# nv-tlabs/LION

Measured on AMD Instinct MI355X. Metric: shapes/sec @1000-step DDIM, Bx2048pts, higher is better.
Workload: dtype f32 (operands of the 3x3x3 voxel convolutions and of the long 1x1 convolutions cut into fp16 hi/lo pairs on the 16-bi...

## Files before the change

include/lion_hip.h:

```cpp
#ifndef LION_HIP_H_
#define LION_HIP_H_

#include <stddef.h>
#include <stdint.h>

#ifdef __cplusplus
extern "C" {
#endif

typedef void *lionStream_t;

#define LION_OK 0
#define LION_EINVAL (-1)
#define LION_EUNSUPPORTED (-2)
#define LION_EWORKSPACE (-3)

int lion_abi_version(void);

size_t lion_avg_voxelize_workspace_bytes(int B, int C, int N, int r);
int lion_avg_voxelize_forward(const float *feat, const int32_t *coords, int B, int C, int N,
                              int r, float *out, int32_t *ind, int32_t *cnt, void *ws,
                              size_t ws_bytes, lionStream_t stream);

int lion_voxelize_points_forward(const float *feat, const float *coords, int B, int C, int N,
// ... 31 lines not shown
int lion_grouping_backward(const float *gy, const int32_t *idx, int B, int C, int N, int M,
                           int U, float *gx, lionStream_t stream);

int lion_furthest_point_sampling(const float *coords, int B, int N, int M, int32_t *idx,
                                 lionStream_t stream);

int lion_gather_features_forward(const float *feat, const int32_t *idx, int B, int C, int N,
                                 int M, float *out, lionStream_t stream);
int lion_gather_features_backward(const float *gy, const int32_t *idx, int B, int C, int N,
                                  int M, float *gx, lionStream_t stream);

int lion_three_nn_interpolate_forward(const float *points, const float *centers,
                                      const float *cfeat, int B, int C, int N, int M,
                                      float *out, int32_t *idx, float *wgt,
                                      lionStream_t stream);
int lion_three_nn_interpolate_cat_forward(const float *points, const float *centers, const float *cfeat, const float *temb,
                                          int ld_t, const float *skip, int B, int C1, int C2, int C3, int N, int M,
                                          float *out, int32_t *idx, float *wgt, lionStream_t stream);
int lion_three_nn_interpolate_backward(const float *gy, const int32_t *idx, const float *wgt,
                                       int B, int C, int N, int M, float *gx,
                                       lionStream_t stream);

int lion_chamfer_forward(const float *xyz1, const float *xyz2, int B, int N, int M,
                         float *dist1, float *dist2, int32_t *idx1, int32_t *idx2,
                         lionStream_t stream);
int lion_chamfer_backward(const float *xyz1, const float *xyz2, const float *gdist1,
                          const float *gdist2, const int32_t *idx1, const int32_t *idx2, int B,
                          int N, int M, float *gxyz1, float *gxyz2, lionStream_t stream);
int lion_chamfer_loss_reduce(const float *dist1, const float *dist2, int B, int N, int M, float s1,
                             float s2, float *loss, lionStream_t stream);
int lion_chamfer_loss_backward(const float *xyz1, const float *xyz2, const int32_t *idx1,
                               const int32_t *idx2, const float *gloss, int B, int N, int M, float s1,
                               float s2, float *gxyz1, float *gxyz2, lionStream_t stream);

size_t lion_emd_workspace_bytes(int B, int N, int M);
int lion_emd_approxmatch(const float *xyz1, const float *xyz2, int B, int N, int M,
                         float *match, void *ws, size_t ws_bytes, lionStream_t stream);
int lion_emd_cost(const float *xyz1, const float *xyz2, int B, int N, int M, float *cost, void *ws,
                  size_t ws_bytes, lionStream_t stream);
int lion_emd_matchcost(const float *xyz1, const float *xyz2, const float *match, int B, int N,
                       int M, float *cost, void *ws, size_t ws_bytes, lionStream_t stream);
int lion_emd_matchcost_backward(const float *grad_cost, const float *xyz1, const float *xyz2,
                                const float *match, int B, int N, int M, float *grad1,
                                float *grad2, lionStream_t stream);

int lion_ddim_update(const float *x, const float *eps, const float *z, size_t numel, float s,
                     float c, float sigma, float *out, lionStream_t stream);
int lion_ddpm_update(const float *x, const float *eps, const float *z, size_t numel,
                     int t_is_zero, float k_outer, float k_a, float k_b, float scale,
                     float temp, float *out, lionStream_t stream);
int lion_chain_begin_step(const float *table, int n_steps, int32_t *counter, float *t_out, int B, float *cur,
                          lionStream_t stream);
int lion_chain_update_noise(int mode, const float *x, const float *eps, size_t numel, const float *cur,
                            const uint32_t *seed , uint32_t stream_id, float *out,
                            float *z_out, lionStream_t stream);
int lion_chain_begin_step_temb(const float *table, int n_steps, int32_t *counter, float *t_out, int B, float *cur,
                               const float *temb_table, int temb_width, float *temb_out, lionStream_t stream);
int lion_chain_update_noise_cm(int mode, const float *x, const float *eps_cm, int B, int N, const float *cur,
                               const uint32_t *seed, uint32_t stream_id, float *out, float *z_out, lionStream_t stream);
int lion_latent_unpack(const float *x, int B, int N, int D, float *all, float *coords, float *rest, lionStream_t stream);
int lion_concat_broadcast(const float *a, const float *t, int B, int Ca, int Ct, int N, int ld_t, float *out,
                          lionStream_t stream);

size_t lion_conv3d_packed_floats(int Cout, int Cin);
int lion_conv3d_pack_weights(const float *w, int Cout, int Cin, float *wp, lionStream_t stream);
int lion_conv3d_k3_forward(const float *x, const float *wp, const float *bias, int B, int Cin,
                           int Cout, int r, float *y, lionStream_t stream);
size_t lion_conv3d_wgrad_workspace_floats(int B, int Cin, int Cout, int r);
int lion_conv3d_k3_wgrad(const float *x, const float *gy, int B, int Cin, int Cout, int r, float *gw, float *ws,
                         size_t ws_floats, lionStream_t stream);
int lion_conv3d_k3_wgrad_split(const float *x, const float *gy, int B, int Cin, int Cout, int r, float *gw, float *ws,
                               size_t ws_floats, lionStream_t stream);
size_t lion_conv3d_wgrad_sparse_workspace_floats(int B, int Cin, int Cout, int r);
int lion_conv3d_k3_wgrad_split_sparse(const float *x, const float *gy, const int32_t *cnt, int B, int Cin, int Cout, int r,
                                      float *gw, float *ws, size_t ws_floats, lionStream_t stream);

int lion_conv3d_stat_tiles(int r, int Cout, int B, int sparse);
int lion_conv3d_k3_fused_forward(const float *x, const float *wp, const float *bias, int B, int Cin,
                                 int Cout, int r, const float *pro_a, const float *pro_b, const float *pro_bias,
                                 const float *tconst, float *y, float *stats, int32_t *occ, lionStream_t stream);
size_t lion_conv3d_occupancy_ints(int r, int Cout, int B);
int lion_conv3d_const_response(const float *wsum, const float *bias2, const float *bias1, const float *pro_a,
                               const float *pro_b, int B, int Cin, int Cout, float *tconst, lionStream_t stream);
int lion_conv3d_tile_occupancy(const int32_t *cnt, int B, int r, int Cout, int32_t *occ_m1, int32_t *occ_m2,
                               lionStream_t stream);
int lion_conv3d_tile_occupancy_aware(const int32_t *cnt, int B, int r, int Cout, int32_t *occ_m1, int32_t *occ_m2,
                                     int consumer_aware, lionStream_t stream);
int lion_groupnorm_fold(const float *stats, int B, int C, int T, int G, int voxels, const float *gamma,
                        const float *beta, const float *fac, const float *gbias, int ld_fg, float eps,
                        float *A, float *Bs, float *chmean, lionStream_t stream);
size_t lion_conv3d_split_packed_halfs(int Cout, int Cin);
int lion_conv3d_split_pack_weights(const float *w, int Cout, int Cin, uint16_t *wp, lionStream_t stream);
int lion_conv3d_split_stat_tiles(int r, int Cout);
int lion_conv3d_k3_split_forward(const float *x, const uint16_t *wp, const float *bias, int B, int Cin, int Cout,
                                 int r, const float *pro_a, const float *pro_b, const float *pro_bias,
                                 const float *tconst, float *y, float *stats, int32_t *occ, lionStream_t stream);
int lion_conv3d_k3_half_forward(const float *x, const uint16_t *wp, const float *bias, int B, int Cin, int Cout,
                                int r, const float *pro_a, const float *pro_b, const float *pro_bias,
                                const float *tconst, float *y, float *stats, int32_t *occ, lionStream_t stream);
size_t lion_skinny_packed_floats(int Cout, int Cin);
int lion_skinny_pack_weights(const float *w, int Cout, int Cin, float *wp, lionStream_t stream);
int lion_skinny_splits(int Cin, int Cout);
int lion_skinny_gemm(const float *pin, int ks_in, const float *bias_in, int act_in, const float *addT,
                     const float *wp, int nb, int Cin, int Cout, float *pout, lionStream_t stream);
int lion_skinny_finish(const float *A, int ks_a, const float *bias_a, const float *Bp, int ks_b, const float *resid,
                       int nb, int C, int mode, float *y, lionStream_t stream);
int lion_skinny_gemm_se_finish(const float *pin, int ks_in, const float *bias_in, int act_in, const float *wp, int nb, int Cin,
                               int Cout, const float *A, int ks_a, const float *bias_a, const float *resid, float *y,
                               lionStream_t stream);
int lion_to_channel_major(const float *a, int lda, int Ca, float *oa, const float *b, int ldb, int Cb, float *ob, int B,
                          lionStream_t stream);
int lion_from_channel_major(const float *x, int B, int C, float *y, lionStream_t stream);
int lion_groupnorm_fold_se(const float *stats, int B, int C, int T, int G, int voxels, const float *gamma,
                           const float *beta, const float *fac, const float *gbias, int ld_fg, float eps, const float *w1,
                           const float *w2, int H, float *A, float *Bs, lionStream_t stream);
int lion_se_gate(const float *chmean, const float *w1, const float *w2, int B, int C, int H, float *A,
                 float *Bs, lionStream_t stream);
int lion_trilinear_devoxelize_affine_forward(const float *coords, const float *feat, const float *scale,
                                             const float *shift, int B, int C, int N, int r, float *out,
                                             lionStream_t stream);
size_t lion_devoxelize_plan_bytes(int B, int N, int r);
int lion_trilinear_devoxelize_plan(const float *coords, int B, int N, int r, void *plan, size_t plan_bytes,
                                   lionStream_t stream);
int lion_trilinear_devoxelize_planned_forward(const void *plan, size_t plan_bytes, const float *coords, const float *feat,
                                              const float *scale, const float *shift, int B, int C, int N, int r,
                                              float *out, lionStream_t stream);

int lion_row_stats(const float *x, int rows, int L, float *stats, lionStream_t stream);
size_t lion_pwconv_packed_floats(int Cout, int Cin);
int lion_pwconv_pack_weights(const float *w, int Cout, int Cin, float *wp, lionStream_t stream);
int lion_pwconv_stat_tiles(int Cout, int Cin, int L);
int lion_pwconv_forward(const float *x, const float *wp, const float *bias, int B, int Cin, int Cout, int L,
                        const float *pro_a, const float *pro_b, float *y, float *stats, lionStream_t stream);
int lion_pwconv_forward_max(const float *x, const float *wp, const float *bias, int B, int Cin, int Cout, int L,
                            const float *pro_a, const float *pro_b, const float *out_a, const float *out_b,
                            float *stats, float *ymax, lionStream_t stream);
size_t lion_pwconv_split_packed_halfs(int Cout, int Cin);
int lion_pwconv_split_pack_weights(const float *w, int Cout, int Cin, uint16_t *wp, lionStream_t stream);
int lion_pwconv_split_pack_weights_t(const float *w, int Cout, int Cin, const uint16_t *wp, uint16_t *wpt, lionStream_t stream);
int lion_pwconv_split_stat_tiles(int Cout, int Cin, int L);
int lion_pwconv_split_forward(const float *x, const uint16_t *wp, const float *bias, int B, int Cin, int Cout, int L,
                              const float *pro_a, const float *pro_b, float *y, float *stats, lionStream_t stream);
int lion_linear_attention_core(const float *qkv, int B, int H, int D, int N, float *out, lionStream_t stream);
int lion_linear_attention_core_backward(const float *qkv, const float *gout, int B, int H, int D, int N, float *gqkv,
                                        lionStream_t stream);
int lion_linear_forward(const float *x, const float *wp, const float *bias, int B, int K, int O, int act, float slope,
                        float *y, lionStream_t stream);
int lion_affine_swish(const float *x, const float *A, const float *Bs, int rows, int L, float *y,
                      lionStream_t stream);
int lion_affine_swish_max(const float *x, const float *A, const float *Bs, int rows, int M, int U,
                          float *y, lionStream_t stream);
int lion_timestep_embedding(const float *t, const float *row, float scale, int B, int half, int D, float *emb,
                            lionStream_t stream);
int lion_affine_swish_add(const float *x, const float *A, const float *Bs, const float *addend, int rows, int L, float *y,
                          lionStream_t stream);

size_t lion_scatter_csr_workspace_bytes(int B, int E, int bins);
int lion_scatter_csr(const float *gy, const int32_t *idx, const float *w, int B, int C, int S, int E, int bins, void *ws,
                     size_t ws_bytes, float *gx, lionStream_t stream);

size_t lion_pwconv_wgrad_workspace_bytes(int B, int Cin, int Cout, int L);
int lion_pwconv_wgrad(const float *x, const float *gy, int B, int Cin, int Cout, int L, void *ws, size_t ws_bytes,
                      float *gw, float *gb, lionStream_t stream);

int lion_gn_train_fold(const float *stats, const float *gw, const float *gb, const float *fac, int fac_stride,
                       const float *bias, int bias_stride, int B, int C, int G, int L, float eps, float *A, float *Bs,
                       float *mean, float *rstd, lionStream_t stream);
int lion_row_stats64(const float *x, int rows, int L, double *stats, lionStream_t stream);
int lion_gn_train_fold64(const double *stats, const float *gw, const float *gb, const float *fac, int fac_stride,
                         const float *bias, int bias_stride, int B, int C, int G, int L, float eps, float *A,
                         float *Bs, float *mean, float *rstd, lionStream_t stream);
int lion_gn_train_bwd_fold(const float *S, const float *mean, const float *rstd, const float *gw, const float *gb,
                           const float *fac, int fac_stride, int B, int C, int G, int L, float *Q, float *R, float *dfac,
                           float *dbias, int d_stride, float *pw, const float *A, const double *xstats, const float *gate,
                           const float *qse, float *Aout, lionStream_t stream);
int lion_gn_train_param_grads(const float *pw, int B, int C, float *dgw, float *dgb, float *dxs, lionStream_t stream);
int lion_se_gate_fwd(const float *stats, const float *w1, const float *w2, int B, int C, int Cr, int L, float *mean, float *h,
                     float *g, float *zero, lionStream_t stream);
int lion_se_gate_bwd(const float *S, const float *g, const float *h, const float *mean, const float *w1, const float *w2, int B,
                     int C, int Cr, int L, float *dpre2, float *dpre1, float *Q, float *dw1, float *dw2, lionStream_t stream);
int lion_rows_dot2(const float *g, const float *v, const float *ws, int B, int C, int N, float *S, lionStream_t stream);
int lion_trilinear_devoxelize_backward_affine(const float *gy, const int32_t *inds, const float *wgts, const float *x,
                                              const float *Ap, const float *Q, const float *R, int B, int C, int N, int r3,
                                              float *dx, lionStream_t stream);
int lion_gn_se_gate_fwd(const double *xstats, const float *A, const float *Bs, const float *w1, const float *w2, int B, int C, int Cr,
                        int L, float *mean, float *h, float *g, float *A2, float *B2, lionStream_t stream);
int lion_gn_se_gate_bwd(const float *S, const double *xstats, const float *A, const float *Bs, const float *g, const float *h,
                        const float *mean, const float *w1, const float *w2, int B, int C, int Cr, int L, float *Sp, float *dpre2,
                        float *dpre1, float *Qse, float *dw1, float *dw2, lionStream_t stream);
int lion_affine_act(const float *x, const float *A, const float *Bs, int rows, int L, int act, float *y,
                    lionStream_t stream);
int lion_affine_act_bwd_stats(const float *x, const float *gy, const float *A, const float *Bs, int rows, int L, int act,
                              float *S, lionStream_t stream);
int lion_affine_act_bwd_apply(const float *x, const float *gy, const float *A, const float *Bs, const float *Q,
                              const float *R, int rows, int L, int act, float *dx, lionStream_t stream);
int lion_affine_act_dropout(const float *x, const float *A, const float *Bs, int rows, int L, int act, const uint64_t *seed,
                            float keep, float *y, lionStream_t stream);
int lion_affine_act_dropout_bwd_stats(const float *x, const float *gy, const float *A, const float *Bs, int rows, int L, int act,
                                      const uint64_t *seed, float keep, float *S, lionStream_t stream);
int lion_affine_act_dropout_bwd_apply(const float *x, const float *gy, const float *A, const float *Bs, const float *Q,
                                      const float *R, int rows, int L, int act, const uint64_t *seed, float keep, float *dx,
                                      lionStream_t stream);
int lion_affine_act_max(const float *x, const float *A, const float *Bs, int rows, int M, int U, int act, float *y,
                        lionStream_t stream);
int lion_affine_act_max_bwd_stats(const float *x, const float *gy, const float *A, const float *Bs, int rows, int M, int U,
                                  int act, float *S, lionStream_t stream);
int lion_affine_act_max_bwd_apply(const float *x, const float *gy, const float *A, const float *Bs, const float *Q,
                                  const float *R, int rows, int M, int U, int act, float *dx, lionStream_t stream);

int lion_adam_chunk(void);
int lion_adam_row(void);
int lion_adam_step(const uint64_t *table, const int32_t *numel, const int32_t *blockmap, int blocks, int tensors, const float *lr,
                   float beta1, float beta2, float eps, float weight_decay, float ema_decay, lionStream_t stream);

int lion_grad_sqnorm_partials(const uint64_t *table, const int32_t *numel, const int32_t *blockmap, int blocks, float *partials,
                              lionStream_t stream);
int lion_grad_clip_coef(const float *partials, int n, float max_norm, float *out2, lionStream_t stream);
int lion_adam_step_scaled(const uint64_t *table, const int32_t *numel, const int32_t *blockmap, int blocks, int tensors,
                          const float *lr, float beta1, float beta2, float eps, float weight_decay, float ema_decay,
                          const float *grad_scale, lionStream_t stream);

#define LION_ODE_RUNNING 0
#define LION_ODE_FINISHED 1
#define LION_ODE_TOO_SMALL_STEP (-1)
typedef struct lion_ode_ctrl {
  double t, h_abs, t_bound, direction, rtol, atol;
  double h, t_new, err_norm, h0, d1, sign;
  int32_t stage, cur, status, step_rejected;
  int32_t yslot, fslot, nfe, n_accepted;
  int32_t n_rejected, accepted, pad0, pad1;
} lion_ode_ctrl;
size_t lion_ode_partials_bytes(size_t n);
int lion_ode_stage(double *Y, const double *K, size_t n, lion_ode_ctrl *ctrl, float *x32, float *t_model, int B,
                   lionStream_t stream);
int lion_ode_drift(const float *eps, int cm_points, const float *x32, size_t n, const float *t_model, float beta_start,
                   float beta_delta, float neg_beta_start, float half_beta_delta, float one_minus_sigma2_0,
                   const float *mix_a, const float *mix_b, int mix_len, double *K, lion_ode_ctrl *ctrl,
                   lionStream_t stream);
// ... 9 lines not shown
```

lion_amd/_lib.py:

```python
from __future__ import annotations

import ctypes as C
import os

_HERE = os.path.dirname(os.path.abspath(__file__))
SO_PATH = os.environ.get("LION_HIP_SO") or os.path.join(_HERE, "csrc", "liblion_hip.so")

_vp, _i, _f, _sz = C.c_void_p, C.c_int, C.c_float, C.c_size_t

SIGNATURES = {
    "lion_abi_version": (_i, []),
    "lion_avg_voxelize_workspace_bytes": (_sz, [_i, _i, _i, _i]),
    "lion_avg_voxelize_forward": (_i, [_vp, _vp, _i, _i, _i, _i, _vp, _vp, _vp, _vp, _sz, _vp]),
    "lion_voxelize_points_forward": (_i, [_vp, _vp, _i, _i, _i, _i, _i, _f, _vp, _vp, _vp, _vp,
                                          _vp, _sz, _vp]),
    "lion_voxel_plan_bytes": (_sz, [_i, _i, _i]),
    "lion_voxel_index": (_i, [_vp, _i, _i, _i, _i, _f, _vp, _vp, _vp, _vp, _sz, _vp]),
    "lion_voxel_scatter": (_i, [_vp, _vp, _sz, _i, _i, _i, _i, _vp, _vp]),
    "lion_voxel_scatter_read": (_i, [_vp, _vp, _sz, _i, _i, _i, _i, _vp, _vp, _vp]),
    "lion_avg_voxelize_backward": (_i, [_vp, _vp, _vp, _i, _i, _i, _i, _vp, _vp]),
    "lion_trilinear_devoxelize_forward": (_i, [_vp, _vp, _i, _i, _i, _i, _i, _vp, _vp, _vp, _vp]),
    "lion_trilinear_devoxelize_backward": (_i, [_vp, _vp, _vp, _i, _i, _i, _i, _vp, _vp]),
    "lion_ball_query": (_i, [_vp, _vp, _i, _i, _i, _f, _i, _vp, _vp]),
    "lion_grouping_forward": (_i, [_vp, _vp, _i, _i, _i, _i, _i, _vp, _vp]),
    "lion_group_points_forward": (_i, [_vp, _vp, _vp, _vp, _i, _i, _i, _i, _i, _vp, _vp]),
    "lion_grouping_backward": (_i, [_vp, _vp, _i, _i, _i, _i, _i, _vp, _vp]),
    "lion_furthest_point_sampling": (_i, [_vp, _i, _i, _i, _vp, _vp]),
    "lion_gather_features_forward": (_i, [_vp, _vp, _i, _i, _i, _i, _vp, _vp]),
    "lion_gather_features_backward": (_i, [_vp, _vp, _i, _i, _i, _i, _vp, _vp]),
    "lion_three_nn_interpolate_forward": (_i, [_vp, _vp, _vp, _i, _i, _i, _i, _vp, _vp, _vp, _vp]),
    "lion_three_nn_interpolate_backward": (_i, [_vp, _vp, _vp, _i, _i, _i, _i, _vp, _vp]),
    "lion_chamfer_forward": (_i, [_vp, _vp, _i, _i, _i, _vp, _vp, _vp, _vp, _vp]),
    "lion_chamfer_backward": (_i, [_vp, _vp, _vp, _vp, _vp, _vp, _i, _i, _i, _vp, _vp, _vp]),
    "lion_chamfer_loss_reduce": (_i, [_vp, _vp, _i, _i, _i, _f, _f, _vp, _vp]),
    "lion_chamfer_loss_backward": (_i, [_vp, _vp, _vp, _vp, _vp, _i, _i, _i, _f, _f, _vp, _vp, _vp]),
    "lion_emd_workspace_bytes": (_sz, [_i, _i, _i]),
    "lion_emd_approxmatch": (_i, [_vp, _vp, _i, _i, _i, _vp, _vp, _sz, _vp]),
    "lion_emd_cost": (_i, [_vp, _vp, _i, _i, _i, _vp, _vp, _sz, _vp]),
    "lion_emd_matchcost": (_i, [_vp, _vp, _vp, _i, _i, _i, _vp, _vp, _sz, _vp]),
    "lion_emd_matchcost_backward": (_i, [_vp, _vp, _vp, _vp, _i, _i, _i, _vp, _vp, _vp]),
    "lion_conv3d_packed_floats": (_sz, [_i, _i]),
    "lion_conv3d_pack_weights": (_i, [_vp, _i, _i, _vp, _vp]),
    "lion_conv3d_k3_forward": (_i, [_vp, _vp, _vp, _i, _i, _i, _i, _vp, _vp]),
    "lion_conv3d_wgrad_workspace_floats": (_sz, [_i, _i, _i, _i]),
    "lion_conv3d_k3_wgrad": (_i, [_vp, _vp, _i, _i, _i, _i, _vp, _vp, _sz, _vp]),
    "lion_conv3d_k3_wgrad_split": (_i, [_vp, _vp, _i, _i, _i, _i, _vp, _vp, _sz, _vp]),
    "lion_conv3d_wgrad_sparse_workspace_floats": (_sz, [_i, _i, _i, _i]),
    "lion_conv3d_k3_wgrad_split_sparse": (_i, [_vp, _vp, _vp, _i, _i, _i, _i, _vp, _vp, _sz, _vp]),
    "lion_conv3d_stat_tiles": (_i, [_i, _i, _i, _i]),
    "lion_conv3d_k3_fused_forward": (_i, [_vp, _vp, _vp, _i, _i, _i, _i, _vp, _vp, _vp, _vp, _vp, _vp, _vp, _vp]),
    "lion_conv3d_const_response": (_i, [_vp, _vp, _vp, _vp, _vp, _i, _i, _i, _vp, _vp]),
    "lion_conv3d_occupancy_ints": (_sz, [_i, _i, _i]),
    "lion_conv3d_tile_occupancy": (_i, [_vp, _i, _i, _i, _vp, _vp, _vp]),
    "lion_conv3d_tile_occupancy_aware": (_i, [_vp, _i, _i, _i, _vp, _vp, _i, _vp]),
    "lion_conv3d_split_packed_halfs": (_sz, [_i, _i]),
    "lion_conv3d_split_pack_weights": (_i, [_vp, _i, _i, _vp, _vp]),
    "lion_conv3d_split_stat_tiles": (_i, [_i, _i]),
    "lion_conv3d_k3_split_forward": (_i, [_vp, _vp, _vp, _i, _i, _i, _i, _vp, _vp, _vp, _vp, _vp, _vp, _vp, _vp]),
    "lion_conv3d_k3_half_forward": (_i, [_vp, _vp, _vp, _i, _i, _i, _i, _vp, _vp, _vp, _vp, _vp, _vp, _vp, _vp]),
    "lion_groupnorm_fold": (_i, [_vp, _i, _i, _i, _i, _i, _vp, _vp, _vp, _vp, _i, _f, _vp, _vp, _vp, _vp]),
    "lion_groupnorm_fold_se": (_i, [_vp, _i, _i, _i, _i, _i, _vp, _vp, _vp, _vp, _i, _f, _vp, _vp, _i, _vp, _vp, _vp]),
    "lion_skinny_packed_floats": (_sz, [_i, _i]),
    "lion_skinny_pack_weights": (_i, [_vp, _i, _i, _vp, _vp]),
    "lion_skinny_splits": (_i, [_i, _i]),
    "lion_skinny_gemm": (_i, [_vp, _i, _vp, _i, _vp, _vp, _i, _i, _i, _vp, _vp]),
    "lion_skinny_gemm_se_finish": (_i, [_vp, _i, _vp, _i, _vp, _i, _i, _i, _vp, _i, _vp, _vp, _vp, _vp]),
    "lion_skinny_finish": (_i, [_vp, _i, _vp, _vp, _i, _vp, _i, _i, _i, _vp, _vp]),
    "lion_to_channel_major": (_i, [_vp, _i, _i, _vp, _vp, _i, _i, _vp, _i, _vp]),
    "lion_from_channel_major": (_i, [_vp, _i, _i, _vp, _vp]),
    "lion_se_gate": (_i, [_vp, _vp, _vp, _i, _i, _i, _vp, _vp, _vp]),
    "lion_trilinear_devoxelize_affine_forward": (_i, [_vp, _vp, _vp, _vp, _i, _i, _i, _i, _vp, _vp]),
    "lion_devoxelize_plan_bytes": (_sz, [_i, _i, _i]),
    "lion_trilinear_devoxelize_plan": (_i, [_vp, _i, _i, _i, _vp, _sz, _vp]),
    "lion_trilinear_devoxelize_planned_forward": (_i, [_vp, _sz, _vp, _vp, _vp, _vp, _i, _i, _i, _i, _vp, _vp]),
    "lion_row_stats": (_i, [_vp, _i, _i, _vp, _vp]),
    "lion_pwconv_packed_floats": (_sz, [_i, _i]),
    "lion_pwconv_pack_weights": (_i, [_vp, _i, _i, _vp, _vp]),
    "lion_pwconv_stat_tiles": (_i, [_i, _i, _i]),
    "lion_pwconv_forward": (_i, [_vp, _vp, _vp, _i, _i, _i, _i, _vp, _vp, _vp, _vp, _vp]),
    "lion_pwconv_forward_max": (_i, [_vp, _vp, _vp, _i, _i, _i, _i, _vp, _vp, _vp, _vp, _vp, _vp, _vp]),
    "lion_pwconv_split_packed_halfs": (_sz, [_i, _i]),
    "lion_pwconv_split_pack_weights": (_i, [_vp, _i, _i, _vp, _vp]),
    "lion_pwconv_split_pack_weights_t": (_i, [_vp, _i, _i, _vp, _vp, _vp]),
    "lion_pwconv_split_stat_tiles": (_i, [_i, _i, _i]),
    "lion_pwconv_split_forward": (_i, [_vp, _vp, _vp, _i, _i, _i, _i, _vp, _vp, _vp, _vp, _vp]),
    "lion_linear_attention_core": (_i, [_vp, _i, _i, _i, _i, _vp, _vp]),
    "lion_linear_attention_core_backward": (_i, [_vp, _vp, _i, _i, _i, _i, _vp, _vp]),
    "lion_linear_forward": (_i, [_vp, _vp, _vp, _i, _i, _i, _i, _f, _vp, _vp]),
    "lion_affine_swish": (_i, [_vp, _vp, _vp, _i, _i, _vp, _vp]),
    "lion_affine_swish_max": (_i, [_vp, _vp, _vp, _i, _i, _i, _vp, _vp]),
    "lion_timestep_embedding": (_i, [_vp, _vp, _f, _i, _i, _i, _vp, _vp]),
    "lion_affine_swish_add": (_i, [_vp, _vp, _vp, _vp, _i, _i, _vp, _vp]),
    "lion_scatter_csr_workspace_bytes": (_sz, [_i, _i, _i]),
    "lion_scatter_csr": (_i, [_vp, _vp, _vp, _i, _i, _i, _i, _i, _vp, _sz, _vp, _vp]),
    "lion_pwconv_wgrad_workspace_bytes": (_sz, [_i, _i, _i, _i]),
    "lion_pwconv_wgrad": (_i, [_vp, _vp, _i, _i, _i, _i, _vp, _sz, _vp, _vp, _vp]),
    "lion_gn_train_fold": (_i, [_vp, _vp, _vp, _vp, _i, _vp, _i, _i, _i, _i, _i, _f, _vp, _vp, _vp, _vp, _vp]),
    "lion_row_stats64": (_i, [_vp, _i, _i, _vp, _vp]),
    "lion_gn_train_fold64": (_i, [_vp, _vp, _vp, _vp, _i, _vp, _i, _i, _i, _i, _i, _f, _vp, _vp, _vp, _vp, _vp]),
    "lion_gn_train_bwd_fold": (_i, [_vp, _vp, _vp, _vp, _vp, _vp, _i, _i, _i, _i, _i, _vp, _vp, _vp, _vp, _i, _vp, _vp, _vp, _vp, _vp,
                                    _vp, _vp]),
    "lion_gn_train_param_grads": (_i, [_vp, _i, _i, _vp, _vp, _vp, _vp]),
    "lion_adam_chunk": (_i, []),
    "lion_adam_row": (_i, []),
    "lion_adam_step": (_i, [_vp, _vp, _vp, _i, _i, _vp, _f, _f, _f, _f, _f, _vp]),
    "lion_grad_sqnorm_partials": (_i, [_vp, _vp, _vp, _i, _vp, _vp]),
    "lion_grad_clip_coef": (_i, [_vp, _i, _f, _vp, _vp]),
    "lion_adam_step_scaled": (_i, [_vp, _vp, _vp, _i, _i, _vp, _f, _f, _f, _f, _f, _vp, _vp]),
    "lion_se_gate_fwd": (_i, [_vp, _vp, _vp, _i, _i, _i, _i, _vp, _vp, _vp, _vp, _vp]),
    "lion_se_gate_bwd": (_i, [_vp, _vp, _vp, _vp, _vp, _vp, _i, _i, _i, _i, _vp, _vp, _vp, _vp, _vp, _vp]),
    "lion_rows_dot2": (_i, [_vp, _vp, _vp, _i, _i, _i, _vp, _vp]),
    "lion_trilinear_devoxelize_backward_affine": (_i, [_vp, _vp, _vp, _vp, _vp, _vp, _vp, _i, _i, _i, _i, _vp, _vp]),
    "lion_gn_se_gate_fwd": (_i, [_vp, _vp, _vp, _vp, _vp, _i, _i, _i, _i, _vp, _vp, _vp, _vp, _vp, _vp]),
    "lion_gn_se_gate_bwd": (_i, [_vp, _vp, _vp, _vp, _vp, _vp, _vp, _vp, _vp, _i, _i, _i, _i, _vp, _vp, _vp, _vp, _vp, _vp, _vp]),
    "lion_affine_act": (_i, [_vp, _vp, _vp, _i, _i, _i, _vp, _vp]),
    "lion_affine_act_bwd_stats": (_i, [_vp, _vp, _vp, _vp, _i, _i, _i, _vp, _vp]),
    "lion_affine_act_bwd_apply": (_i, [_vp, _vp, _vp, _vp, _vp, _vp, _i, _i, _i, _vp, _vp]),
    "lion_affine_act_dropout": (_i, [_vp, _vp, _vp, _i, _i, _i, _vp, _f, _vp, _vp]),
    "lion_affine_act_dropout_bwd_stats": (_i, [_vp, _vp, _vp, _vp, _i, _i, _i, _vp, _f, _vp, _vp]),
    "lion_affine_act_dropout_bwd_apply": (_i, [_vp, _vp, _vp, _vp, _vp, _vp, _i, _i, _i, _vp, _f, _vp, _vp]),
    "lion_affine_act_max": (_i, [_vp, _vp, _vp, _i, _i, _i, _i, _vp, _vp]),
    "lion_affine_act_max_bwd_stats": (_i, [_vp, _vp, _vp, _vp, _i, _i, _i, _i, _vp, _vp]),
    "lion_affine_act_max_bwd_apply": (_i, [_vp, _vp, _vp, _vp, _vp, _vp, _i, _i, _i, _i, _vp, _vp]),
    "lion_ddim_update": (_i, [_vp, _vp, _vp, _sz, _f, _f, _f, _vp, _vp]),
    "lion_ddpm_update": (_i, [_vp, _vp, _vp, _sz, _i, _f, _f, _f, _f, _f, _vp, _vp]),
    "lion_chain_begin_step": (_i, [_vp, _i, _vp, _vp, _i, _vp, _vp]),
    "lion_chain_update_noise": (_i, [_i, _vp, _vp, _sz, _vp, _vp, C.c_uint32, _vp, _vp, _vp]),
    "lion_chain_begin_step_temb": (_i, [_vp, _i, _vp, _vp, _i, _vp, _vp, _i, _vp, _vp]),
    "lion_chain_update_noise_cm": (_i, [_i, _vp, _vp, _i, _i, _vp, _vp, C.c_uint32, _vp, _vp, _vp]),
    "lion_latent_unpack": (_i, [_vp, _i, _i, _i, _vp, _vp, _vp, _vp]),
    "lion_concat_broadcast": (_i, [_vp, _vp, _i, _i, _i, _i, _i, _vp, _vp]),
    "lion_three_nn_interpolate_cat_forward": (_i, [_vp, _vp, _vp, _vp, _i, _vp, _i, _i, _i, _i, _i, _i, _vp, _vp, _vp, _vp]),
    "lion_ode_partials_bytes": (_sz, [_sz]),
    "lion_ode_stage": (_i, [_vp, _vp, _sz, _vp, _vp, _vp, _i, _vp]),
    "lion_ode_drift": (_i, [_vp, _i, _vp, _sz, _vp, _f, _f, _f, _f, _f, _vp, _vp, _i, _vp, _vp, _vp]),
    "lion_ode_error_partials": (_i, [_vp, _vp, _sz, _vp, _vp, _vp]),
    "lion_ode_control": (_i, [_vp, _sz, _vp, _vp]),
}



_ERR = {-1: "LION_EINVAL (bad shape / null pointer)",
        -2: "LION_EUNSUPPORTED (shape outside what the kernels implement)",
        -3: "LION_EWORKSPACE (workspace too small)"}

_lib = None


def load() -> C.CDLL:
    global _lib
    if _lib is not None:
        return _lib
    if not os.path.exists(SO_PATH):
        raise RuntimeError(
            f"lion_amd: HIP extension not built: {SO_PATH} is missing. Run "
            f"`python -c 'import __graft_entry__ as g; g.build()'` or lion_amd/csrc/build.sh. "
            f"There is no CPU fallback.")
    lib = C.CDLL(SO_PATH)
    for name, (res, args) in SIGNATURES.items():
        try:
            fn = getattr(lib, name)
        except AttributeError as e:
            raise RuntimeError(f"lion_amd: {SO_PATH} does not export {name}") from e
        fn.restype = res
        fn.argtypes = args
    _lib = lib
    return lib


def check(code: int, what: str) -> None:
    if code != 0:
        msg = _ERR.get(code, f"hipError {code}" if code > 0 else f"error {code}")
        raise RuntimeError(f"lion_amd: {what} failed: {msg}")


# ... 40 lines not shown
```

lion_amd/chain.py:

```python
from __future__ import annotations

from collections import OrderedDict

import numpy as np
import torch

from . import _lib, _wcache

DDIM, DDPM = 0, 1
RECORD = None
TEMB_TABLE = __import__("os").environ.get("LION_TEMB_TABLE", "1") != "0"
CHANNEL_MAJOR_EPS = __import__("os").environ.get("LION_CHAIN_CM_EPS", "1") != "0"

def policy_key() -> tuple:
    from . import conv_ops, fused_ops, geometry
    from .models import pvcnn2_ada
    return (pvcnn2_ada.SPARSE_CONV1, pvcnn2_ada.FUSE_INFERENCE, pvcnn2_ada.OVERLAP_POINT_BRANCH, geometry.ENABLED,
            geometry.SPLIT_GRAPH, conv_ops.SPLIT, fused_ops.PW_SPLIT, pvcnn2_ada.VOX_PLAN, TEMB_TABLE, fused_ops.MAX_RECOMPUTE,
            pvcnn2_ada.SKIP_UNREAD, pvcnn2_ada.SKIP_UNREAD_LEVEL2, CHANNEL_MAJOR_EPS, conv_ops.PRECISION)


def channel_major(model, shape) -> bool:
    n_pts, n_cls = getattr(model, "num_points", 0), getattr(model, "num_classes", 0)
    return CHANNEL_MAJOR_EPS and hasattr(model, "geometry_source") and n_cls == 4 and int(np.prod(shape)) == n_pts * n_cls


def same_conditioning(owner, condition_input, clip_feat) -> bool:
    same = lambda buf, new: (buf is None) == (new is None) and (buf is None or buf.shape == new.shape)
    return same(owner.cond, condition_input) and same(owner.clip, clip_feat)


class LRU:

    def __init__(self, capacity=4):
        self._entries, self._capacity = OrderedDict(), capacity

    def lookup(self, key, usable, build):
        hit = self._entries.get(key)
        if hit is not None and usable(hit):
            self._entries.move_to_end(key)
            return hit
        self._entries.pop(key, None)
        hit = self._entries[key] = build()
        while len(self._entries) > self._capacity:
            self._entries.popitem(last=False)
        return hit

    def clear(self):
        self._entries.clear()


class CapturedStep:

    def __init__(self, model, step, x, *, warmup=2, split=None):
        self.model, self.x = model, x
        self.fingerprint, self.policy = _wcache.fingerprint(model), policy_key()
        self.pinned = []
        dev = x.device
        from . import geometry
        src = getattr(model, "geometry_source", None)
        self.geo_graphs = self.graph_b = self.graphs = self.waits = self.geo_plan = None
        if split is None:
            split = geometry.SPLIT_GRAPH and src is not None and not geometry.ENABLED
        main = torch.cuda.current_stream(dev)
        side = torch.cuda.Stream(device=dev)
        side.wait_stream(main)
        with _wcache.pinning(self.pinned):
            with torch.no_grad(), torch.cuda.stream(side):
                for _ in range(warmup):
                    step()
            main.wait_stream(side)
            if split:
                self.geo_stream = torch.cuda.Stream(device=dev)
                self.ev_step = torch.cuda.Event()

                def geo(boundary=None):
                    mods, coords = src(x)
                    return geometry.compute_chain(mods, coords, boundary=boundary)
                self.geo_stream.wait_stream(main)
                with torch.no_grad(), torch.cuda.stream(self.geo_stream):
                    geo()
                main.wait_stream(self.geo_stream)
                torch.cuda.synchronize(dev)
                self.geo_graphs = [torch.cuda.CUDAGraph()]
                gs = torch.cuda.Stream(device=dev)
                gs.wait_stream(main)

                def geo_cut(i):
                    if i == 1:
                        self.geo_graphs[-1].capture_end()
                        self.geo_graphs.append(torch.cuda.CUDAGraph())
                        self.geo_graphs[-1].capture_begin(pool=self.geo_graphs[0].pool())
                with torch.no_grad(), torch.cuda.stream(gs):
                    self.geo_graphs[0].capture_begin()
                    try:
                        self.geo_plan = geo(geo_cut)
                    finally:
                        self.geo_graphs[-1].capture_end()
                main.wait_stream(gs)
                torch.cuda.synchronize(dev)
                self.geo_stage_of_graph = [0, self.geo_plan["stages"] - 1][:len(self.geo_graphs)]
                self.ev_geo = [torch.cuda.Event() for _ in self.geo_graphs]
# ... 166 lines not shown
```

lion_amd/csrc/conv3d.hip:

```cpp
#include "common.h"

namespace {

typedef float f32x16 __attribute__((ext_vector_type(16)));
#ifndef LION_CONV_KC
#define LION_CONV_KC 4
#endif
#ifndef LION_CONV_WAVES
#define LION_CONV_WAVES 2
#endif
constexpr int KC = LION_CONV_KC;

__device__ __forceinline__ float pro_act(float v, float pa, float pb) {
  const float t = v * pa + pb;
  return swish_fast(t);
}

template <int TD, int TH, int TW, int COT, int VB, bool PRO, bool STATS>
__global__ __launch_bounds__(256, LION_CONV_WAVES) void conv3d_k3_kernel(const float *__restrict__ x,
                                                                const float *__restrict__ wp,
                                                                const float *__restrict__ bias,
                                                                float *__restrict__ y, int Cin,
                                                                int Cout, int r,
                                                                const float *__restrict__ pro_a,
                                                                const float *__restrict__ pro_b,
                                                                const float *__restrict__ pro_bias,
                                                                const float *__restrict__ tconst,
                                                                float *__restrict__ stats,
                                                                int32_t *__restrict__ occ, int B,
                                                                int ntiles) {
  constexpr int TM = 256;
  static_assert(TD * TH * TW == 4 * VB * 32, "tile voxels = 4 waves x VB column blocks x 32");
  constexpr int HD = TD + 2, HH = TH + 2, HW = TW + 2, HALO = HD * HH * HW;
  constexpr int NJ = (HALO + TM - 1) / TM;
  constexpr int WV4 = KC * 27 * COT / 4;
  constexpr int NWV = (WV4 + TM - 1) / TM;
  constexpr int CB = COT / 32;
  constexpr int SWS = ((KC * 27 * COT + 255) / 256) * 256 + 256;
  extern __shared__ __attribute__((aligned(16))) float smem[];
  float *sx = smem;
  float *sw = sx + ((KC * HALO + 3) & ~3);
  float *sbias = sw + 2 * SWS;
  const int npro = PRO ? ((Cin + 63) & ~63) : 0;
  float *spa = sbias + COT, *spb = spa + npro;
  float *spc = spb + npro;
  float *sred = spc + npro;
  float *sT = sx;
  const int tid = threadIdx.x, lane = tid & 63, wave = __builtin_amdgcn_readfirstlane(tid >> 6);
  __shared__ int s_work;
  const bool queued = occ != nullptr;
  const int ncz = Cout / COT;
  for (int iter = 0;; ++iter) {
  int b, tile, co0;
  if (queued) {
    __syncthreads();
    if (tid == 0) s_work = atomicAdd(occ + 2 * B * ntiles, 1);
    __syncthreads();
    const int work = s_work;
    if (work >= B * ntiles * ncz) break;
    const int item = work / ncz;
    b = item % B;
    tile = occ[B * ntiles + b * ntiles + item / B];
    co0 = (work % ncz) * COT;
  } else {
    if (iter) break;
    b = blockIdx.x;
    tile = blockIdx.y;
    co0 = blockIdx.z * COT;
  }
  const int ntw = r / TW, nth = r / TH;
  const int tw_i = tile % ntw, th_i = (tile / ntw) % nth, td_i = tile / (ntw * nth);
  const int d0 = td_i * TD, h0 = th_i * TH, w0 = tw_i * TW;
  const int r2 = r * r, r3 = r2 * r;

  const bool delta = PRO && tconst != nullptr;
  if (PRO) {
    for (int c = tid; c < Cin; c += TM) {
      const float pa = pro_a[(size_t)b * Cin + c], pb = pro_b[(size_t)b * Cin + c];
      spa[c] = pa;
      spb[c] = pb;
      spc[c] = delta ? pro_act(pro_bias ? pro_bias[c] : 0.f, pa, pb) : 0.f;
    }
  }
// ... 87 lines not shown
      for (int cb = 0; cb < CB; ++cb) av[buf][cb] = ap[cb * 32];
    };
    if (wave_on) {
    lds_step(0, 0);
#pragma unroll
    for (int st = 0; st < NS; ++st) {
      if (st + 1 < NS) lds_step(st + 1, (st + 1) & 1);
      __builtin_amdgcn_sched_barrier(0);
#pragma unroll
      for (int cb = 0; cb < CB; ++cb)
#pragma unroll
        for (int vb = 0; vb < VB; ++vb)
          acc[cb][vb] = __builtin_amdgcn_mfma_f32_32x32x2f32(av[st & 1][cb], bv[st & 1][vb], acc[cb][vb], 0, 0, 0);
      __builtin_amdgcn_sched_barrier(0);
    }
    }
  }

  if (delta) {
    __syncthreads();
    for (int e = tid; e < 27 * COT; e += TM) sT[e] = tconst[((size_t)b * 27 + e / COT) * Cout + co0 + e % COT];
    __syncthreads();
  } else if (empty) {
    __syncthreads();
  }
  float *yb = y + ((size_t)b * Cout + co0) * r3;
#pragma unroll
  for (int vb = 0; vb < VB; ++vb) {
    const int v = (wave * VB + vb) * 32 + (lane & 31);
    const int d = v / (TH * TW), h = (v / TW) % TH, w = v % TW;
    const int gv = ((d0 + d) * r + (h0 + h)) * r + (w0 + w);
    const int gd = d0 + d, gh = h0 + h, gw = w0 + w;
    const int cfg = (((gd == 0 ? 0 : gd == r - 1 ? 2 : 1) * 3 + (gh == 0 ? 0 : gh == r - 1 ? 2 : 1)) * 3 +
                     (gw == 0 ? 0 : gw == r - 1 ? 2 : 1));
    const float *addv = delta ? sT + cfg * COT : sbias;
#pragma unroll
    for (int cb = 0; cb < CB; ++cb)
#pragma unroll
      for (int i = 0; i < 16; ++i) {
        const int co = cb * 32 + (i & 3) + 8 * (i >> 2) + 4 * (lane >> 5);
        const float o = acc[cb][vb][i] + addv[co];
        acc[cb][vb][i] = o;
        yb[(size_t)co * r3 + gv] = o;
      }
  }
  if (STATS) {
    constexpr int NWAVE = 4;
#pragma unroll
    for (int cb = 0; cb < CB; ++cb)
#pragma unroll
      for (int i = 0; i < 16; ++i) {
        float s1 = acc[cb][0][i], s2 = acc[cb][0][i] * acc[cb][0][i];
#pragma unroll
        for (int vb = 1; vb < VB; ++vb) { s1 += acc[cb][vb][i]; s2 += acc[cb][vb][i] * acc[cb][vb][i]; }
        s1 = row16_sum_rn(s1); s2 = row16_sum_rn(s2);
        s1 = row_pair_sum_odd_rows(s1); s2 = row_pair_sum_odd_rows(s2);
        if ((lane & 31) == 16) {
          const int co = cb * 32 + (i & 3) + 8 * (i >> 2) + 4 * (lane >> 5);
          sred[(wave * COT + co) * 2] = s1;
          sred[(wave * COT + co) * 2 + 1] = s2;
        }
      }
    __syncthreads();
    if (tid < COT) {
      float s1 = 0.f, s2 = 0.f;
#pragma unroll
      for (int w = 0; w < NWAVE; ++w) { s1 += sred[(w * COT + tid) * 2]; s2 += sred[(w * COT + tid) * 2 + 1]; }
      float *o = stats + (((size_t)b * Cout + co0 + tid) * ntiles + tile) * 2;
      o[0] = s1;
      o[1] = s2;
    }
  }
  }
  if (queued && tid == 0) {
    int32_t *q = occ + 2 * B * ntiles;
    if (atomicAdd(q + 1, 1) == (int)gridDim.x - 1) { q[0] = 0; q[1] = 0; }
  }
}

__global__ void gn_fold_kernel(const float *__restrict__ stats, int C, int T, int G, float count,
                               const float *__restrict__ gamma, const float *__restrict__ beta,
                               const float *__restrict__ fac, const float *__restrict__ gbias, int ld_fg, float eps,
                               float *__restrict__ A, float *__restrict__ Bs, float *__restrict__ chmean) {
  __shared__ double cs[64][2];
  __shared__ double gs[2];
  const int b = blockIdx.y, g = blockIdx.x, cpg = C / G, tid = threadIdx.x;
  int cp2 = 1;
  while (cp2 < cpg) cp2 <<= 1;
  const int LPC = 256 / cp2, ch = tid / LPC, sub = tid % LPC;
  double s1 = 0.0, s2 = 0.0;
  if (ch < cpg) {
    const float2 *p = reinterpret_cast<const float2 *>(stats + (((size_t)b * C + g * cpg + ch) * T) * 2);
    for (int t = sub; t < T; t += LPC) { const float2 v = p[t]; s1 += (double)v.x; s2 += (double)v.y; }
  }
  for (int m = 1; m < LPC && m < 64; m <<= 1) { s1 += __shfl_xor(s1, m, 64); s2 += __shfl_xor(s2, m, 64); }
  if (LPC > 64) {
    __shared__ double ws[4][2];
    if ((tid & 63) == 0) { ws[tid >> 6][0] = s1; ws[tid >> 6][1] = s2; }
    __syncthreads();
    if (sub == 0) {
      s1 = 0.0; s2 = 0.0;
      for (int w = 0; w < LPC / 64; ++w) { s1 += ws[(tid >> 6) + w][0]; s2 += ws[(tid >> 6) + w][1]; }
    }
  }
  if (ch < cpg && sub == 0) {
    cs[ch][0] = s1;
    cs[ch][1] = s2;
    chmean[(size_t)b * C + g * cpg + ch] = (float)(s1 / count);
  }
  __syncthreads();
  if (tid == 0) {
    double g1 = 0.0, g2 = 0.0;
    for (int c = 0; c < cpg; ++c) { g1 += cs[c][0]; g2 += cs[c][1]; }
    gs[0] = g1;
    gs[1] = g2;
  }
  __syncthreads();
  if (tid < cpg) {
    const double n = (double)count * cpg;
    const double mean = gs[0] / n;
    double var = gs[1] / n - mean * mean;
    var = var > 0.0 ? var : 0.0;
    const float rstd = (float)(1.0 / sqrt(var + (double)eps));
    const int c = g * cpg + tid;
    const float f = fac[(size_t)b * ld_fg + c], gb = gbias[(size_t)b * ld_fg + c];
    const float a0 = rstd * gamma[c];
    A[(size_t)b * C + c] = a0 * f;
    Bs[(size_t)b * C + c] = (beta[c] - (float)mean * a0) * f + gb;
  }
}

__global__ __launch_bounds__(256) void gn_fold_se_kernel(const float *__restrict__ stats, int C, int T, int G, float count,
                                                         const float *__restrict__ gamma, const float *__restrict__ beta,
                                                         const float *__restrict__ fac, const float *__restrict__ gbias,
                                                         int ld_fg, float eps, const float *__restrict__ w1,
                                                         const float *__restrict__ w2, int H, float *__restrict__ A,
                                                         float *__restrict__ Bs) {
  __shared__ double cs[256][2];
  __shared__ float sA[256], sB[256], sm[256], sh[128];
  const int b = blockIdx.x, tid = threadIdx.x, lane = tid & 63, wave = tid >> 6, cpg = C / G;
  int cp2 = 1;
  while (cp2 < C) cp2 <<= 1;
  const int LPC = 256 / cp2, ch = tid / LPC, sub = tid % LPC;
  double s1 = 0.0, s2 = 0.0;
  if (ch < C) {
    const float2 *p = reinterpret_cast<const float2 *>(stats + (((size_t)b * C + ch) * T) * 2);
    for (int t = sub; t < T; t += LPC) { const float2 v = p[t]; s1 += (double)v.x; s2 += (double)v.y; }
  }
  for (int m = 1; m < LPC; m <<= 1) { s1 += __shfl_xor(s1, m, 64); s2 += __shfl_xor(s2, m, 64); }
  if (ch < C && sub == 0) { cs[ch][0] = s1; cs[ch][1] = s2; }
  __syncthreads();
  if (tid < C) {
    const int g0 = (tid / cpg) * cpg;
    double g1 = 0.0, g2 = 0.0;
    for (int k = 0; k < cpg; ++k) { g1 += cs[g0 + k][0]; g2 += cs[g0 + k][1]; }
    const double n = (double)count * cpg, mean = g1 / n;
    double var = g2 / n - mean * mean;
    var = var > 0.0 ? var : 0.0;
    const float rstd = (float)(1.0 / sqrt(var + (double)eps));
    const float f = fac[(size_t)b * ld_fg + tid], gb = gbias[(size_t)b * ld_fg + tid];
    const float a0 = rstd * gamma[tid];
    const float a = a0 * f, bb = (beta[tid] - (float)mean * a0) * f + gb;
    sA[tid] = a;
    sB[tid] = bb;
    sm[tid] = a * (float)(cs[tid][0] / count) + bb;
  }
  __syncthreads();
  for (int j = wave; j < H; j += 4) {
    float acc = 0.f;
    for (int c = lane; c < C; c += 64) acc += w1[(size_t)j * C + c] * sm[c];
#pragma unroll
    for (int m = 32; m >= 1; m >>= 1) acc += __shfl_xor(acc, m, 64);
    if (lane == 0) sh[j] = acc > 0.f ? acc : 0.f;
  }
  __syncthreads();
  if (tid < C) {
    float acc = 0.f;
    for (int j = 0; j < H; ++j) acc += w2[(size_t)tid * H + j] * sh[j];
    const float g = 1.0f / (1.0f + expf(-acc));
    A[(size_t)b * C + tid] = sA[tid] * g;
    Bs[(size_t)b * C + tid] = sB[tid] * g;
  }
}

__global__ __launch_bounds__(1024) void conv_tile_occ_kernel(const int32_t *__restrict__ cnt, int r, int TD, int TH,
                                                             int32_t *__restrict__ occ1, int32_t *__restrict__ occ2,
                                                             int aware) {
  __shared__ unsigned col[32 * 32];
  __shared__ int flag[2][256];
  const int b = blockIdx.x, B = gridDim.x, tid = threadIdx.x;
  const int nth = r / TH, ntiles = (r / TD) * nth, total = B * ntiles;
  for (int i = tid; i < r * r; i += 1024) col[i] = 0u;
  __syncthreads();
  const int4 *c4 = reinterpret_cast<const int4 *>(cnt + (size_t)b * r * r * r);
  for (int i = tid; i < (r * r * r) >> 2; i += 1024) {
    const int4 v = c4[i];
    if (v.x | v.y | v.z | v.w) {
      const unsigned m4 = (v.x ? 1u : 0u) | (v.y ? 2u : 0u) | (v.z ? 4u : 0u) | (v.w ? 8u : 0u);
      atomicOr(&col[(i << 2) / r], m4 << ((i << 2) % r));
    }
  }
  __syncthreads();
  const int RW = 64 / r;
  for (int e = tid; e < 2 * ntiles; e += 1024) {
    const int t = e % ntiles, margin = 1 + e / ntiles;
    const int dt = (t / nth) * TD, ht = (t % nth) * TH;
    int mask = 0;
    for (int w = 0; w < 4; ++w) {
      const int dl = dt + (w * RW) / TH, hl = ht + (w * RW) % TH;
      unsigned any = 0u;
      for (int d = max(dl - margin, 0); d <= min(dl + margin, r - 1); ++d)
        for (int h = max(hl - margin, 0); h <= min(hl + RW - 1 + margin, r - 1); ++h) any |= col[d * r + h];
      mask |= (any ? 1 : 0) << w;
    }
    flag[margin - 1][t] = mask;
  }
  __syncthreads();
  __shared__ unsigned long long bal[2][4];
  const int m = tid >> 8, t = tid & 255, lane = tid & 63, w = (tid >> 6) & 3;
  const bool live = tid < 512 && t < ntiles;
  const int f = live ? flag[m][t] : 0;
  const unsigned long long bl = __ballot(f != 0);
  if (tid < 512 && lane == 0) bal[m][w] = bl;
  __syncthreads();
  if (live) {
    int32_t *occ = m == 0 ? occ1 : occ2;
    if (occ) {
      int before = __popcll(bal[m][w] & ((1ull << lane) - 1ull)), occupied = 0;
      for (int ww = 0; ww < 4; ++ww) {
        const int c = __popcll(bal[m][ww]);
        if (ww < w) before += c;
        occupied += c;
      }
      int32_t *fl = occ + (size_t)b * ntiles, *list = occ + total + (size_t)b * ntiles;
      int need = flag[1][t] != 0;
      if (m == 0) {
        if (aware == 2) {
          need = 0;
        } else {
          const int td = t / nth, th = t % nth;
          for (int dd = max(td - 1, 0); dd <= min(td + 1, r / TD - 1); ++dd)
            for (int hh = max(th - 1, 0); hh <= min(th + 1, nth - 1); ++hh) need |= flag[1][dd * nth + hh] != 0;
        }
      }
      fl[t] = f | (need << 8) | ((m == 1 && flag[0][t] != 0) ? (1 << 9) : 0);
      list[f ? before : occupied + (t - before)] = t;
      if (b == 0 && t == 0) { occ[2 * total] = 0; occ[2 * total + 1] = 0; occ[2 * total + 2] = aware; }
    }
  }
}

__global__ __launch_bounds__(256) void conv_tconst_kernel(const float *__restrict__ wsum, const float *__restrict__ bias2,
                                                          const float *__restrict__ bias1, const float *__restrict__ pro_a,
                                                          const float *__restrict__ pro_b, int Cin, int Cout,
                                                          float *__restrict__ tconst) {
  __shared__ float sc[256];
  const int cfg = blockIdx.x, b = blockIdx.y, tid = threadIdx.x;
  for (int c = tid; c < Cin; c += 256)
    sc[c] = pro_act(bias1 ? bias1[c] : 0.f, pro_a[(size_t)b * Cin + c], pro_b[(size_t)b * Cin + c]);
  __syncthreads();
  for (int co = tid; co < Cout; co += 256) {
    double acc = bias2 ? (double)bias2[co] : 0.0;
    const float *w = wsum + (size_t)cfg * Cin * Cout + co;
    for (int c = 0; c < Cin; ++c) acc += (double)w[(size_t)c * Cout] * (double)sc[c];
    tconst[((size_t)b * 27 + cfg) * Cout + co] = (float)acc;
  }
}

__global__ void conv3d_pack_kernel(const float *__restrict__ w, int Cout, int Cin, int Cin_pad,
                                   float *__restrict__ wp) {
  const int i = blockIdx.x * blockDim.x + threadIdx.x;
  const int total = Cin_pad * 27 * Cout;
  if (i >= total) return;
  const int co = i % Cout, t = (i / Cout) % 27, ci = i / (Cout * 27);
  wp[i] = ci < Cin ? w[((size_t)co * Cin + ci) * 27 + t] : 0.f;
}

template <int TD, int TH, int TW, int COT, int VB>
static int launch_conv_t(const float *x, const float *wp, const float *bias, float *y, int B, int Cin,
                         int Cout, int r, const float *pa, const float *pb, const float *pbias, const float *tconst,
                         float *stats, int32_t *occ, hipStream_t st) {
  const int tiles = (r / TD) * (r / TH) * (r / TW);
  int n_cu = 0;
  if (int e = lion_cu_count(&n_cu)) return e;
  const long items = (long)B * tiles * (Cout / COT);
  const dim3 grid = occ ? dim3((unsigned)(items < 2L * n_cu ? items : 2L * n_cu)) : dim3(B, tiles, Cout / COT);
  constexpr int NT = 256;
  constexpr int HALO = (TD + 2) * (TH + 2) * (TW + 2);
  constexpr int SWS = ((KC * 27 * COT + 255) / 256) * 256 + 256;
  static_assert(KC * HALO >= 27 * COT, "the response table must fit the input tile buffer");
  const size_t LDS = (size_t)(((KC * HALO + 3) & ~3) + 2 * SWS + COT + (pa ? 3 * ((Cin + 63) & ~63) : 0) +
                              (NT / 64) * COT * 2) * 4;
#define LION_CONV_GO(PRO_, ST_)                                                                           \
  {                                                                                                       \
    static LionLdsLimit cfg = {};                                                                         \
    if (int e = lion_dynamic_lds(&conv3d_k3_kernel<TD, TH, TW, COT, VB, PRO_, ST_>, LDS, cfg)) return e;  \
    conv3d_k3_kernel<TD, TH, TW, COT, VB, PRO_, ST_><<<grid, NT, LDS, st>>>(x, wp, bias, y, Cin, Cout, r, \
                                                                            pa, pb, pbias, tconst, stats, occ, B, \
                                                                            tiles);                      \
  }
  if (pa && stats) LION_CONV_GO(true, true)
  else if (pa) LION_CONV_GO(true, false)
  else if (stats) LION_CONV_GO(false, true)
  else LION_CONV_GO(false, false)
#undef LION_CONV_GO
  LION_LAUNCH_CHECK();
  return 0;
}

struct ConvPlan { int vb, cot, tiles; };
static ConvPlan conv_plan(int r, int Cout, int B, bool sparse) {
  const int r3 = r * r * r;
  if (!sparse && Cout % 64 == 0 && r >= 16 && (long)(r3 / 512) * (Cout / 64) * B >= 512) return {4, 64, r3 / 512};
  if (Cout % 64 == 0 && (long)(r3 / 256) * (Cout / 64) * B >= 512) return {2, 64, r3 / 256};
  if (Cout % 32 == 0 && r >= 16 && !sparse) return {4, 32, r3 / 512};
  if (Cout % 32 == 0 && r >= 16) return {2, 32, r3 / 256};
  if (Cout % 32 == 0) return {1, 32, r3 / 128};
  return {0, 0, 0};
}

static void conv_tile_dims(int r, int vb, int *td, int *th, int *tw) {
  *tw = r;
  if (r == 32) { *td = vb == 2 ? 2 : 4; *th = 4; }
  else if (r == 16) { *td = vb == 2 ? 4 : 8; *th = 4; }
  else { *td = vb == 2 ? 4 : 2; *th = 8; }
}

static int launch_conv(const float *x, const float *wp, const float *bias, float *y, int B, int Cin, int Cout,
                       int r, const float *pa, const float *pb, const float *pbias, const float *tconst, float *stats,
                       int32_t *occ, hipStream_t st) {
  const ConvPlan p = conv_plan(r, Cout, B, occ != nullptr);
#define LION_CONV_TILE(R_, VB_, COT_, TD_, TH_, TW_)                                                       \
  if (r == R_ && p.vb == VB_ && p.cot == COT_)                                                             \
    return launch_conv_t<TD_, TH_, TW_, COT_, VB_>(x, wp, bias, y, B, Cin, Cout, r, pa, pb, pbias, tconst, stats, occ, st);
  LION_CONV_TILE(32, 2, 64, 2, 4, 32)
  LION_CONV_TILE(32, 4, 64, 4, 4, 32)
  LION_CONV_TILE(16, 4, 64, 8, 4, 16)
  LION_CONV_TILE(32, 4, 32, 4, 4, 32)
  LION_CONV_TILE(32, 2, 32, 2, 4, 32)
  LION_CONV_TILE(16, 2, 32, 4, 4, 16)
  LION_CONV_TILE(16, 2, 64, 4, 4, 16)
  LION_CONV_TILE(16, 4, 32, 8, 4, 16)
  LION_CONV_TILE(8, 2, 64, 4, 8, 8)
  LION_CONV_TILE(8, 1, 32, 2, 8, 8)
#undef LION_CONV_TILE
  return LION_EUNSUPPORTED;
}

}

int lion_internal_sparse_tile_dims(int r, int *td, int *th) {
  if (r != 16 && r != 32) return LION_EUNSUPPORTED;
  const ConvPlan a = conv_plan(r, 64, 32, true), b = conv_plan(r, 32, 32, true), c = conv_plan(r, 64, 1, true);
  if (!a.vb || a.vb != b.vb || a.vb != c.vb) return LION_EUNSUPPORTED;
  int tw;
  conv_tile_dims(r, a.vb, td, th, &tw);
  return 0;
}

extern "C" {

size_t lion_conv3d_packed_floats(int Cout, int Cin) {
  return (size_t)((Cin + KC - 1) / KC * KC) * 27 * Cout;
}

int lion_conv3d_pack_weights(const float *w, int Cout, int Cin, float *wp, lionStream_t stream) {
  if (!w || !wp || Cout <= 0 || Cin <= 0) return LION_EINVAL;
  const int Cin_pad = (Cin + KC - 1) / KC * KC;
  const int total = Cin_pad * 27 * Cout;
  conv3d_pack_kernel<<<lion_cdiv(total, 256), 256, 0, static_cast<hipStream_t>(stream)>>>(w, Cout, Cin, Cin_pad, wp);
  LION_LAUNCH_CHECK();
  return 0;
}

int lion_conv3d_k3_fused_forward(const float *x, const float *wp, const float *bias, int B, int Cin,
                                 int Cout, int r, const float *pro_a, const float *pro_b, const float *pro_bias,
                                 const float *tconst, float *y, float *stats, int32_t *occ, lionStream_t stream) {
  if (!x || !wp || !y || B <= 0 || Cin <= 0 || Cout <= 0) return LION_EINVAL;
  if ((pro_a == nullptr) != (pro_b == nullptr)) return LION_EINVAL;
  if (tconst && !pro_a) return LION_EINVAL;
  if (occ && pro_a && !tconst) return LION_EINVAL;
  if (Cin % KC != 0 || (pro_a && Cin > 256)) return LION_EUNSUPPORTED;
  hipStream_t st = static_cast<hipStream_t>(stream);
  if (r != 8 && r != 16 && r != 32) return LION_EUNSUPPORTED;
  return launch_conv(x, wp, bias, y, B, Cin, Cout, r, pro_a, pro_b, pro_bias, tconst, stats, occ, st);
}

int lion_conv3d_k3_forward(const float *x, const float *wp, const float *bias, int B, int Cin,
                           int Cout, int r, float *y, lionStream_t stream) {
  return lion_conv3d_k3_fused_forward(x, wp, bias, B, Cin, Cout, r, nullptr, nullptr, nullptr, nullptr, y, nullptr,
                                      nullptr, stream);
}

int lion_conv3d_const_response(const float *wsum, const float *bias2, const float *bias1, const float *pro_a,
                               const float *pro_b, int B, int Cin, int Cout, float *tconst, lionStream_t stream) {
  if (!wsum || !pro_a || !pro_b || !tconst || B <= 0 || Cin <= 0 || Cout <= 0) return LION_EINVAL;
  if (Cin > 256) return LION_EUNSUPPORTED;
  conv_tconst_kernel<<<dim3(27, B), 256, 0, static_cast<hipStream_t>(stream)>>>(wsum, bias2, bias1, pro_a, pro_b, Cin,
                                                                                 Cout, tconst);
  LION_LAUNCH_CHECK();
  return 0;
}

size_t lion_conv3d_occupancy_ints(int r, int Cout, int B) {
  if (r != 16 && r != 32) return 0;
  return (size_t)2 * B * conv_plan(r, Cout, B, true).tiles + 4;
}

int lion_conv3d_tile_occupancy(const int32_t *cnt, int B, int r, int Cout, int32_t *occ_m1, int32_t *occ_m2,
                               lionStream_t stream) {
  return lion_conv3d_tile_occupancy_aware(cnt, B, r, Cout, occ_m1, occ_m2, 0, stream);
}

int lion_conv3d_tile_occupancy_aware(const int32_t *cnt, int B, int r, int Cout, int32_t *occ_m1, int32_t *occ_m2,
                                     int consumer_aware, lionStream_t stream) {
  if (!cnt || (!occ_m1 && !occ_m2) || B <= 0 || Cout <= 0) return LION_EINVAL;
  if (r != 16 && r != 32) return LION_EUNSUPPORTED;
  const ConvPlan p = conv_plan(r, Cout, B, true);
  if (!p.vb || p.tiles > 256 || (((uintptr_t)cnt) & 15) != 0) return LION_EUNSUPPORTED;
  int td, th, tw;
  conv_tile_dims(r, p.vb, &td, &th, &tw);
  conv_tile_occ_kernel<<<B, 1024, 0, static_cast<hipStream_t>(stream)>>>(cnt, r, td, th, occ_m1, occ_m2,
                                                                         consumer_aware == 2 ? 2 : consumer_aware ? 1 : 0);
  LION_LAUNCH_CHECK();
  return 0;
}

int lion_conv3d_stat_tiles(int r, int Cout, int B, int sparse) {
  if (r != 8 && r != 16 && r != 32) return 0;
  return conv_plan(r, Cout, B, sparse != 0).tiles;
}

int lion_groupnorm_fold_se(const float *stats, int B, int C, int T, int G, int voxels, const float *gamma,
                           const float *beta, const float *fac, const float *gbias, int ld_fg, float eps, const float *w1,
                           const float *w2, int H, float *A, float *Bs, lionStream_t stream) {
  if (!stats || !gamma || !beta || !fac || !gbias || !w1 || !w2 || !A || !Bs) return LION_EINVAL;
  if (B <= 0 || C <= 0 || T <= 0 || G <= 0 || C % G != 0 || ld_fg < C || H <= 0) return LION_EINVAL;
  if (C > 256 || C < 4 || H > 128) return LION_EUNSUPPORTED;
  gn_fold_se_kernel<<<B, 256, 0, static_cast<hipStream_t>(stream)>>>(stats, C, T, G, (float)voxels, gamma, beta, fac, gbias,
                                                                     ld_fg, eps, w1, w2, H, A, Bs);
  LION_LAUNCH_CHECK();
  return 0;
}

int lion_groupnorm_fold(const float *stats, int B, int C, int T, int G, int voxels, const float *gamma,
                        const float *beta, const float *fac, const float *gbias, int ld_fg, float eps,
                        float *A, float *Bs, float *chmean, lionStream_t stream) {
  if (!stats || !gamma || !beta || !fac || !gbias || !A || !Bs || !chmean) return LION_EINVAL;
  if (B <= 0 || C <= 0 || T <= 0 || G <= 0 || C % G != 0 || C / G > 64 || ld_fg < C) return LION_EINVAL;
  gn_fold_kernel<<<dim3(G, B), 256, 0, static_cast<hipStream_t>(stream)>>>(stats, C, T, G, (float)voxels, gamma,
                                                                         beta, fac, gbias, ld_fg, eps, A, Bs, chmean);
  LION_LAUNCH_CHECK();
  return 0;
}

}
```

lion_amd/csrc/devoxelize.hip:

```cpp
#include "common.h"

namespace {

template <bool V> struct BoolT { static constexpr bool value = V; };

struct Corners {
  int ix[8];
  float w[8];
};

__device__ __forceinline__ Corners corners_of(float x, float y, float z, int r, int r2) {
  Corners k;
  const float xl = floorf(x), yl = floorf(y), zl = floorf(z);
  const float xd1 = sub_rn(x, xl), yd1 = sub_rn(y, yl), zd1 = sub_rn(z, zl);
  const float xd0 = sub_rn(1.0f, xd1), yd0 = sub_rn(1.0f, yd1), zd0 = sub_rn(1.0f, zd1);
  k.w[0] = mul_rn(mul_rn(xd0, yd0), zd0);
  k.w[1] = mul_rn(mul_rn(xd0, yd0), zd1);
  k.w[2] = mul_rn(mul_rn(xd0, yd1), zd0);
  k.w[3] = mul_rn(mul_rn(xd0, yd1), zd1);
  k.w[4] = mul_rn(mul_rn(xd1, yd0), zd0);
  k.w[5] = mul_rn(mul_rn(xd1, yd0), zd1);
  k.w[6] = mul_rn(mul_rn(xd1, yd1), zd0);
  k.w[7] = mul_rn(mul_rn(xd1, yd1), zd1);
  const int xlo = (int)xl, ylo = (int)yl, zlo = (int)zl;
  const int xs = (xd1 > 0.0f) ? r2 : 0;
  const int ys = (yd1 > 0.0f) ? r : 0;
  const int zs = (zd1 > 0.0f) ? 1 : 0;
  k.ix[0] = xlo * r2 + ylo * r + zlo;
  k.ix[1] = k.ix[0] + zs;
  k.ix[2] = k.ix[0] + ys;
  k.ix[3] = k.ix[2] + zs;
  k.ix[4] = k.ix[0] + xs;
  k.ix[5] = k.ix[4] + zs;
  k.ix[6] = k.ix[4] + ys;
  k.ix[7] = k.ix[6] + zs;
  return k;
}

template <int CT, bool AFF>
__global__ __launch_bounds__(256) void devox_fwd_kernel(const float *__restrict__ coords,
                                                        const float *__restrict__ feat, int C,
                                                        int N, int r, int training,
                                                        float *__restrict__ out,
                                                        int32_t *__restrict__ inds,
                                                        float *__restrict__ wgts,
                                                        const float *__restrict__ scale,
                                                        const float *__restrict__ shift) {
  const int b = blockIdx.z, i = blockIdx.x * blockDim.x + threadIdx.x;
  if (i >= N) return;
  const int r2 = r * r, r3 = r2 * r;
  const float *co = coords + (size_t)b * 3 * N;
  Corners k = corners_of(co[i], co[i + N], co[i + 2 * N], r, r2);
  if (training && blockIdx.y == 0) {
#pragma unroll
    for (int q = 0; q < 8; ++q) {
      wgts[((size_t)b * 8 + q) * N + i] = k.w[q];
      inds[((size_t)b * 8 + q) * N + i] = k.ix[q];
    }
  }
#pragma unroll
  for (int q = 0; q < 8; ++q) k.ix[q] = min(max(k.ix[q], 0), r3 - 1);
  const int c0 = blockIdx.y * CT, c1 = min(C, c0 + CT);
  const float *f = feat + ((size_t)b * C + c0) * r3;
  float *o = out + ((size_t)b * C + c0) * N + i;
  float wsum = 0.f;
  if (AFF) {
    wsum = k.w[0];
#pragma unroll
    for (int q = 1; q < 8; ++q) wsum += k.w[q];
  }
#pragma unroll 4
  for (int c = c0; c < c1; ++c, f += r3, o += N) {
    float v[8];
#pragma unroll
    for (int q = 0; q < 8; ++q) v[q] = f[k.ix[q]];
    float acc = mul_rn(k.w[0], v[0]);
#pragma unroll
    for (int q = 1; q < 8; ++q) acc = add_rn(acc, mul_rn(k.w[q], v[q]));
    if (AFF) acc = acc * scale[(size_t)b * C + c] + shift[(size_t)b * C + c] * wsum;
    *o = acc;
  }
}


template <int LD, bool AFF>
__global__ __launch_bounds__(256) void devox_slab_kernel(
    const float *__restrict__ coords, const float *__restrict__ feat, int C, int N, int r, int PX,
    int XS, int CT, int CI, int slab_floats, int training, float *__restrict__ out,
    int32_t *__restrict__ inds, float *__restrict__ wgts, const float *__restrict__ scale,
    const float *__restrict__ shift) {
  extern __shared__ __attribute__((aligned(16))) unsigned char smem[];
  float *lds = reinterpret_cast<float *>(smem);
  constexpr int PP = 8;
  const int tid = threadIdx.x, b = blockIdx.y, c0 = blockIdx.x * CT;
  const int nch = min(CT, C - c0);
  const int r2 = r * r, r3 = r2 * r;
  const float *co = coords + (size_t)b * 3 * N;
  uint16_t *sorted = reinterpret_cast<uint16_t *>(lds + 2 * slab_floats);
  int *scnt = reinterpret_cast<int *>(sorted + ((N + 1) & ~1));
  unsigned *need = reinterpret_cast<unsigned *>(scnt + XS);

  const int ngrp = (nch + CI - 1) / CI;
  const int nit = ngrp * XS;
  auto slab_count4 = [&](int g, int xs) {
    return XS == 1 ? (min(CI, nch - g * CI) * r3) >> 2 : ((min(r, xs * PX + PX + 1) - xs * PX) * r2) >> 2;
  };
  typedef __attribute__((address_space(3))) float lds_float;
  const uint32_t lds_base = (uint32_t)(uintptr_t)(lds_float *)lds;
  const int wave = __builtin_amdgcn_readfirstlane(tid >> 6);
  auto issue = [&](int it) {
    const int g = it / XS, xs = it - g * XS;
    const float4 *src = reinterpret_cast<const float4 *>(feat + ((size_t)b * C + c0 + g * CI) * r3 + (size_t)xs * PX * r2);
    const int n4 = slab_count4(g, xs);
    const uint32_t dst0 = lds_base + (uint32_t)((it & 1) * slab_floats * 4 + wave * 1024);
    const int row0 = XS == 1 ? 0 : xs * PX * r;
#pragma unroll
    for (int j = 0; j < LD; ++j) {
      const int f = tid + j * 256;
      const float4 *gp = src + f;
      const uint32_t dst = __builtin_amdgcn_readfirstlane(dst0 + j * 4096);
      int row = (4 * f) / r;
      if (XS == 1) row %= r2;
      else row += row0;
      const bool want = f < n4 && ((need[row >> 5] >> (row & 31)) & 1u);
      if (want) {
        unsigned keep;
        asm volatile("s_mov_b32 %0, m0\n\ts_mov_b32 m0, %2\n\ts_nop 0\n\tglobal_load_lds_dwordx4 %1, off\n\ts_mov_b32 m0, %0"
                     : "=&s"(keep) : "v"(gp), "s"(dst) : "memory");
      }
    }
  };
  const int nwords = (r2 + 31) >> 5;
  for (int w = tid; w < nwords; w += 256) need[w] = 0u;
  __syncthreads();
  for (int i = tid; i < N; i += 256) {
    const float x = co[i], y = co[i + N];
    const float xl = floorf(x), yl = floorf(y);
    if (xl >= 0.f && yl >= 0.f && xl < (float)r && yl < (float)r) {
      const int x0 = (int)xl, y0 = (int)yl;
      const int x1 = min(x0 + (sub_rn(x, xl) > 0.0f ? 1 : 0), r - 1), y1 = min(y0 + (sub_rn(y, yl) > 0.0f ? 1 : 0), r - 1);
      const int ra = x0 * r + y0, rb = x0 * r + y1, rc = x1 * r + y0, rd = x1 * r + y1;
      atomicOr(&need[ra >> 5], 1u << (ra & 31));
      atomicOr(&need[rb >> 5], 1u << (rb & 31));
      atomicOr(&need[rc >> 5], 1u << (rc & 31));
      atomicOr(&need[rd >> 5], 1u << (rd & 31));
    }
  }
  __syncthreads();
  issue(0);

  for (int s2 = tid; s2 < XS; s2 += 256) scnt[s2] = 0;
  __syncthreads();
  int sl0[PP];
#pragma unroll
  for (int p = 0; p < PP; ++p) {
    const int i = tid + p * 256;
    sl0[p] = -1;
    if (i < N) {
      sl0[p] = min(max((int)floorf(co[i]) / PX, 0), XS - 1);
      if (XS > 1) atomicAdd(&scnt[sl0[p]], 1);
    }
  }
  __syncthreads();
  if (tid == 0) {
    int run = 0;
    for (int s2 = 0; s2 < XS; ++s2) { const int c = scnt[s2]; scnt[s2] = run; run += c; }
  }
  __syncthreads();
#pragma unroll
  for (int p = 0; p < PP; ++p) {
    const int i = tid + p * 256;
    if (i < N) sorted[XS > 1 ? atomicAdd(&scnt[sl0[p]], 1) : i] = (uint16_t)i;
  }
  __syncthreads();

  int ix0[PP], xsl[PP], pid[PP];
  float xd1[PP], yd1[PP], zd1[PP];
#pragma unroll
  for (int p = 0; p < PP; ++p) {
    const int k = tid + p * 256;
    xsl[p] = -1;
    ix0[p] = 0;
    pid[p] = 0;
    xd1[p] = yd1[p] = zd1[p] = 0.f;
    if (k < N) {
      const int i = sorted[k];
      pid[p] = i;
      const float x = co[i], y = co[i + N], z = co[i + 2 * N];
      const Corners kk = corners_of(x, y, z, r, r2);
      if (training && blockIdx.x == 0) {
#pragma unroll
        for (int q = 0; q < 8; ++q) {
          wgts[((size_t)b * 8 + q) * N + i] = kk.w[q];
          inds[((size_t)b * 8 + q) * N + i] = kk.ix[q];
        }
      }
      const float xl = floorf(x), yl = floorf(y), zl = floorf(z);
      xd1[p] = sub_rn(x, xl);
      yd1[p] = sub_rn(y, yl);
      zd1[p] = sub_rn(z, zl);
      ix0[p] = kk.ix[0];
      xsl[p] = min(max((int)xl / PX, 0), XS - 1);
      const int xin = (int)xl - xsl[p] * PX;
      const bool ok = xl >= 0.f && yl >= 0.f && zl >= 0.f && xl < (float)r && yl < (float)r && zl < (float)r &&
                      kk.ix[7] < r3 && xin >= 0 && xin < PX;
      if (!ok) xsl[p] = -2;
    }
  }

  for (int it = 0; it < nit; ++it) {
    const int g = it / XS, xs = it - g * XS;
    const int cg = c0 + g * CI, cin = min(CI, nch - g * CI);
    float *buf = lds + (it & 1) * slab_floats;
    asm volatile("s_waitcnt vmcnt(0)" ::: "memory");
    __syncthreads();
    if (it + 1 < nit) issue(it + 1);
    const int base = xs * PX * r2;
    float *o = out + ((size_t)b * C + cg) * N;
#pragma unroll
    for (int p = 0; p < PP; ++p) {
      if (xsl[p] == xs) {
        const float xd0 = sub_rn(1.0f, xd1[p]), yd0 = sub_rn(1.0f, yd1[p]), zd0 = sub_rn(1.0f, zd1[p]);
        const int xo = (xd1[p] > 0.0f) ? r2 : 0, yo = (yd1[p] > 0.0f) ? r : 0, zo = (zd1[p] > 0.0f) ? 1 : 0;
        const float w0 = mul_rn(mul_rn(xd0, yd0), zd0), w1 = mul_rn(mul_rn(xd0, yd0), zd1[p]);
        const float w2 = mul_rn(mul_rn(xd0, yd1[p]), zd0), w3 = mul_rn(mul_rn(xd0, yd1[p]), zd1[p]);
        const float w4 = mul_rn(mul_rn(xd1[p], yd0), zd0), w5 = mul_rn(mul_rn(xd1[p], yd0), zd1[p]);
        const float w6 = mul_rn(mul_rn(xd1[p], yd1[p]), zd0), w7 = mul_rn(mul_rn(xd1[p], yd1[p]), zd1[p]);
        float wsum = w0;
        if (AFF) { wsum += w1; wsum += w2; wsum += w3; wsum += w4; wsum += w5; wsum += w6; wsum += w7; }
        const float *f0 = buf + (ix0[p] - base);
        for (int ci = 0; ci < cin; ++ci, f0 += r3) {
          const float *f1 = f0 + xo;
          const float v0 = f0[0], v1 = f0[zo], v2 = f0[yo], v3 = f0[yo + zo];
          const float v4 = f1[0], v5 = f1[zo], v6 = f1[yo], v7 = f1[yo + zo];
          float a = mul_rn(w0, v0);
          a = add_rn(a, mul_rn(w1, v1));
          a = add_rn(a, mul_rn(w2, v2));
          a = add_rn(a, mul_rn(w3, v3));
          a = add_rn(a, mul_rn(w4, v4));
          a = add_rn(a, mul_rn(w5, v5));
          a = add_rn(a, mul_rn(w6, v6));
          a = add_rn(a, mul_rn(w7, v7));
          if (AFF) a = a * scale[(size_t)b * C + cg + ci] + shift[(size_t)b * C + cg + ci] * wsum;
          o[(size_t)ci * N + pid[p]] = a;
        }
      } else if (xsl[p] == -2 && xs == 0) {
        for (int ci = 0; ci < cin; ++ci) o[(size_t)ci * N + pid[p]] = 0.f;
      }
    }
  }
}

constexpr int DVR_R = 32, DVR_NT = 512, DVR_PP = 2048 / DVR_NT;
constexpr int DVR_RING_BYTES = 144 * 1024;
constexpr int DVR_NJ = 9;

__device__ __forceinline__ void wait_vm_uniform(int n) {
  n = __builtin_amdgcn_readfirstlane(n);
#define LION_WVM(k) case k: asm volatile("s_waitcnt vmcnt(" #k ")" ::: "memory"); break;
  switch (n < 0 ? 0 : n) {
    LION_WVM(0) LION_WVM(1) LION_WVM(2) LION_WVM(3) LION_WVM(4) LION_WVM(5) LION_WVM(6) LION_WVM(7) LION_WVM(8) LION_WVM(9)
    LION_WVM(10) LION_WVM(11) LION_WVM(12) LION_WVM(13) LION_WVM(14) LION_WVM(15) LION_WVM(16) LION_WVM(17) LION_WVM(18)
    LION_WVM(19) LION_WVM(20) LION_WVM(21) LION_WVM(22) LION_WVM(23) LION_WVM(24) LION_WVM(25) LION_WVM(26) LION_WVM(27)
    LION_WVM(28) LION_WVM(29) LION_WVM(30) LION_WVM(31) LION_WVM(32) LION_WVM(33) LION_WVM(34) LION_WVM(35) LION_WVM(36)
    LION_WVM(37) LION_WVM(38) LION_WVM(39)
  default: asm volatile("s_waitcnt vmcnt(40)" ::: "memory"); break;
  }
#undef LION_WVM
}

template <int G> constexpr int devox_plan_stride() { return 16 + (DVR_NJ * DVR_NT / (G / 4)) * 2 + 2048 * 16 + 2048; }

template <bool AFF, int G, int MODE>
__global__ __launch_bounds__(DVR_NT) void devox_ring_kernel(const float *__restrict__ coords,
                                                            const float *__restrict__ feat, int C, int N, int CT,
                                                            int training, float *__restrict__ out,
                                                            int32_t *__restrict__ inds, float *__restrict__ wgts,
                                                            const float *__restrict__ scale,
                                                            const float *__restrict__ shift, int dmax,
                                                            unsigned char *__restrict__ plan) {
  extern __shared__ __attribute__((aligned(16))) unsigned char smem[];
  constexpr int PP = DVR_PP, r = DVR_R, r2 = r * r, r3 = r2 * r, NT = DVR_NT;
  constexpr int PPR = r / G, NP = r2 * PPR, nwords = NP / 32, LP = G / 4;
  constexpr int NPMAX = DVR_NJ * NT / LP;
  static_assert(nwords <= 128, "two bitmap words per lane of the ranking wave");
  float *lds = reinterpret_cast<float *>(smem);
  const int tid = threadIdx.x, b = blockIdx.y, c0 = blockIdx.x * CT;
  const int nch = min(CT, C - c0);
  unsigned *need = reinterpret_cast<unsigned *>(smem + DVR_RING_BYTES);
  unsigned *base = need + nwords;
  uint16_t *plist = reinterpret_cast<uint16_t *>(base + nwords);
  float *s_sc = reinterpret_cast<float *>(plist + NPMAX);
  int *s_np = reinterpret_cast<int *>(s_sc + 32);
  const float *co = coords + (size_t)b * 3 * N;
  unsigned char *pl_b = (MODE != 0) ? plan + (size_t)b * devox_plan_stride<G>() : nullptr;
  const uint16_t *pl_list = reinterpret_cast<const uint16_t *>(pl_b + 16);
  uint16_t *pl_off = reinterpret_cast<uint16_t *>(pl_b + 16 + NPMAX * 2);
  signed char *pl_st = reinterpret_cast<signed char *>(pl_b + 16 + NPMAX * 2 + 2048 * 16);

  if (tid < nwords) need[tid] = 0u;
  if (AFF && tid < 2 * 16) {
    const int ci = tid & 15;
    s_sc[tid] = ci < nch ? (tid < 16 ? scale : shift)[(size_t)b * C + c0 + ci] : 0.f;
  }
  __syncthreads();
  int np = 0, nj = 0, buf_bytes = 0, D = 2;
  bool fits = false;
  int goff[DVR_NJ];
  typedef __attribute__((address_space(3))) float lds_float;
  const uint32_t lds_base = (uint32_t)(uintptr_t)(lds_float *)lds;
  const int wave = __builtin_amdgcn_readfirstlane(tid >> 6);
  int ops = 0;
  int mark[4] = {0, 0, 0, 0};
  auto ring_shape = [&]() {
    nj = (np * LP + NT - 1) / NT;
    buf_bytes = nj * NT * 16;
    D = nj == 0 ? 2 : min(min(dmax, 4), DVR_RING_BYTES / (nj ? buf_bytes : 1));
    fits = nj <= DVR_NJ && D >= 2;
  };
  auto issue = [&](int ci) {
    const float *src = feat + ((size_t)b * C + c0 + ci) * r3;
    const uint32_t dst0 = lds_base + (uint32_t)((ci % D) * buf_bytes + wave * 1024);
#pragma unroll
    for (int j = 0; j < DVR_NJ; ++j) {
      if (j < nj) {
        const uint32_t dst = __builtin_amdgcn_readfirstlane(dst0 + j * (NT * 16));
// ... 212 lines not shown
  const float *wg = wgts + (size_t)b * 8 * N;
  for (int i = tid; i < N; i += nt) {
    const float gv = g[i];
#pragma unroll
    for (int q = 0; q < 8; ++q) {
      const int ix = min(max(id[(size_t)q * N + i], 0), r3 - 1) - lo;
      if (ix >= 0 && ix < part) atomicAdd(slab + ix, mul_rn(wg[(size_t)q * N + i], gv));
    }
  }
  __syncthreads();
  float *o = gx + ((size_t)b * C + c) * r3 + lo;
  for (int v = tid * 4; v < part; v += nt * 4)
    *reinterpret_cast<float4 *>(o + v) = *reinterpret_cast<const float4 *>(slab + v);
}

__global__ __launch_bounds__(1024) void devox_bwd_affine_kernel(const float *__restrict__ gy, const int32_t *__restrict__ inds,
                                                                const float *__restrict__ wgts, const float *__restrict__ x,
                                                                const float *__restrict__ Ap, const float *__restrict__ Q,
                                                                const float *__restrict__ R, int C, int N, int r3,
                                                                float *__restrict__ dx) {
  extern __shared__ __attribute__((aligned(16))) unsigned char smem[];
  float *slab = reinterpret_cast<float *>(smem);
  const int tid = threadIdx.x, nt = blockDim.x;
  const int c = blockIdx.x, b = blockIdx.y;
  const int part = r3 / gridDim.z, lo = blockIdx.z * part;
  const size_t row = (size_t)b * C + c;
  const float a = Ap[row], q = Q[row], rr = R[row];
  const float *xr = x + row * r3 + lo;
  for (int v = tid * 4; v < part; v += nt * 4) {
    const float4 t = *reinterpret_cast<const float4 *>(xr + v);
    *reinterpret_cast<float4 *>(slab + v) = make_float4(q + rr * t.x, q + rr * t.y, q + rr * t.z, q + rr * t.w);
  }
  __syncthreads();
  const float *g = gy + row * N;
  const int32_t *id = inds + (size_t)b * 8 * N;
  const float *wg = wgts + (size_t)b * 8 * N;
  for (int i = tid; i < N; i += nt) {
    const float gv = a * g[i];
#pragma unroll
    for (int k = 0; k < 8; ++k) {
      const int ix = min(max(id[(size_t)k * N + i], 0), r3 - 1) - lo;
      if (ix >= 0 && ix < part) atomicAdd(slab + ix, mul_rn(wg[(size_t)k * N + i], gv));
    }
  }
  __syncthreads();
  float *o = dx + row * r3 + lo;
  for (int v = tid * 4; v < part; v += nt * 4)
    *reinterpret_cast<float4 *>(o + v) = *reinterpret_cast<const float4 *>(slab + v);
}

__global__ void devox_bwd_atomic_kernel(const float *__restrict__ gy,
                                        const int32_t *__restrict__ inds,
                                        const float *__restrict__ wgts, int C, int N, int r3,
                                        int CT, float *__restrict__ gx) {
  const int b = blockIdx.z, i = blockIdx.x * blockDim.x + threadIdx.x;
  if (i >= N) return;
  int ix[8];
  float w[8];
  for (int q = 0; q < 8; ++q) {
    ix[q] = min(max(inds[((size_t)b * 8 + q) * N + i], 0), r3 - 1);
    w[q] = wgts[((size_t)b * 8 + q) * N + i];
  }
  const int c0 = blockIdx.y * CT, c1 = min(C, c0 + CT);
  for (int c = c0; c < c1; ++c) {
    const float gv = gy[((size_t)b * C + c) * N + i];
    for (int q = 0; q < 8; ++q) atomicAdd(gx + ((size_t)b * C + c) * r3 + ix[q], mul_rn(w[q], gv));
  }
}

}

constexpr int DVR_G = 8;
constexpr size_t DVR_LDS = (size_t)DVR_RING_BYTES + (size_t)2 * (DVR_R * DVR_R * (DVR_R / DVR_G) / 32) * 4 +
                           (size_t)(DVR_NJ * DVR_NT / (DVR_G / 4)) * 2 + 32 * 4 + 16;
static int devox_ring_depth() {
  static const int d = getenv("LION_DEVOX_RING") ? atoi(getenv("LION_DEVOX_RING")) : 4;
  return d < 2 ? 2 : d;
}

extern "C" {

static int devox_launch(const float *coords, const float *feat, int B, int C, int N, int r,
                        int training, float *out, int32_t *inds, float *wgts, const float *scale,
                        const float *shift, hipStream_t st) {
  const int r2 = r * r;
  if (r == DVR_R && N <= 2048 && (((uintptr_t)feat) & 15) == 0) {
    int CT = 8;
    while (CT > 1 && (long)B * lion_cdiv(C, CT) < 256) CT >>= 1;
    dim3 grid(lion_cdiv(C, CT), B);
    static LionLdsLimit cfgr0 = {}, cfgr1 = {};
    if (scale) {
      if (int e = lion_dynamic_lds(&devox_ring_kernel<true, DVR_G, 0>, DVR_LDS, cfgr1)) return e;
      devox_ring_kernel<true, DVR_G, 0><<<grid, DVR_NT, DVR_LDS, st>>>(coords, feat, C, N, CT, training, out, inds, wgts, scale, shift, devox_ring_depth(), nullptr);
    } else {
      if (int e = lion_dynamic_lds(&devox_ring_kernel<false, DVR_G, 0>, DVR_LDS, cfgr0)) return e;
      devox_ring_kernel<false, DVR_G, 0><<<grid, DVR_NT, DVR_LDS, st>>>(coords, feat, C, N, CT, training, out, inds, wgts, scale, shift, devox_ring_depth(), nullptr);
    }
    LION_LAUNCH_CHECK();
    return 0;
  }
  if ((r2 % 4) == 0 && N <= 2048 && r2 <= 4608 && (((uintptr_t)feat) & 15) == 0) {
    const int planes_max = 9216 / r2;
    const int PX = planes_max >= r ? r : planes_max - 1;
    const int XS = lion_cdiv(r, PX);
    const int CI = XS == 1 ? (9216 / (r2 * r) < 16 ? 9216 / (r2 * r) : 16) : 1;
    const int ld0 = lion_cdiv((XS == 1 ? CI * r2 * r : (PX + 1) * r2) / 4, 256);
    const int ld = ld0 <= 1 ? 1 : ld0 <= 2 ? 2 : ld0 <= 4 ? 4 : 9;
    const int slab_floats = ld * 1024;
    const size_t lds = (size_t)2 * slab_floats * 4 + (size_t)((N + 1) & ~1) * 2 + (size_t)XS * 4 +
                       (size_t)((r2 + 31) / 32) * 4;
    int CT = 4 * CI;
    while (CT > CI && (long)B * lion_cdiv(C, CT) < 512) CT >>= 1;
    dim3 grid(lion_cdiv(C, CT), B);
#define DEVOX_SLAB(LD_)                                                                                    \
  {                                                                                                        \
    static LionLdsLimit cfg0 = {}, cfg1 = {};                                                              \
    if (scale) {                                                                                           \
      if (int e = lion_dynamic_lds(&devox_slab_kernel<LD_, true>, lds, cfg1)) return e;                    \
      devox_slab_kernel<LD_, true><<<grid, 256, lds, st>>>(coords, feat, C, N, r, PX, XS, CT, CI, slab_floats, \
                                                           training, out, inds, wgts, scale, shift);       \
    } else {                                                                                               \
      if (int e = lion_dynamic_lds(&devox_slab_kernel<LD_, false>, lds, cfg0)) return e;                   \
      devox_slab_kernel<LD_, false><<<grid, 256, lds, st>>>(coords, feat, C, N, r, PX, XS, CT, CI, slab_floats, \
                                                            training, out, inds, wgts, scale, shift);      \
    }                                                                                                      \
  }
    if (ld <= 1) DEVOX_SLAB(1)
    else if (ld <= 2) DEVOX_SLAB(2)
    else if (ld <= 4) DEVOX_SLAB(4)
    else DEVOX_SLAB(9)
#undef DEVOX_SLAB
    LION_LAUNCH_CHECK();
    return 0;
  }
  const int pt = lion_cdiv(N, 256);
  int ct = 16;
  while (ct > 2 && (long)B * pt * lion_cdiv(C, ct) < 2048) ct >>= 1;
  dim3 grid(pt, lion_cdiv(C, ct), B);
#define DEVOX_CASE(CT_)                                                                                   \
  if (scale) devox_fwd_kernel<CT_, true><<<grid, 256, 0, st>>>(coords, feat, C, N, r, training, out, inds, wgts, scale, shift); \
  else devox_fwd_kernel<CT_, false><<<grid, 256, 0, st>>>(coords, feat, C, N, r, training, out, inds, wgts, scale, shift)
  switch (ct) {
  case 16: DEVOX_CASE(16); break;
  case 8:  DEVOX_CASE(8); break;
  case 4:  DEVOX_CASE(4); break;
  default: DEVOX_CASE(2); break;
  }
#undef DEVOX_CASE
  LION_LAUNCH_CHECK();
  return 0;
}

int lion_trilinear_devoxelize_forward(const float *coords, const float *feat, int B, int C, int N,
                                      int r, int training, float *out, int32_t *inds, float *wgts,
                                      lionStream_t stream) {
  if (!coords || !feat || !out || B <= 0 || C <= 0 || N <= 0 || r <= 0) return LION_EINVAL;
  if (training && (!inds || !wgts)) return LION_EINVAL;
  return devox_launch(coords, feat, B, C, N, r, training, out, inds, wgts, nullptr, nullptr,
                      static_cast<hipStream_t>(stream));
}

int lion_trilinear_devoxelize_affine_forward(const float *coords, const float *feat, const float *scale,
                                             const float *shift, int B, int C, int N, int r, float *out,
                                             lionStream_t stream) {
  if (!coords || !feat || !out || !scale || !shift || B <= 0 || C <= 0 || N <= 0 || r <= 0) return LION_EINVAL;
  return devox_launch(coords, feat, B, C, N, r, 0, out, nullptr, nullptr, scale, shift,
                      static_cast<hipStream_t>(stream));
}

size_t lion_devoxelize_plan_bytes(int B, int N, int r) {
  if (B <= 0 || N <= 0 || N > 2048 || r != DVR_R) return 0;
  return (size_t)B * devox_plan_stride<DVR_G>();
}

int lion_trilinear_devoxelize_plan(const float *coords, int B, int N, int r, void *plan, size_t plan_bytes,
                                   lionStream_t stream) {
  if (!coords || !plan || B <= 0 || N <= 0) return LION_EINVAL;
  const size_t need = lion_devoxelize_plan_bytes(B, N, r);
  if (!need || (((uintptr_t)plan) & 15) != 0) return LION_EUNSUPPORTED;
  if (plan_bytes < need) return LION_EWORKSPACE;
  static LionLdsLimit cfg = {};
  if (int e = lion_dynamic_lds(&devox_ring_kernel<false, DVR_G, 2>, DVR_LDS, cfg)) return e;
  devox_ring_kernel<false, DVR_G, 2><<<dim3(1, B), DVR_NT, DVR_LDS, static_cast<hipStream_t>(stream)>>>(
      coords, nullptr, 1, N, 1, 0, nullptr, nullptr, nullptr, nullptr, nullptr, devox_ring_depth(),
      static_cast<unsigned char *>(plan));
  LION_LAUNCH_CHECK();
  return 0;
}

int lion_trilinear_devoxelize_planned_forward(const void *plan, size_t plan_bytes, const float *coords, const float *feat,
                                              const float *scale, const float *shift, int B, int C, int N, int r,
                                              float *out, lionStream_t stream) {
  if (!plan || !coords || !feat || !out || B <= 0 || C <= 0 || N <= 0) return LION_EINVAL;
  if ((scale == nullptr) != (shift == nullptr)) return LION_EINVAL;
  const size_t need = lion_devoxelize_plan_bytes(B, N, r);
  if (!need || (((uintptr_t)plan) & 15) != 0 || (((uintptr_t)feat) & 15) != 0) return LION_EUNSUPPORTED;
  if (plan_bytes < need) return LION_EWORKSPACE;
  hipStream_t st = static_cast<hipStream_t>(stream);
  int CT = 8;
  while (CT > 1 && (long)B * lion_cdiv(C, CT) < 256) CT >>= 1;
  dim3 grid(lion_cdiv(C, CT), B);
  unsigned char *pl = const_cast<unsigned char *>(static_cast<const unsigned char *>(plan));
  static LionLdsLimit cfg0 = {}, cfg1 = {};
  if (scale) {
    if (int e = lion_dynamic_lds(&devox_ring_kernel<true, DVR_G, 1>, DVR_LDS, cfg1)) return e;
    devox_ring_kernel<true, DVR_G, 1><<<grid, DVR_NT, DVR_LDS, st>>>(coords, feat, C, N, CT, 0, out, nullptr, nullptr, scale, shift, devox_ring_depth(), pl);
  } else {
    if (int e = lion_dynamic_lds(&devox_ring_kernel<false, DVR_G, 1>, DVR_LDS, cfg0)) return e;
    devox_ring_kernel<false, DVR_G, 1><<<grid, DVR_NT, DVR_LDS, st>>>(coords, feat, C, N, CT, 0, out, nullptr, nullptr, nullptr, nullptr, devox_ring_depth(), pl);
  }
  LION_LAUNCH_CHECK();
  return 0;
}

int lion_trilinear_devoxelize_backward(const float *gy, const int32_t *inds, const float *wgts,
                                       int B, int C, int N, int r3, float *gx,
                                       lionStream_t stream) {
  if (!gy || !inds || !wgts || !gx || B <= 0 || C <= 0 || N <= 0 || r3 <= 0) return LION_EINVAL;
  hipStream_t st = static_cast<hipStream_t>(stream);
  if ((size_t)r3 * 4 <= 128 * 1024 && (r3 % 4) == 0) {
    int parts = (size_t)r3 * 4 > 64 * 1024 ? 2 : 1;
    if (r3 % (4 * parts) != 0) parts = 1;
    const size_t lds = (size_t)(r3 / parts) * 4;
    static LionLdsLimit configured = {};
    if (int e = lion_dynamic_lds(&devox_bwd_lds_kernel, lds, configured)) return e;
    const int nt = r3 >= 16384 ? 1024 : 256;
    devox_bwd_lds_kernel<<<dim3(C, B, parts), nt, lds, st>>>(gy, inds, wgts, C, N, r3, gx);
    LION_LAUNCH_CHECK();
    return 0;
  }
  hipError_t e = hipMemsetAsync(gx, 0, (size_t)B * C * r3 * 4, st);
  if (e != hipSuccess) return (int)e;
  const int CT = 8;
  devox_bwd_atomic_kernel<<<dim3(lion_cdiv(N, 256), lion_cdiv(C, CT), B), 256, 0, st>>>(
      gy, inds, wgts, C, N, r3, CT, gx);
  LION_LAUNCH_CHECK();
  return 0;
}

int lion_trilinear_devoxelize_backward_affine(const float *gy, const int32_t *inds, const float *wgts, const float *x,
                                              const float *Ap, const float *Q, const float *R, int B, int C, int N, int r3,
                                              float *dx, lionStream_t stream) {
  if (!gy || !inds || !wgts || !x || !Ap || !Q || !R || !dx || B <= 0 || C <= 0 || N <= 0 || r3 <= 0) return LION_EINVAL;
  if ((size_t)r3 * 4 > 128 * 1024 || (r3 % 8) != 0 || (((uintptr_t)x | (uintptr_t)dx) & 15) != 0) return LION_EUNSUPPORTED;
  hipStream_t st = static_cast<hipStream_t>(stream);
  const int parts = (size_t)r3 * 4 > 64 * 1024 ? 2 : 1;
  const size_t lds = (size_t)(r3 / parts) * 4;
  static LionLdsLimit configured = {};
  if (int e = lion_dynamic_lds(&devox_bwd_affine_kernel, lds, configured)) return e;
  const int nt = r3 >= 16384 ? 1024 : 256;
// ... 7 lines not shown
```

lion_amd/csrc/pointwise.hip:

```cpp
#include "common.h"

namespace {

__device__ __forceinline__ float swishf(float t) { return swish_fast(t); }

__global__ __launch_bounds__(256) void row_stats_kernel(const float *__restrict__ x, int L,
                                                        float *__restrict__ stats) {
  __shared__ float r1[4], r2[4];
  const int row = blockIdx.x, tid = threadIdx.x, lane = tid & 63, wave = tid >> 6;
  const float *p = x + (size_t)row * L;
  float s1 = 0.f, s2 = 0.f;
  if ((L & 3) == 0) {
    for (int i = tid * 4; i < L; i += 1024) {
      const float4 v = *reinterpret_cast<const float4 *>(p + i);
      s1 += (v.x + v.y) + (v.z + v.w);
      s2 += (v.x * v.x + v.y * v.y) + (v.z * v.z + v.w * v.w);
    }
  } else {
    for (int i = tid; i < L; i += 256) { const float v = p[i]; s1 += v; s2 += v * v; }
  }
  s1 = row16_sum_rn(s1); s2 = row16_sum_rn(s2);
#pragma unroll
  for (int m = 16; m < 64; m <<= 1) { s1 += __shfl_xor(s1, m, 64); s2 += __shfl_xor(s2, m, 64); }
  if (lane == 0) { r1[wave] = s1; r2[wave] = s2; }
  __syncthreads();
  if (tid == 0) {
    stats[(size_t)row * 2] = (r1[0] + r1[1]) + (r1[2] + r1[3]);
    stats[(size_t)row * 2 + 1] = (r2[0] + r2[1]) + (r2[2] + r2[3]);
  }
}

__global__ __launch_bounds__(256) void affine_swish_kernel(const float *__restrict__ x,
                                                           const float *__restrict__ A,
                                                           const float *__restrict__ Bs, int L,
                                                           float *__restrict__ y) {
  const int row = blockIdx.y;
  const float a = A[row], b = Bs[row];
  const float *p = x + (size_t)row * L;
  float *q = y + (size_t)row * L;
  const int i = (blockIdx.x * 256 + threadIdx.x) * 4;
  if (i + 3 < L && (L & 3) == 0) {
    const float4 v = *reinterpret_cast<const float4 *>(p + i);
    *reinterpret_cast<float4 *>(q + i) =
        make_float4(swishf(v.x * a + b), swishf(v.y * a + b), swishf(v.z * a + b), swishf(v.w * a + b));
  } else {
    for (int j = i; j < L && j < i + 4; ++j) q[j] = swishf(p[j] * a + b);
  }
}

__global__ __launch_bounds__(256) void affine_swish_add_kernel(const float *__restrict__ x, const float *__restrict__ A,
                                                               const float *__restrict__ Bs,
                                                               const float *__restrict__ addend, int L,
                                                               float *__restrict__ y) {
  const int row = blockIdx.y;
  const float a = A[row], b = Bs[row];
  const float *p = x + (size_t)row * L, *ad = addend + (size_t)row * L;
  float *q = y + (size_t)row * L;
  const int i = (blockIdx.x * 256 + threadIdx.x) * 4;
  if (i + 3 < L && (L & 3) == 0) {
    const float4 v = *reinterpret_cast<const float4 *>(p + i), w = *reinterpret_cast<const float4 *>(ad + i);
    *reinterpret_cast<float4 *>(q + i) = make_float4(swishf(v.x * a + b) + w.x, swishf(v.y * a + b) + w.y,
                                                     swishf(v.z * a + b) + w.z, swishf(v.w * a + b) + w.w);
  } else {
    for (int j = i; j < L && j < i + 4; ++j) q[j] = swishf(p[j] * a + b) + ad[j];
  }
}

__global__ void timestep_embedding_kernel(const float *__restrict__ t, const float *__restrict__ row, float scale, int B,
                                          int half, int D, float *__restrict__ emb) {
  const int e = blockIdx.x * blockDim.x + threadIdx.x;
  if (e >= B * D) return;
  const int b = e / D, i = e - b * D;
  float v = 0.f;
  if (i < 2 * half) {
    const float ang = mul_rn(mul_rn(t[b], scale), row[i < half ? i : i - half]);
    v = i < half ? sinf(ang) : cosf(ang);
  }
  emb[e] = v;
}

__global__ __launch_bounds__(256) void affine_swish_max_kernel(const float *__restrict__ x,
                                                               const float *__restrict__ A,
                                                               const float *__restrict__ Bs, int M,
                                                               int U, float *__restrict__ y) {
  const int row = blockIdx.y, m = blockIdx.x * 256 + threadIdx.x;
  if (m >= M) return;
  const float a = A[row], b = Bs[row];
  const float *p = x + ((size_t)row * M + m) * U;
  float best = -INFINITY;
  if ((U & 3) == 0) {
    for (int u = 0; u < U; u += 4) {
      const float4 v = *reinterpret_cast<const float4 *>(p + u);
      best = fmaxf(best, fmaxf(fmaxf(swishf(v.x * a + b), swishf(v.y * a + b)),
                               fmaxf(swishf(v.z * a + b), swishf(v.w * a + b))));
    }
  } else {
    for (int u = 0; u < U; ++u) best = fmaxf(best, swishf(p[u] * a + b));
  }
  y[(size_t)row * M + m] = best;
}

template <int LPM>
__global__ __launch_bounds__(256) void affine_swish_max_coop_kernel(const float *__restrict__ x,
                                                                    const float *__restrict__ A,
                                                                    const float *__restrict__ Bs, int M,
                                                                    float *__restrict__ y) {
  constexpr int MPW = 64 / LPM;
  constexpr int IT = 8;
  const int row = blockIdx.y, lane = threadIdx.x & 63, wave = threadIdx.x >> 6;
  const float a = A[row], b = Bs[row];
  const int m0 = (blockIdx.x * 4 + wave) * MPW * IT;
  const float4 *p = reinterpret_cast<const float4 *>(x + (size_t)row * M * (LPM * 4));
  float4 v[IT];
#pragma unroll
  for (int i = 0; i < IT; ++i) {
    const int m = min(m0 + i * MPW + lane / LPM, M - 1);
    v[i] = p[(size_t)m * LPM + (lane % LPM)];
  }
#pragma unroll
  for (int i = 0; i < IT; ++i) {
    float best = fmaxf(fmaxf(swishf(v[i].x * a + b), swishf(v[i].y * a + b)),
                       fmaxf(swishf(v[i].z * a + b), swishf(v[i].w * a + b)));
    if (LPM >= 2) best = fmaxf(best, LION_DPP_F32(best, 0xB1));
    if (LPM >= 4) best = fmaxf(best, LION_DPP_F32(best, 0x4E));
    if (LPM >= 8) best = fmaxf(best, LION_DPP_F32(best, 0x141));
    if (LPM >= 16) best = fmaxf(best, LION_DPP_F32(best, 0x140));
    const int m = m0 + i * MPW + lane / LPM;
    if ((lane % LPM) == 0 && m < M) y[(size_t)row * M + m] = best;
  }
}

__global__ __launch_bounds__(256) void se_gate_kernel(const float *__restrict__ chmean,
                                                      const float *__restrict__ w1,
                                                      const float *__restrict__ w2, int C, int H,
                                                      float *__restrict__ A, float *__restrict__ Bs) {
  __shared__ float sm[1024], sh[128];
  const int b = blockIdx.x, tid = threadIdx.x, lane = tid & 63, wave = tid >> 6;
  for (int c = tid; c < C; c += 256) sm[c] = A[(size_t)b * C + c] * chmean[(size_t)b * C + c] + Bs[(size_t)b * C + c];
  __syncthreads();
  for (int j = wave; j < H; j += 4) {
    float acc = 0.f;
    for (int c = lane; c < C; c += 64) acc += w1[(size_t)j * C + c] * sm[c];
#pragma unroll
    for (int m = 32; m >= 1; m >>= 1) acc += __shfl_xor(acc, m, 64);
    if (lane == 0) sh[j] = acc > 0.f ? acc : 0.f;
  }
  __syncthreads();
  for (int c = tid; c < C; c += 256) {
    float acc = 0.f;
    for (int j = 0; j < H; ++j) acc += w2[(size_t)c * H + j] * sh[j];
    const float g = 1.0f / (1.0f + expf(-acc));
    A[(size_t)b * C + c] *= g;
    Bs[(size_t)b * C + c] *= g;
  }
}


__global__ __launch_bounds__(256) void latent_unpack_kernel(const float *__restrict__ x, int N, int D,
                                                            float *__restrict__ all, float *__restrict__ coords,
                                                            float *__restrict__ rest) {
  __shared__ float tile[256 * 9];
  const int b = blockIdx.y, n0 = blockIdx.x * 256, tid = threadIdx.x;
  const int np = min(256, N - n0);
  const float *src = x + ((size_t)b * N + n0) * D;
  for (int i = tid; i < np * D; i += 256) tile[(i / D) * (D + 1) + i % D] = src[i];
  __syncthreads();
  if (tid >= np) return;
  for (int d = 0; d < D; ++d) {
    const float v = tile[tid * (D + 1) + d];
    if (all) all[((size_t)b * D + d) * N + n0 + tid] = v;
    if (coords && d < 3) coords[((size_t)b * 3 + d) * N + n0 + tid] = v;
    if (rest && d >= 3) rest[((size_t)b * (D - 3) + d - 3) * N + n0 + tid] = v;
  }
}

__global__ __launch_bounds__(256) void concat_broadcast_kernel(const float *__restrict__ a, const float *__restrict__ t,
                                                               int Ca, int Ct, int N4, int ld_t, float4 *__restrict__ out) {
  const int row = blockIdx.y, C = Ca + Ct, b = row / C, c = row % C;
  float4 *o = out + (size_t)row * N4;
  if (c < Ca) {
    const float4 *s = reinterpret_cast<const float4 *>(a) + ((size_t)b * Ca + c) * N4;
    for (int i = blockIdx.x * 256 + threadIdx.x; i < N4; i += gridDim.x * 256) o[i] = s[i];
  } else {
    const float v = t[(size_t)b * ld_t + c - Ca];
    for (int i = blockIdx.x * 256 + threadIdx.x; i < N4; i += gridDim.x * 256) o[i] = make_float4(v, v, v, v);
  }
}

}

extern "C" {

int lion_row_stats(const float *x, int rows, int L, float *stats, lionStream_t stream) {
  if (!x || !stats || rows <= 0 || L <= 0) return LION_EINVAL;
  row_stats_kernel<<<rows, 256, 0, static_cast<hipStream_t>(stream)>>>(x, L, stats);
  LION_LAUNCH_CHECK();
  return 0;
}

int lion_affine_swish(const float *x, const float *A, const float *Bs, int rows, int L, float *y,
                      lionStream_t stream) {
  if (!x || !A || !Bs || !y || rows <= 0 || L <= 0) return LION_EINVAL;
  affine_swish_kernel<<<dim3(lion_cdiv(lion_cdiv(L, 4), 256), rows), 256, 0, static_cast<hipStream_t>(stream)>>>(
      x, A, Bs, L, y);
  LION_LAUNCH_CHECK();
  return 0;
}

int lion_timestep_embedding(const float *t, const float *row, float scale, int B, int half, int D, float *emb,
                            lionStream_t stream) {
  if (!t || !row || !emb || B <= 0 || half <= 0 || D < 2 * half) return LION_EINVAL;
  timestep_embedding_kernel<<<lion_cdiv(B * D, 256), 256, 0, static_cast<hipStream_t>(stream)>>>(t, row, scale, B, half, D, emb);
  LION_LAUNCH_CHECK();
  return 0;
}

int lion_affine_swish_add(const float *x, const float *A, const float *Bs, const float *addend, int rows, int L, float *y,
                          lionStream_t stream) {
  if (!x || !A || !Bs || !addend || !y || rows <= 0 || L <= 0) return LION_EINVAL;
  affine_swish_add_kernel<<<dim3(lion_cdiv(lion_cdiv(L, 4), 256), rows), 256, 0, static_cast<hipStream_t>(stream)>>>(
      x, A, Bs, addend, L, y);
  LION_LAUNCH_CHECK();
  return 0;
}

int lion_affine_swish_max(const float *x, const float *A, const float *Bs, int rows, int M, int U,
                          float *y, lionStream_t stream) {
  if (!x || !A || !Bs || !y || rows <= 0 || M <= 0 || U <= 0) return LION_EINVAL;
  hipStream_t st = static_cast<hipStream_t>(stream);
  const bool al = (((uintptr_t)x) & 15) == 0;
#define LION_ASM_COOP(LPM_)                                                                                  \
  affine_swish_max_coop_kernel<LPM_><<<dim3(lion_cdiv(M, 4 * (64 / LPM_) * 8), rows), 256, 0, st>>>(x, A, Bs, M, y)
  if (al && U == 32) LION_ASM_COOP(8);
  else if (al && U == 16) LION_ASM_COOP(4);
  else if (al && U == 64) LION_ASM_COOP(16);
  else affine_swish_max_kernel<<<dim3(lion_cdiv(M, 256), rows), 256, 0, st>>>(x, A, Bs, M, U, y);
#undef LION_ASM_COOP
  LION_LAUNCH_CHECK();
  return 0;
}

int lion_se_gate(const float *chmean, const float *w1, const float *w2, int B, int C, int H, float *A,
                 float *Bs, lionStream_t stream) {
  if (!chmean || !w1 || !w2 || !A || !Bs || B <= 0 || C <= 0 || H <= 0) return LION_EINVAL;
  if (C > 1024 || H > 128) return LION_EUNSUPPORTED;
  se_gate_kernel<<<B, 256, 0, static_cast<hipStream_t>(stream)>>>(chmean, w1, w2, C, H, A, Bs);
  LION_LAUNCH_CHECK();
  return 0;
}

int lion_latent_unpack(const float *x, int B, int N, int D, float *all, float *coords, float *rest, lionStream_t stream) {
  if (!x || B <= 0 || N <= 0 || D < 3 || D > 8 || (!all && !coords && !rest)) return LION_EINVAL;
  if (rest && D == 3) return LION_EINVAL;
  latent_unpack_kernel<<<dim3(lion_cdiv(N, 256), B), 256, 0, static_cast<hipStream_t>(stream)>>>(x, N, D, all, coords, rest);
  LION_LAUNCH_CHECK();
  return 0;
}

int lion_concat_broadcast(const float *a, const float *t, int B, int Ca, int Ct, int N, int ld_t, float *out,
                          lionStream_t stream) {
  if (!a || !t || !out || B <= 0 || Ca <= 0 || Ct <= 0 || N <= 0 || ld_t < 0) return LION_EINVAL;
  if (N % 4 != 0 || ((((uintptr_t)a) | ((uintptr_t)out)) & 15) != 0) return LION_EUNSUPPORTED;
  if ((long)B * (Ca + Ct) > 65535) return LION_EUNSUPPORTED;
  const int N4 = N / 4;
  concat_broadcast_kernel<<<dim3(lion_cdiv(N4, 256) > 4 ? 4 : lion_cdiv(N4, 256), B * (Ca + Ct)), 256, 0,
                            static_cast<hipStream_t>(stream)>>>(a, t, Ca, Ct, N4, ld_t, reinterpret_cast<float4 *>(out));
  LION_LAUNCH_CHECK();
  return 0;
}

}
```

lion_amd/fused_ops.py:

```python
import os

import torch

from . import _lib
from ._wcache import WeightCache
from . import conv_ops
from .conv_ops import packed_weight, supported


def _border_sums(weight):
    m = torch.tensor([[0., 1., 1.], [1., 1., 1.], [1., 1., 0.]], dtype=torch.float64, device=weight.device)
    ws = torch.einsum("oidhw,ad,bh,cw->abcio", weight.detach().double(), m, m, m)
    return ws.reshape(27, weight.shape[1], weight.shape[0]).float().contiguous()


_WSUM_CACHE = WeightCache(_border_sums)


def border_weight_sums(weight):
    return _WSUM_CACHE.get(weight)


def conv3d_occupancy(counts, r, cout, b, consumer_aware=False):
    lib = _lib.load()
    n = lib.lion_conv3d_occupancy_ints(r, cout, b)
    buf = torch.empty((2, n), device=counts.device, dtype=torch.int32)
    _lib.call("lion_conv3d_tile_occupancy_aware", counts.contiguous(), b, r, cout, buf[0], buf[1], int(consumer_aware))
    return buf[0], buf[1]


class FoldSpec:

    def __init__(self, gn: torch.nn.GroupNorm, fac, gbias, count, se=None):
        self.gn, self.fac, self.gbias, self.count, self.se = gn, fac, gbias, int(count), se

    def apply(self, stats):
        if self.se is not None:
            merged = groupnorm_fold_se(stats, self.gn, self.fac, self.gbias, self.count, self.se)
            if merged is not None:
                return merged
            a, b_, m = groupnorm_fold(stats, self.gn, self.fac, self.gbias, self.count)
            return se_gate_(a, b_, m, self.se)
        a, b_, _ = groupnorm_fold(stats, self.gn, self.fac, self.gbias, self.count)
        return a, b_


def conv3d_fused(x, conv, pro=None, want_stats=True, occ=None, prev_conv=None, split=None, fold=None):
    lib = _lib.load()
    b, cin, r = x.shape[0], x.shape[1], x.shape[2]
    cout = conv.out_channels
    use_split = conv_ops.use_split(split, cin, cout, r)
    if cin % 4:
        assert pro is None
        x = torch.cat([x, x.new_zeros(b, 4 - cin % 4, r, r, r)], dim=1)
        cin = x.shape[1]
    x = x.contiguous()
    wp = conv_ops.split_packed_weight(conv.weight) if use_split else packed_weight(conv.weight)
    y = torch.empty((b, cout, r, r, r), device=x.device, dtype=torch.float32)
    pa = pb = pbias = tconst = None
    if pro is not None:
        pa, pb = pro[0].contiguous(), pro[1].contiguous()
    bias = conv.bias.detach().contiguous() if conv.bias is not None else None
    sparse = occ is not None and r >= 16
    if sparse and pro is not None:
        if prev_conv is None or cin > 256:
            sparse = False
        else:
            ws = border_weight_sums(conv.weight)
            pbias = prev_conv.bias.detach().contiguous() if prev_conv.bias is not None else None
            tconst = torch.empty((b, 27, cout), device=x.device, dtype=torch.float32)
            _lib.call("lion_conv3d_const_response", ws, bias, pbias, pa, pb, b, cin, cout, tconst)
    stats = None
    if want_stats:
        tiles = lib.lion_conv3d_split_stat_tiles(r, cout) if use_split else lib.lion_conv3d_stat_tiles(r, cout, b, int(sparse))
        stats = torch.empty((b, cout, tiles, 2), device=x.device, dtype=torch.float32)
    if not sparse:
        occ = None
    entry = "lion_conv3d_k3_fused_forward"
    if use_split:
        entry = "lion_conv3d_k3_half_forward" if conv_ops.use_half(cin, cout, r, x) else "lion_conv3d_k3_split_forward"
    _lib.call(entry, x, wp, bias, b, cin, cout, r, pa, pb, pbias, tconst, y, stats, occ)
    if fold is not None:
        return y, fold.apply(stats)
    return y, stats


def groupnorm_fold(stats, gn: torch.nn.GroupNorm, fac, gbias, voxels):
    b, c, t, _ = stats.shape
    A = torch.empty((b, c), device=stats.device, dtype=torch.float32)
    Bs = torch.empty_like(A)
    cm = torch.empty_like(A)
    if not (fac.stride(1) == 1 and gbias.stride(1) == 1 and fac.stride(0) == gbias.stride(0) and fac.stride(0) >= c):
        fac, gbias = fac.contiguous(), gbias.contiguous()
    _lib.call("lion_groupnorm_fold", stats, b, c, t, gn.num_groups, int(voxels), gn.weight, gn.bias, fac, gbias,
              int(fac.stride(0)), float(gn.eps), A, Bs, cm)
    return A, Bs, cm


def groupnorm_fold_se(stats, gn: torch.nn.GroupNorm, fac, gbias, voxels, se):
    b, c, t, _ = stats.shape
    w1, w2 = se.fc[0].weight.detach(), se.fc[2].weight.detach()
    h = w1.shape[0]
    if c > 256 or c < 4 or h > 128 or not (w1.is_contiguous() and w2.is_contiguous()):
        return None
    A = torch.empty((b, c), device=stats.device, dtype=torch.float32)
    Bs = torch.empty_like(A)
    if not (fac.stride(1) == 1 and gbias.stride(1) == 1 and fac.stride(0) == gbias.stride(0) and fac.stride(0) >= c):
        fac, gbias = fac.contiguous(), gbias.contiguous()
    _lib.call("lion_groupnorm_fold_se", stats, b, c, t, gn.num_groups, int(voxels), gn.weight, gn.bias, fac, gbias,
              int(fac.stride(0)), float(gn.eps), w1, w2, h, A, Bs)
    return A, Bs


def se_gate_(A, Bs, chmean, se):
    w1, w2 = se.fc[0].weight.detach(), se.fc[2].weight.detach()
    h, c = w1.shape
    if c > 1024 or h > 128 or not (w1.is_contiguous() and w2.is_contiguous()):
        gate = se.fc(A * chmean + Bs)
        return A * gate, Bs * gate
    _lib.call("lion_se_gate", chmean, w1, w2, A.shape[0], c, h, A, Bs)
    return A, Bs


def devoxelize_plan(coords, r):
    lib = _lib.load()
    b, _, n = coords.shape
    nbytes = lib.lion_devoxelize_plan_bytes(b, n, int(r))
    if nbytes == 0 or not coords.is_contiguous() or coords.dtype != torch.float32:
        return None
    buf = torch.empty((nbytes,), device=coords.device, dtype=torch.uint8)
    _lib.call("lion_trilinear_devoxelize_plan", coords, b, n, int(r), buf, nbytes)
    return {"buf": buf, "coords": coords, "shape": (b, n, int(r))}


def devoxelize_affine(grid, coords, r, scale, shift, plan=None):
    b, c = grid.shape[:2]
    n = coords.shape[2]
    out = torch.empty((b, c, n), device=grid.device, dtype=torch.float32)
    co_c, gr_c, sc_c, sh_c = coords.contiguous(), grid.contiguous(), scale.contiguous(), shift.contiguous()
    if plan is not None and plan["shape"] == (b, n, int(r)) and plan["coords"].data_ptr() == co_c.data_ptr():
        buf = plan["buf"]
        _lib.call("lion_trilinear_devoxelize_planned_forward", buf, buf.numel(), co_c, gr_c, sc_c, sh_c, b, c, n, int(r), out)
        return out
    _lib.call("lion_trilinear_devoxelize_affine_forward", co_c, gr_c, sc_c, sh_c, b, c, n, int(r), out)
    return out


def fusable(conv1, conv2, r, x):
    return (x.is_cuda and x.dtype == torch.float32 and not torch.is_autocast_enabled()
            and supported(conv1.in_channels, conv1.out_channels, r)
            and supported(conv2.in_channels, conv2.out_channels, r)
            and conv2.in_channels % 4 == 0 and conv2.in_channels <= 256)


def _pw_pack(weight):
    return conv_ops.pack_with(weight, "lion_pwconv_packed_floats", "lion_pwconv_pack_weights", torch.float32, as_matrix=True)


_PW_CACHE = WeightCache(_pw_pack)
PW_ALL = os.environ.get("LION_PW_ALL", "1") != "0"


def pw_packed_weight(weight):
    return _PW_CACHE.get(weight)


def _pw_split_pack(weight):
    return conv_ops.pack_with(weight, "lion_pwconv_split_packed_halfs", "lion_pwconv_split_pack_weights", torch.int16,
                              as_matrix=True)


_PW_SPLIT_CACHE = WeightCache(_pw_split_pack)
PW_SPLIT = os.environ.get("LION_PW_SPLIT", "1") != "0"


def pw_use_split(split, b, cin, cout, L):
    can = cin * L < (1 << 29) and cin <= 4096
    if split is None:
        return PW_SPLIT and can and b * L >= 8192 and (L <= 4096 or cin * cout >= 8192)
    return bool(split) and can


def pw_supported(conv, x):
    if not PW_ALL:
        L = x[0, 0].numel()
        if not (conv.out_channels in (32, 64, 128, 256) and L >= 1024 and x.shape[0] * L * conv.out_channels >= (1 << 22)):
            return False
    return (conv.groups == 1 and all(k == 1 for k in conv.kernel_size) and all(s == 1 for s in conv.stride)
            and all(p == 0 for p in conv.padding) and x.is_cuda and x.dtype == torch.float32 and x[0, 0].numel() > 0
            and _lib.load().lion_pwconv_stat_tiles(conv.out_channels, conv.in_channels, x[0, 0].numel()) > 0)


def pwconv_fused(x, conv, pro=None, want_stats=True, split=None):
    lib = _lib.load()
    x = x.contiguous()
    b, cin = x.shape[:2]
    L = x[0, 0].numel()
    cout = conv.out_channels
    use_split = pw_use_split(split, b, cin, cout, L)
    wp = _PW_SPLIT_CACHE.get(conv.weight) if use_split else pw_packed_weight(conv.weight)
    y = torch.empty((b, cout) + tuple(x.shape[2:]), device=x.device, dtype=torch.float32)
    tiles = (lib.lion_pwconv_split_stat_tiles if use_split else lib.lion_pwconv_stat_tiles)(cout, cin, L)
    stats = torch.empty((b, cout, tiles, 2), device=x.device, dtype=torch.float32) if want_stats else None
    pa = pb = None
    if pro is not None:
        pa, pb = pro[0].contiguous(), pro[1].contiguous()
    bias = conv.bias.detach().contiguous() if conv.bias is not None else None
    _lib.call("lion_pwconv_split_forward" if use_split else "lion_pwconv_forward",
              x, wp, bias, b, cin, cout, L, pa, pb, y, stats)
    return y, stats


MAX_RECOMPUTE = os.environ.get("LION_PW_MAX_RECOMPUTE", "0") != "0"


def pwconv_max_recompute(x, conv, gn, style, pro):
    lib = _lib.load()
    x = x.contiguous()
    b, cin, m, u = x.shape
    L = m * u
    cout = conv.out_channels
# ... 31 lines not shown
        _lib.call("lion_pwconv_split_pack_weights_t", w2d.detach().contiguous(), cin, cout, wf, wp)
    elif transposed:
        wp = (_pw_split_pack if use_split else _pw_pack)(w2d.detach().t().contiguous())
    elif cached_param is not None:
        wp = _PW_SPLIT_CACHE.get(cached_param) if use_split else _PW_CACHE.get(cached_param)
    else:
        wp = (_pw_split_pack if use_split else _pw_pack)(w2d)
    y = torch.empty((b, cout) + tuple(x.shape[2:]), device=x.device, dtype=torch.float32)
    bias_c = bias.detach().contiguous() if bias is not None else None
    _lib.call("lion_pwconv_split_forward" if use_split else "lion_pwconv_forward",
              x, wp, bias_c, b, cin, cout, L, None, None, y, None)
    return y


def pwconv_wgrad(x, gy, want_bias=False):
    lib = _lib.load()
    x, gy = x.contiguous(), gy.contiguous()
    b, cin = x.shape[:2]
    cout = gy.shape[1]
    L = x[0, 0].numel()
    wsb = lib.lion_pwconv_wgrad_workspace_bytes(b, cin, cout, L)
    ws = torch.empty((wsb,), device=x.device, dtype=torch.uint8)
    gw = torch.empty((cout, cin), device=x.device, dtype=torch.float32)
    gb = torch.empty((cout,), device=x.device, dtype=torch.float32) if want_bias else None
    _lib.call("lion_pwconv_wgrad", x, gy, b, cin, cout, L, ws, wsb, gw, gb)
    return (gw, gb) if want_bias else gw


def group_points(coords, centers, feat, idx):
    b, _, n = coords.shape
    m, u = idx.shape[1], idx.shape[2]
    c = 0 if feat is None else feat.shape[1]
    out = torch.empty((b, 3 + c, m, u), device=coords.device, dtype=torch.float32)
    _lib.call("lion_group_points_forward", coords.contiguous(), centers.contiguous(), None if feat is None else feat.contiguous(),
              idx.contiguous(), b, c, n, m, u, out)
    return out


def linear_rows(x, weight, bias=None, act=0, slope=0.0):
    x = x.contiguous()
    b, k = x.shape
    o = weight.shape[0]
    wp = pw_packed_weight(weight)
    y = torch.empty((b, o), device=x.device, dtype=torch.float32)
    bias_c = bias.detach().contiguous() if bias is not None else None
    _lib.call("lion_linear_forward", x, wp, bias_c, b, k, o, int(act), float(slope), y)
    return y


def linear_attention_core(qkv, heads, dim_head):
    qkv = qkv.contiguous()
    b, n = qkv.shape[0], qkv[0, 0].numel()
    out = torch.empty((b, heads * dim_head) + tuple(qkv.shape[2:]), device=qkv.device, dtype=torch.float32)
    _lib.call("lion_linear_attention_core", qkv, b, heads, dim_head, n, out)
    return out


def row_stats(x):
    x = x.contiguous()
    rows = x.shape[0] * x.shape[1]
    stats = torch.empty((rows, 2), device=x.device, dtype=torch.float32)
    _lib.call("lion_row_stats", x, rows, x[0, 0].numel(), stats)
    return stats


def affine_swish(x, A, Bs, reduce_max=False, add=None):
    b, c = x.shape[:2]
    if add is not None and not reduce_max:
        add = add.contiguous()
        assert add.shape == x.shape and add.dtype == torch.float32
        y = torch.empty_like(x)
        _lib.call("lion_affine_swish_add", x, A, Bs, add, b * c, x[0, 0].numel(), y)
        return y
    if reduce_max:
        m, u = x.shape[2], x.shape[3]
        y = torch.empty((b, c, m), device=x.device, dtype=torch.float32)
        _lib.call("lion_affine_swish_max", x, A, Bs, b * c, m, u, y)
        return y
    y = torch.empty_like(x)
    _lib.call("lion_affine_swish", x, A, Bs, b * c, x[0, 0].numel(), y)
    return y


def shared_mlp(x, convs, adagns, style, reduce_max=False, add=None):
    pro = None
    for li, (conv, gn) in enumerate(zip(convs, adagns)):
        if (MAX_RECOMPUTE and reduce_max and add is None and li == len(convs) - 1 and x.dim() == 4 and x.shape[3] == 32
                and pw_supported(conv, x)
                and not pw_use_split(None, x.shape[0], x.shape[1], conv.out_channels, x[0, 0].numel())):
            out = pwconv_max_recompute(x, conv, gn, style, pro)
            if out is not None:
                return out
        if pw_supported(conv, x):
            x, st = pwconv_fused(x, conv, pro)
        else:
            if pro is not None:
                x = affine_swish(x, pro[0], pro[1])
            x = conv(x).contiguous()
            st = row_stats(x).view(x.shape[0], x.shape[1], 1, 2)
        f, g = gn.affine(style)
        A, Bs, _ = groupnorm_fold(st, gn.norm, f, g, x[0, 0].numel())
        pro = (A, Bs)
    out = affine_swish(x, pro[0], pro[1], reduce_max, add=None if reduce_max else add)
    return out + add if (add is not None and reduce_max) else out


def adagn_swish(x, adagn, style, reduce_max=False):
    x = x.contiguous()
    stats = row_stats(x).view(x.shape[0], x.shape[1], 1, 2)
    f, g = adagn.affine(style)
    A, Bs, _ = groupnorm_fold(stats, adagn.norm, f, g, x[0, 0].numel())
    return affine_swish(x, A, Bs, reduce_max)



def broadcast_rows(temb):
    if temb is None or temb.dim() != 3 or temb.stride(2) != 0 or temb.stride(1) != 1 or temb.dtype != torch.float32:
        return None
    rows = temb[:, :, 0]
    return rows, int(rows.stride(0))


def latent_unpack(x, n_points, d, want_all=True, want_coords=True, want_rest=True):
    b = x.shape[0]
    mk = lambda c, want: torch.empty((b, c, n_points), device=x.device, dtype=torch.float32) if want and c > 0 else None
    al, co, re = mk(d, want_all), mk(3, want_coords), mk(d - 3, want_rest)
    _lib.call("lion_latent_unpack", x.contiguous(), b, n_points, d, al, co, re)
    return al, co, re


def concat_broadcast(a, temb):
    br = broadcast_rows(temb)
    if br is None or a.dim() != 3 or a.dtype != torch.float32 or a.shape[2] % 4 or not a.is_contiguous() \
            or temb.shape[0] != a.shape[0] or temb.shape[2] != a.shape[2]:
        return None
    rows, ld = br
    b, ca, n = a.shape
    ct = rows.shape[1]
    out = torch.empty((b, ca + ct, n), device=a.device, dtype=torch.float32)
    return out if _lib.call("lion_concat_broadcast", a, rows, b, ca, ct, n, ld, out, unsupported_ok=True) else None


def three_nn_interpolate_cat(points, centers, cfeat, temb, skip):
    rows, ld, c2 = None, 0, 0
    if temb is not None:
        br = broadcast_rows(temb)
        if br is None or temb.shape[0] != cfeat.shape[0]:
            return None
        rows, ld = br
        c2 = rows.shape[1]
    if cfeat.dtype != torch.float32 or (skip is not None and skip.dtype != torch.float32):
        return None
    from .functional import backend as _bk
    fn = getattr(_bk._backend, "three_nearest_neighbors_interpolate_cat_forward", None)
    if fn is None:
        return None
    points, centers, cfeat = points[:, :3].contiguous(), centers[:, :3].contiguous(), cfeat.contiguous()
    skip = None if skip is None else skip.contiguous()
    return fn(points, centers, cfeat, rows, ld, skip)[0]



def _rows2d(x):
    b, c = x.shape[0], x.shape[1]
    v = x.reshape(b, c) if x.dim() != 2 else x
    if not (v.is_cuda and v.dtype == torch.float32 and (c == 1 or v.stride(1) == 1)):
        return None
    return v, (0 if b == 1 else int(v.stride(0)))


def to_channel_major_pair(x, t):
    rx, rt = _rows2d(x), _rows2d(t)
    if rx is None or rt is None or torch.is_grad_enabled():
        if t.shape[0] == 1 and x.shape[0] > 1:
            t = t.expand(x.shape[0], *t.shape[1:])
        return to_channel_major(x), to_channel_major(t)
    (vx, ldx), (vt, ldt) = rx, rt
    b = x.shape[0]
    nb = (b + 31) // 32
    ox = torch.empty((nb, vx.shape[1], 32), device=x.device, dtype=torch.float32)
    ot = torch.empty((nb, vt.shape[1], 32), device=x.device, dtype=torch.float32)
    _lib.call("lion_to_channel_major", vx, ldx, vx.shape[1], ox, vt, ldt, vt.shape[1], ot, b)
    return ox, ot
# ... 63 lines not shown
```

lion_amd/models/pvcnn2_ada.py:

```python
import contextlib
import functools
import os

import torch
import torch.nn as nn
from einops import rearrange

from .. import functional as F
from ..conv_ops import conv3d_module
from .. import fused_ops

FUSE_INFERENCE = True
SPARSE_CONV1 = True
OVERLAP_POINT_BRANCH = os.environ.get("LION_OVERLAP_POINT_BRANCH", "0") != "0"
_POINT_STREAMS = {}


_VOX_PLANS = None
VOX_PLAN = os.environ.get("LION_VOX_PLAN", "1") != "0"
OCC_PLAN = os.environ.get("LION_OCC_PLAN", "1") != "0"
SKIP_UNREAD = os.environ.get("LION_CONV_SKIP_UNREAD", "1") != "0"
SKIP_UNREAD_LEVEL2 = os.environ.get("LION_CONV_SKIP_UNREAD_LEVEL2", "1") != "0"
OCC_CLONE = os.environ.get("LION_OCC_CLONE", "0") != "0"
DEVOX_PLAN = os.environ.get("LION_DEVOX_PLAN", "1") != "0"


@contextlib.contextmanager
def voxel_plans():
    global _VOX_PLANS
    prev, _VOX_PLANS = _VOX_PLANS, ({} if VOX_PLAN else None)
    try:
        yield
    finally:
        _VOX_PLANS = prev


def _occupancy(counts, r, cout, b, level=None):
    if level is None:
        level = 1 if SKIP_UNREAD else 0
    if _VOX_PLANS is None or not OCC_PLAN:
        return fused_ops.conv3d_occupancy(counts, r, cout, b, consumer_aware=level)
    key = ("occ", counts.data_ptr(), tuple(counts.shape), int(r), int(b), int(level))
    hit = _VOX_PLANS.get(key)
    if hit is None:
        o1, o2 = fused_ops.conv3d_occupancy(counts, r, cout, b, consumer_aware=level)
        hit = (counts, (o1, o2))
        _VOX_PLANS[key] = hit
    if OCC_CLONE:
        return hit[1][0].clone(), hit[1][1].clone()
    return hit[1]


def _devox_plan(voxel_coords, r):
    if _VOX_PLANS is None or not DEVOX_PLAN or r != 32 or voxel_coords.shape[2] > 2048 or not voxel_coords.is_contiguous():
        return None
    key = ("devox", voxel_coords.data_ptr(), tuple(voxel_coords.shape), int(r))
    hit = _VOX_PLANS.get(key)
    if hit is None:
        plan = fused_ops.devoxelize_plan(voxel_coords, r)
        hit = (voxel_coords, plan)
        _VOX_PLANS[key] = hit
    return hit[1]


def _point_stream(device):
    key = (device.type, device.index)
    if key not in _POINT_STREAMS:
        _POINT_STREAMS[key] = torch.cuda.Stream(device=device)
    return _POINT_STREAMS[key]
from .adagn import AdaGN


class SE3d(nn.Module):

    def __init__(self, channel, reduction=8):
        super().__init__()
        self.fc = nn.Sequential(
            nn.Linear(channel, channel // reduction, bias=False),
            nn.ReLU(inplace=True),
            nn.Linear(channel // reduction, channel, bias=False),
            nn.Sigmoid())
        self.channel = channel

    def __repr__(self):
        return f"SE({self.channel}, {self.channel})"

    def gate(self, inputs):
        return self.fc(inputs.mean(-1).mean(-1).mean(-1))

    def forward(self, inputs):
        return inputs * self.gate(inputs).view(inputs.shape[0], inputs.shape[1], 1, 1, 1)


class LinearAttention(nn.Module):

    def __init__(self, dim, heads=4, dim_head=32, verbose=True):
        super().__init__()
        self.heads = heads
        hidden_dim = dim_head * heads
        self.to_qkv = nn.Conv2d(dim, hidden_dim * 3, 1, bias=False)
        self.to_out = nn.Conv2d(hidden_dim, dim, 1)

    def forward(self, x):
        if own_kernels(x) and self.to_qkv.out_channels == 3 * self.heads * 32 and fused_ops.pw_supported(self.to_qkv, x):
            qkv = fused_ops.pwconv_fused(x, self.to_qkv, None, want_stats=False)[0]
            core = fused_ops.linear_attention_core(qkv, self.heads, 32)
            return fused_ops.pwconv_fused(core, self.to_out, None, want_stats=False)[0]
# ... 68 lines not shown
    if own_kernels(x) and fused_ops.pw_supported(conv, x):
        if x[0, 0].numel() == 1:
            y = fused_ops.linear_rows(x.reshape(x.shape[0], x.shape[1]), conv.weight.flatten(1), conv.bias)
            return y.reshape(x.shape[0], conv.out_channels, *x.shape[2:])
        return fused_ops.pwconv_fused(x, conv, None, want_stats=False)[0]
    from .. import train_ops
    if train_ops.pwconv_trainable(conv, x):
        return train_ops.pwconv(conv, x)
    from .. import _fallback
    if (x.is_cuda and torch.is_grad_enabled() and all(k == 1 for k in conv.kernel_size) and all(s == 1 for s in conv.stride)
            and all(p == 0 for p in conv.padding) and conv.groups == 1):
        _fallback.note("pvcnn2_ada.conv1x1 (training matmul)", f"{tuple(conv.weight.shape)} on {tuple(x.shape)}")
        y = torch.matmul(conv.weight.flatten(1), x.flatten(2))
        if conv.bias is not None:
            y = y + conv.bias[:, None]
        return y.reshape(x.shape[0], conv.out_channels, *x.shape[2:])
    _fallback.note("pvcnn2_ada.conv1x1 (library conv)", f"{tuple(conv.weight.shape)} on {tuple(x.shape)} {x.dtype} {x.device.type}")
    return type(conv).forward(conv, x)


def route_1x1_convs(module):
    for m in module.modules():
        if (isinstance(m, (nn.Conv1d, nn.Conv2d)) and all(k == 1 for k in m.kernel_size) and m.groups == 1
                and all(s == 1 for s in m.stride) and all(p == 0 for p in m.padding)
                and "forward" not in m.__dict__):
            m.forward = functools.partial(conv1x1, m)
    return module


def run_layers(layers, x, style, conv, reduce_max=False):
    from .. import train_ops
    i, n = 0, len(layers)
    while i < n:
        layer = layers[i]
        if isinstance(layer, AdaGN):
            if train_ops.usable(x) and layer.n_channel <= 1024:
                fused_act = i + 1 < n and isinstance(layers[i + 1], Swish)
                factor, bias = layer.affine(style)
                if (not fused_act and i + 1 < n and isinstance(layers[i + 1], SE3d) and x.dim() == 5
                        and train_ops.se3d_trainable(layers[i + 1], x)):
                    x = train_ops.adagn_se(x, layer.norm, factor, bias, layers[i + 1])
                    i += 2
                    continue
                if reduce_max and i + (2 if fused_act else 1) == n and train_ops.adagn_act_max_usable(x):
                    return train_ops.adagn_act_max(x, layer.norm, factor, bias, act=fused_act)
                i += 2 if fused_act else 1
                drop_p, used = train_ops.fusable_dropout(layers, i) if fused_act else (0.0, 0)
                x = train_ops.adagn_act(x, layer.norm, factor, bias, act=fused_act, dropout_p=drop_p)
                i += used
                continue
            x = layer(x, style)
        elif isinstance(layer, (nn.Conv1d, nn.Conv2d, nn.Conv3d)):
            x = conv(layer, x)
        elif isinstance(layer, SE3d) and train_ops.se3d_trainable(layer, x):
            x = train_ops.se3d(layer, x)
        else:
            x = layer(x)
        i += 1
    return x.max(dim=-1).values if reduce_max else x


class SharedMLP(nn.Module):

    def __init__(self, in_channels, out_channels, dim=1, cfg={}):
        assert len(cfg) > 0, cfg
        super().__init__()
        conv = nn.Conv1d if dim == 1 else nn.Conv2d
        if not isinstance(out_channels, (list, tuple)):
            out_channels = [out_channels]
        layers = []
        for oc in out_channels:
            layers += [conv(in_channels, oc, 1), AdaGN(dim, cfg, oc), Swish()]
            in_channels = oc
        self.layers = nn.ModuleList(layers)

    def _fusable(self, x):
        return (FUSE_INFERENCE and not self.training and not torch.is_grad_enabled() and x.is_cuda
                and x.dtype == torch.float32 and not torch.is_autocast_enabled())

    def _run(self, x, style, reduce_max=False, add=None):
        if self._fusable(x):
            n = len(self.layers) // 3
            convs, gns = [self.layers[3 * i] for i in range(n)], [self.layers[3 * i + 1] for i in range(n)]
            return fused_ops.shared_mlp(x, convs, gns, style, reduce_max, add=add)
        x = run_layers(list(self.layers), x, style, conv1x1, reduce_max=reduce_max)
        return x if add is None else x + add

    def forward_max(self, x, style):
        return self._run(x, style, reduce_max=True)

    def forward(self, *inputs):
        if len(inputs) == 1 and len(inputs[0]) == 4:
            inputs = inputs[0]
        if len(inputs) == 4:
            x, _, _, style = inputs
            return (self._run(x, style), *inputs[1:])
        if len(inputs) == 2:
            return self._run(*inputs)
        raise NotImplementedError


class Voxelization(nn.Module):

    def __init__(self, resolution, normalize=True, eps=0):
        super().__init__()
        self.r = int(resolution)
        self.normalize = normalize
        self.eps = eps

    def forward(self, features, coords, return_counts=False, sparse_reader=False):
        coords = coords.detach()
        if return_counts:
            from ..functional.backend import _backend
            b, c = features.shape[:2]
            co = coords[:, :3].float().contiguous()
            plan = None
            if _VOX_PLANS is not None and hasattr(_backend, "voxel_index"):
                key = (co.data_ptr(), tuple(co.shape), self.r, bool(self.normalize), float(self.eps))
                hit = _VOX_PLANS.get(key)
                if hit is None:
                    plan = _backend.voxel_index(co, self.r, self.normalize, self.eps)
                    if plan is not None:
                        _VOX_PLANS[key] = (co, plan)
                else:
                    plan = hit[1]
            if plan is not None:
                occ_m1 = None
                if sparse_reader and SKIP_UNREAD and SPARSE_CONV1 and self.r in (16, 32) and hasattr(_backend, "voxel_scatter"):
                    occ_m1 = _occupancy(plan["cnt"], self.r, 64, b, int(sparse_reader))[0]
                out = _backend.voxel_scatter(features.float().contiguous(), plan, occ_m1)
                return out.view(b, c, self.r, self.r, self.r), plan["norm"], plan["cnt"]
            out, norm_coords, _, counts = _backend.voxelize_points_forward(
                features.float().contiguous(), co, self.r, self.normalize, self.eps)
            return out.view(b, c, self.r, self.r, self.r), norm_coords, counts
        if features is None:
            from ..functional.backend import _backend
            _, norm_coords, _, _ = _backend.voxelize_points_forward(
                None, coords[:, :3].float().contiguous(), self.r, self.normalize, self.eps)
            return features, norm_coords
        return F.voxelize_points(features, coords, self.r, self.normalize, self.eps)

    def extra_repr(self):
        return 'resolution={}{}'.format(
            self.r, ', normalized eps = {}'.format(self.eps) if self.normalize else '')


class PVConv(nn.Module):

    def __init__(self, in_channels, out_channels, kernel_size, resolution, normalize=1, eps=0,
                 with_se=False, add_point_feat=True, attention=False, dropout=0.1, verbose=True,
                 cfg={}):
        super().__init__()
        assert len(cfg) > 0, cfg
        self.resolution = resolution
        self.voxelization = Voxelization(resolution, normalize=normalize, eps=eps)
        norm = functools.partial(AdaGN, 3, cfg)
        voxel_layers = [
            nn.Conv3d(in_channels, out_channels, kernel_size, stride=1, padding=kernel_size // 2),
            norm(out_channels),
            Swish(),
            nn.Dropout(dropout),
            nn.Conv3d(out_channels, out_channels, kernel_size, stride=1, padding=kernel_size // 2),
            norm(out_channels),
        ]
        if with_se:
            voxel_layers.append(SE3d(out_channels))
        self.voxel_layers = nn.ModuleList(voxel_layers)
        self.attn = LinearAttention(out_channels, verbose=verbose) if attention else None
        if add_point_feat:
            self.point_features = SharedMLP(in_channels, out_channels, cfg=cfg)
        self.add_point_feat = add_point_feat

    def _aware_level(self):
        if not SKIP_UNREAD:
            return 0
        from .. import conv_ops
        conv2 = self.voxel_layers[4]
        return 2 if (SKIP_UNREAD_LEVEL2 and conv_ops.use_split(None, conv2.in_channels, conv2.out_channels, self.resolution)) else 1

    def _fused_voxel_branch(self, grid, voxel_coords, style, counts=None):
        conv1, gn1, conv2, gn2 = self.voxel_layers[0], self.voxel_layers[1], self.voxel_layers[4], self.voxel_layers[5]
        se = self.voxel_layers[6] if len(self.voxel_layers) > 6 else None
        r = self.resolution
        occ1 = occ2 = None
        if SPARSE_CONV1 and counts is not None and r >= 16:
            occ1, occ2 = _occupancy(counts, r, conv1.out_channels, grid.shape[0], self._aware_level())
        f1, g1 = gn1.affine(style)
        y1, (a1, b1) = fused_ops.conv3d_fused(grid, conv1, None, True, occ1,
                                              fold=fused_ops.FoldSpec(gn1.norm, f1, g1, r ** 3))
        f2, g2 = gn2.affine(style)
        y2, (a2, b2) = fused_ops.conv3d_fused(y1, conv2, (a1, b1), True, occ2, prev_conv=conv1,
                                              fold=fused_ops.FoldSpec(gn2.norm, f2, g2, r ** 3, se))
        return fused_ops.devoxelize_affine(y2, voxel_coords, r, a2, b2, plan=_devox_plan(voxel_coords, r))

    def forward(self, inputs):
        features, coords_input, time_emb, style = inputs
        coords = coords_input[:, :3] if coords_input.shape[1] > 3 else coords_input
        assert features.shape[0] == coords.shape[0] and features.shape[2] == coords.shape[2], \
            f'get feat: {features.shape} and {coords.shape}'
        assert coords.shape[1] == 3, f'expect coords: B,3,Npoint, get: {coords.shape}'
        counts = None
        if (FUSE_INFERENCE and not self.training and not torch.is_grad_enabled() and features.is_cuda
                and not torch.is_autocast_enabled()):
            will_fuse = fused_ops.fusable(self.voxel_layers[0], self.voxel_layers[4], self.resolution, features.float())
            grid, voxel_coords, counts = self.voxelization(features, coords, return_counts=True,
                                                           sparse_reader=self._aware_level() if will_fuse else 0)
        else:
            grid, voxel_coords = self.voxelization(features, coords)
        if (FUSE_INFERENCE and not self.training and not torch.is_grad_enabled()
                and fused_ops.fusable(self.voxel_layers[0], self.voxel_layers[4], self.resolution, grid)):
            pf = None
            if self.add_point_feat and OVERLAP_POINT_BRANCH:
                main, side = torch.cuda.current_stream(features.device), _point_stream(features.device)
                side.wait_stream(main)
                with torch.cuda.stream(side):
                    pf = self.point_features(features, style)
            fused = self._fused_voxel_branch(grid, voxel_coords, style, counts)
            if pf is not None:
                main.wait_stream(side)
                pf.record_stream(main)
                fused = fused + pf
            elif self.add_point_feat:
                fused = self.point_features._run(features, style, add=fused)
            if self.attn is not None:
                fused = self.attn(fused)
            return fused, coords_input, time_emb, style
        layers = list(self.voxel_layers)
        from .. import train_ops
        if (self.training and len(layers) >= 2 and isinstance(layers[-1], SE3d) and isinstance(layers[-2], AdaGN)
                and train_ops.usable(grid) and layers[-2].n_channel <= 1024 and train_ops.adagn_se_devox_usable(grid, layers[-1])):
            grid = run_layers(layers[:-2], grid, style, conv3d_module)
            factor, bias = layers[-2].affine(style)
            fused = train_ops.adagn_se_devox(grid, layers[-2].norm, factor, bias, layers[-1], voxel_coords, self.resolution)
        else:
            grid = run_layers(layers, grid, style, conv3d_module)
            fused = F.trilinear_devoxelize(grid, voxel_coords, self.resolution, self.training)
        if self.add_point_feat:
            fused = fused + self.point_features(features, style)
        if self.attn is not None:
            fused = self.attn(fused)
        return fused, coords_input, time_emb, style


class PointNetAModule(nn.Module):

    def __init__(self, in_channels, out_channels, include_coordinates=True, cfg={}):
        super().__init__()
        if not isinstance(out_channels, (list, tuple)):
            out_channels = [[out_channels]]
        elif not isinstance(out_channels[0], (list, tuple)):
            out_channels = [out_channels]
        mlps, total = [], 0
        for oc in out_channels:
            mlps.append(SharedMLP(in_channels + (3 if include_coordinates else 0), oc, dim=1, cfg=cfg))
            total += oc[-1]
        self.include_coordinates = include_coordinates
        self.out_channels = total
        self.mlps = nn.ModuleList(mlps)

    def forward(self, inputs):
        features, coords, time_emb, style = inputs
        if self.include_coordinates:
            features = torch.cat([features, coords], dim=1)
        coords = torch.zeros((coords.size(0), 3, 1), device=coords.device)
        pooled = [mlp(features, style).max(dim=-1, keepdim=True).values for mlp in self.mlps]
        return (torch.cat(pooled, dim=1) if len(pooled) > 1 else pooled[0]), coords, time_emb

    def extra_repr(self):
        return f'out_channels={self.out_channels}, include_coordinates={self.include_coordinates}'


class PointNetSAModule(nn.Module):

    def __init__(self, num_centers, radius, num_neighbors, in_channels, out_channels,
                 include_coordinates=True, cfg={}):
        super().__init__()
# ... 173 lines not shown
```

Before: 5.390.

## Defer GroupNorm fold into consumer kernels to cut small launches

GroupNorm statistics are no longer reduced to per-channel scale/shift in a standalone kernel. The reduction now runs inside whichever kernel consumes it: the const-response kernel for the next conv3d, the devoxelize slab kernel (with the SE gate) and the final affine-swish-add of the shared MLP. The fold code moves into a shared header so all consumers use the same logic. This removes several tiny kernel launches per block in each diffusion step, at the cost of repeating the fold work per consumer block and adding fallback paths for unsupported shapes.

```diff
diff --git a/include/lion_hip.h b/include/lion_hip.h
--- a/include/lion_hip.h
+++ b/include/lion_hip.h
@@ -137,6 +137,10 @@
 size_t lion_conv3d_occupancy_ints(int r, int Cout, int B);
 int lion_conv3d_const_response(const float *wsum, const float *bias2, const float *bias1, const float *pro_a,
                                const float *pro_b, int B, int Cin, int Cout, float *tconst, lionStream_t stream);
+int lion_conv3d_fold_const_response(const float *stats, int B, int Cin, int T, int G, int voxels, const float *gamma,
+                                    const float *beta, const float *fac, const float *gbias, int ld_fg, float eps,
+                                    const float *wsum, const float *bias2, const float *bias1, int Cout, float *A1,
+                                    float *Bs1, float *tconst, lionStream_t stream);
 int lion_conv3d_tile_occupancy(const int32_t *cnt, int B, int r, int Cout, int32_t *occ_m1, int32_t *occ_m2,
                                lionStream_t stream);
 int lion_conv3d_tile_occupancy_aware(const int32_t *cnt, int B, int r, int Cout, int32_t *occ_m1, int32_t *occ_m2,
@@ -209,6 +213,14 @@
                             lionStream_t stream);
 int lion_affine_swish_add(const float *x, const float *A, const float *Bs, const float *addend, int rows, int L, float *y,
                           lionStream_t stream);
+
+int lion_trilinear_devoxelize_fold_se_forward(const float *coords, const float *feat, const float *stats, int T, int G,
+                                              int voxels, const float *gamma, const float *beta, const float *fac,
+                                              const float *gbias, int ld_fg, float eps, const float *w1, const float *w2,
+                                              int H, int B, int C, int N, int r, float *out, lionStream_t stream);
+int lion_fold_affine_swish_add(const float *stats, int B, int C, int T, int G, int count, const float *gamma,
+                               const float *beta, const float *fac, const float *gbias, int ld_fg, float eps,
+                               const float *x, const float *addend, int L, float *y, lionStream_t stream);
 
 size_t lion_scatter_csr_workspace_bytes(int B, int E, int bins);
 int lion_scatter_csr(const float *gy, const int32_t *idx, const float *w, int B, int C, int S, int E, int bins, void *ws,
diff --git a/lion_amd/_lib.py b/lion_amd/_lib.py
--- a/lion_amd/_lib.py
+++ b/lion_amd/_lib.py
@@ -50,6 +50,8 @@
     "lion_conv3d_stat_tiles": (_i, [_i, _i, _i, _i]),
     "lion_conv3d_k3_fused_forward": (_i, [_vp, _vp, _vp, _i, _i, _i, _i, _vp, _vp, _vp, _vp, _vp, _vp, _vp, _vp]),
     "lion_conv3d_const_response": (_i, [_vp, _vp, _vp, _vp, _vp, _i, _i, _i, _vp, _vp]),
+    "lion_conv3d_fold_const_response": (_i, [_vp, _i, _i, _i, _i, _i, _vp, _vp, _vp, _vp, _i, _f, _vp, _vp, _vp, _i, _vp, _vp,
+                                             _vp, _vp]),
     "lion_conv3d_occupancy_ints": (_sz, [_i, _i, _i]),
     "lion_conv3d_tile_occupancy": (_i, [_vp, _i, _i, _i, _vp, _vp, _vp]),
     "lion_conv3d_tile_occupancy_aware": (_i, [_vp, _i, _i, _i, _vp, _vp, _i, _vp]),
@@ -70,6 +72,8 @@
     "lion_from_channel_major": (_i, [_vp, _i, _i, _vp, _vp]),
     "lion_se_gate": (_i, [_vp, _vp, _vp, _i, _i, _i, _vp, _vp, _vp]),
     "lion_trilinear_devoxelize_affine_forward": (_i, [_vp, _vp, _vp, _vp, _i, _i, _i, _i, _vp, _vp]),
+    "lion_trilinear_devoxelize_fold_se_forward": (_i, [_vp, _vp, _vp, _i, _i, _i, _vp, _vp, _vp, _vp, _i, _f, _vp, _vp, _i, _i, _i,
+                                                       _i, _i, _vp, _vp]),
     "lion_devoxelize_plan_bytes": (_sz, [_i, _i, _i]),
     "lion_trilinear_devoxelize_plan": (_i, [_vp, _i, _i, _i, _vp, _sz, _vp]),
     "lion_trilinear_devoxelize_planned_forward": (_i, [_vp, _sz, _vp, _vp, _vp, _vp, _i, _i, _i, _i, _vp, _vp]),
@@ -91,6 +95,7 @@
     "lion_affine_swish_max": (_i, [_vp, _vp, _vp, _i, _i, _i, _vp, _vp]),
     "lion_timestep_embedding": (_i, [_vp, _vp, _f, _i, _i, _i, _vp, _vp]),
     "lion_affine_swish_add": (_i, [_vp, _vp, _vp, _vp, _i, _i, _vp, _vp]),
+    "lion_fold_affine_swish_add": (_i, [_vp, _i, _i, _i, _i, _i, _vp, _vp, _vp, _vp, _i, _f, _vp, _vp, _i, _vp, _vp]),
     "lion_scatter_csr_workspace_bytes": (_sz, [_i, _i, _i]),
     "lion_scatter_csr": (_i, [_vp, _vp, _vp, _i, _i, _i, _i, _i, _vp, _sz, _vp, _vp]),
     "lion_pwconv_wgrad_workspace_bytes": (_sz, [_i, _i, _i, _i]),
diff --git a/lion_amd/chain.py b/lion_amd/chain.py
--- a/lion_amd/chain.py
+++ b/lion_amd/chain.py
@@ -17,7 +17,8 @@
     from .models import pvcnn2_ada
     return (pvcnn2_ada.SPARSE_CONV1, pvcnn2_ada.FUSE_INFERENCE, pvcnn2_ada.OVERLAP_POINT_BRANCH, geometry.ENABLED,
             geometry.SPLIT_GRAPH, conv_ops.SPLIT, fused_ops.PW_SPLIT, pvcnn2_ada.VOX_PLAN, TEMB_TABLE, fused_ops.MAX_RECOMPUTE,
-            pvcnn2_ada.SKIP_UNREAD, pvcnn2_ada.SKIP_UNREAD_LEVEL2, CHANNEL_MAJOR_EPS, conv_ops.PRECISION)
+            pvcnn2_ada.SKIP_UNREAD, pvcnn2_ada.SKIP_UNREAD_LEVEL2, CHANNEL_MAJOR_EPS, conv_ops.PRECISION,
+            pvcnn2_ada.FOLD_AT_CONSUMER, fused_ops.FOLD_MAX_TILES)
 
 
 def channel_major(model, shape) -> bool:
diff --git a/lion_amd/csrc/conv3d.hip b/lion_amd/csrc/conv3d.hip
--- a/lion_amd/csrc/conv3d.hip
+++ b/lion_amd/csrc/conv3d.hip
@@ -1,4 +1,5 @@
 #include "common.h"
+#include "gn_fold.h"
 
 namespace {
 
@@ -252,51 +253,14 @@
                                const float *__restrict__ gamma, const float *__restrict__ beta,
                                const float *__restrict__ fac, const float *__restrict__ gbias, int ld_fg, float eps,
                                float *__restrict__ A, float *__restrict__ Bs, float *__restrict__ chmean) {
-  __shared__ double cs[64][2];
-  __shared__ double gs[2];
-  const int b = blockIdx.y, g = blockIdx.x, cpg = C / G, tid = threadIdx.x;
-  int cp2 = 1;
-  while (cp2 < cpg) cp2 <<= 1;
-  const int LPC = 256 / cp2, ch = tid / LPC, sub = tid % LPC;
-  double s1 = 0.0, s2 = 0.0;
-  if (ch < cpg) {
-    const float2 *p = reinterpret_cast<const float2 *>(stats + (((size_t)b * C + g * cpg + ch) * T) * 2);
-    for (int t = sub; t < T; t += LPC) { const float2 v = p[t]; s1 += (double)v.x; s2 += (double)v.y; }
-  }
-  for (int m = 1; m < LPC && m < 64; m <<= 1) { s1 += __shfl_xor(s1, m, 64); s2 += __shfl_xor(s2, m, 64); }
-  if (LPC > 64) {
-    __shared__ double ws[4][2];
-    if ((tid & 63) == 0) { ws[tid >> 6][0] = s1; ws[tid >> 6][1] = s2; }
-    __syncthreads();
-    if (sub == 0) {
-      s1 = 0.0; s2 = 0.0;
-      for (int w = 0; w < LPC / 64; ++w) { s1 += ws[(tid >> 6) + w][0]; s2 += ws[(tid >> 6) + w][1]; }
-    }
-  }
-  if (ch < cpg && sub == 0) {
-    cs[ch][0] = s1;
-    cs[ch][1] = s2;
-    chmean[(size_t)b * C + g * cpg + ch] = (float)(s1 / count);
-  }
-  __syncthreads();
-  if (tid == 0) {
-    double g1 = 0.0, g2 = 0.0;
-    for (int c = 0; c < cpg; ++c) { g1 += cs[c][0]; g2 += cs[c][1]; }
-    gs[0] = g1;
-    gs[1] = g2;
-  }
-  __syncthreads();
-  if (tid < cpg) {
-    const double n = (double)count * cpg;
-    const double mean = gs[0] / n;
-    double var = gs[1] / n - mean * mean;
-    var = var > 0.0 ? var : 0.0;
-    const float rstd = (float)(1.0 / sqrt(var + (double)eps));
-    const int c = g * cpg + tid;
-    const float f = fac[(size_t)b * ld_fg + c], gb = gbias[(size_t)b * ld_fg + c];
-    const float a0 = rstd * gamma[c];
-    A[(size_t)b * C + c] = a0 * f;
-    Bs[(size_t)b * C + c] = (beta[c] - (float)mean * a0) * f + gb;
+  __shared__ lion_fold::Lds lds;
+  const int b = blockIdx.y, g = blockIdx.x, tid = threadIdx.x;
+  const lion_fold::Args f = {stats, C, T, G, count, gamma, beta, fac, gbias, ld_fg, eps};
+  float a, bs;
+  if (lion_fold::fold_groups<1>(f, b, g, 1, tid, lds, chmean, a, bs)) {
+    const int c = g * (C / G) + tid;
+    A[(size_t)b * C + c] = a;
+    Bs[(size_t)b * C + c] = bs;
   }
 }
 
@@ -306,50 +270,13 @@
                                                          int ld_fg, float eps, const float *__restrict__ w1,
                                                          const float *__restrict__ w2, int H, float *__restrict__ A,
                                                          float *__restrict__ Bs) {
-  __shared__ double cs[256][2];
-  __shared__ float sA[256], sB[256], sm[256], sh[128];
-  const int b = blockIdx.x, tid = threadIdx.x, lane = tid & 63, wave = tid >> 6, cpg = C / G;
-  int cp2 = 1;
-  while (cp2 < C) cp2 <<= 1;
-  const int LPC = 256 / cp2, ch = tid / LPC, sub = tid % LPC;
-  double s1 = 0.0, s2 = 0.0;
-  if (ch < C) {
-    const float2 *p = reinterpret_cast<const float2 *>(stats + (((size_t)b * C + ch) * T) * 2);
-    for (int t = sub; t < T; t += LPC) { const float2 v = p[t]; s1 += (double)v.x; s2 += (double)v.y; }
-  }
-  for (int m = 1; m < LPC; m <<= 1) { s1 += __shfl_xor(s1, m, 64); s2 += __shfl_xor(s2, m, 64); }
-  if (ch < C && sub == 0) { cs[ch][0] = s1; cs[ch][1] = s2; }
-  __syncthreads();
-  if (tid < C) {
-    const int g0 = (tid / cpg) * cpg;
-    double g1 = 0.0, g2 = 0.0;
-    for (int k = 0; k < cpg; ++k) { g1 += cs[g0 + k][0]; g2 += cs[g0 + k][1]; }
-    const double n = (double)count * cpg, mean = g1 / n;
-    double var = g2 / n - mean * mean;
-    var = var > 0.0 ? var : 0.0;
-    const float rstd = (float)(1.0 / sqrt(var + (double)eps));
-    const float f = fac[(size_t)b * ld_fg + tid], gb = gbias[(size_t)b * ld_fg + tid];
-    const float a0 = rstd * gamma[tid];
-    const float a = a0 * f, bb = (beta[tid] - (float)mean * a0) * f + gb;
-    sA[tid] = a;
-    sB[tid] = bb;
-    sm[tid] = a * (float)(cs[tid][0] / count) + bb;
-  }
-  __syncthreads();
-  for (int j = wave; j < H; j += 4) {
-    float acc = 0.f;
-    for (int c = lane; c < C; c += 64) acc += w1[(size_t)j * C + c] * sm[c];
-#pragma unroll
-    for (int m = 32; m >= 1; m >>= 1) acc += __shfl_xor(acc, m, 64);
-    if (lane == 0) sh[j] = acc > 0.f ? acc : 0.f;
-  }
-  __syncthreads();
-  if (tid < C) {
-    float acc = 0.f;
-    for (int j = 0; j < H; ++j) acc += w2[(size_t)tid * H + j] * sh[j];
-    const float g = 1.0f / (1.0f + expf(-acc));
-    A[(size_t)b * C + tid] = sA[tid] * g;
-    Bs[(size_t)b * C + tid] = sB[tid] * g;
+  __shared__ lion_fold::SeLds lds;
+  const int b = blockIdx.x, tid = threadIdx.x;
+  const lion_fold::Args f = {stats, C, T, G, count, gamma, beta, fac, gbias, ld_fg, eps};
+  float a, bs;
+  if (lion_fold::fold_se(f, b, w1, w2, H, tid, lds, a, bs)) {
+    A[(size_t)b * C + tid] = a;
+    Bs[(size_t)b * C + tid] = bs;
   }
 }
 
@@ -437,6 +364,52 @@
   }
 }
 
+__global__ __launch_bounds__(256) void conv_fold_tconst_kernel(lion_fold::Args f, const float *__restrict__ wsum,
+                                                               const float *__restrict__ bias2,
+                                                               const float *__restrict__ bias1, int Cout,
+                                                               float *__restrict__ A1, float *__restrict__ Bs1,
+                                                               float *__restrict__ tconst) {
+  __shared__ float sc[256];
+  __shared__ lion_fold::Lds lds;
+  const int cfg = blockIdx.x, b = blockIdx.y, tid = threadIdx.x, Cin = f.C;
+  constexpr int WB = 16;
+  float w0[WB];
+  const bool pre = tid < Cout && Cin >= WB;
+  if (pre) {
+    const float *w = wsum + (size_t)cfg * Cin * Cout + tid;
+#pragma unroll
+    for (int k = 0; k < WB; ++k) w0[k] = w[(size_t)k * Cout];
+  }
+  float a, bs;
+  if (lion_fold::fold_groups<lion_fold::UNROLL>(f, b, 0, f.G, tid, lds, nullptr, a, bs)) {
+    sc[tid] = pro_act(bias1 ? bias1[tid] : 0.f, a, bs);
+    if (cfg == 0) {
+      A1[(size_t)b * Cin + tid] = a;
+      Bs1[(size_t)b * Cin + tid] = bs;
+    }
+  }
+  __syncthreads();
+  for (int co = tid; co < Cout; co += 256) {
+    double acc = bias2 ? (double)bias2[co] : 0.0;
+    const float *w = wsum + (size_t)cfg * Cin * Cout + co;
+    int c = 0;
+    if (pre && co == tid) {
+#pragma unroll
+      for (int k = 0; k < WB; ++k) acc += (double)w0[k] * (double)sc[k];
+      c = WB;
+    }
+    for (; c + WB <= Cin; c += WB) {
+      float wv[WB];
+#pragma unroll
+      for (int k = 0; k < WB; ++k) wv[k] = w[(size_t)(c + k) * Cout];
+#pragma unroll
+      for (int k = 0; k < WB; ++k) acc += (double)wv[k] * (double)sc[c + k];
+    }
+    for (; c < Cin; ++c) acc += (double)w[(size_t)c * Cout] * (double)sc[c];
+    tconst[((size_t)b * 27 + cfg) * Cout + co] = (float)acc;
+  }
+}
+
 __global__ void conv3d_pack_kernel(const float *__restrict__ w, int Cout, int Cin, int Cin_pad,
                                    float *__restrict__ wp) {
   const int i = blockIdx.x * blockDim.x + threadIdx.x;
@@ -572,6 +545,20 @@
   return 0;
 }
 
+int lion_conv3d_fold_const_response(const float *stats, int B, int Cin, int T, int G, int voxels, const float *gamma,
+                                    const float *beta, const float *fac, const float *gbias, int ld_fg, float eps,
+                                    const float *wsum, const float *bias2, const float *bias1, int Cout, float *A1,
+                                    float *Bs1, float *tconst, lionStream_t stream) {
+  if (!stats || !gamma || !beta || !fac || !gbias || !wsum || !A1 || !Bs1 || !tconst) return LION_EINVAL;
+  if (B <= 0 || Cin <= 0 || Cout <= 0 || T <= 0 || G <= 0 || Cin % G != 0 || Cin / G > 64 || ld_fg < Cin) return LION_EINVAL;
+  if (Cin > lion_fold::MAX_C || G > lion_fold::MAX_G || B > 65535) return LION_EUNSUPPORTED;
+  const lion_fold::Args f = {stats, Cin, T, G, (float)voxels, gamma, beta, fac, gbias, ld_fg, eps};
+  conv_fold_tconst_kernel<<<dim3(27, B), 256, 0, static_cast<hipStream_t>(stream)>>>(f, wsum, bias2, bias1, Cout, A1, Bs1,
+                                                                                      tconst);
+  LION_LAUNCH_CHECK();
+  return 0;
+}
+
 size_t lion_conv3d_occupancy_ints(int r, int Cout, int B) {
   if (r != 16 && r != 32) return 0;
   return (size_t)2 * B * conv_plan(r, Cout, B, true).tiles + 4;
diff --git a/lion_amd/csrc/devoxelize.hip b/lion_amd/csrc/devoxelize.hip
--- a/lion_amd/csrc/devoxelize.hip
+++ b/lion_amd/csrc/devoxelize.hip
@@ -1,4 +1,5 @@
 #include "common.h"
+#include "gn_fold.h"
 
 namespace {
 
@@ -83,13 +84,20 @@
 }
 
 
-template <int LD, bool AFF>
+struct DevoxFold {
+  lion_fold::Args f;
+  const float *w1, *w2;
+  int H;
+};
+template <int LD, bool AFF, bool FOLD = false>
 __global__ __launch_bounds__(256) void devox_slab_kernel(
     const float *__restrict__ coords, const float *__restrict__ feat, int C, int N, int r, int PX,
     int XS, int CT, int CI, int slab_floats, int training, float *__restrict__ out,
     int32_t *__restrict__ inds, float *__restrict__ wgts, const float *__restrict__ scale,
-    const float *__restrict__ shift) {
+    const float *__restrict__ shift, DevoxFold fold) {
+  static_assert(!FOLD || AFF, "the head fold feeds the affine form");
   extern __shared__ __attribute__((aligned(16))) unsigned char smem[];
+  __shared__ float s_aff[FOLD ? 128 : 1];
   float *lds = reinterpret_cast<float *>(smem);
   constexpr int PP = 8;
   const int tid = threadIdx.x, b = blockIdx.y, c0 = blockIdx.x * CT;
@@ -148,6 +156,14 @@
   }
   __syncthreads();
   issue(0);
+  if (FOLD) {
+    lion_fold::SeLds &fl = *reinterpret_cast<lion_fold::SeLds *>(lds + slab_floats);
+    float fa, fb;
+    if (lion_fold::fold_se(fold.f, b, fold.w1, fold.w2, fold.H, tid, fl, fa, fb) && tid >= c0 && tid < c0 + nch) {
+      s_aff[tid - c0] = fa;
+      s_aff[64 + tid - c0] = fb;
+    }
+  }
 
   for (int s2 = tid; s2 < XS; s2 += 256) scnt[s2] = 0;
   __syncthreads();
@@ -241,7 +257,8 @@
           a = add_rn(a, mul_rn(w5, v5));
           a = add_rn(a, mul_rn(w6, v6));
           a = add_rn(a, mul_rn(w7, v7));
-          if (AFF) a = a * scale[(size_t)b * C + cg + ci] + shift[(size_t)b * C + cg + ci] * wsum;
+          if (FOLD) a = a * s_aff[g * CI + ci] + s_aff[64 + g * CI + ci] * wsum;
+          else if (AFF) a = a * scale[(size_t)b * C + cg + ci] + shift[(size_t)b * C + cg + ci] * wsum;
           o[(size_t)ci * N + pid[p]] = a;
         }
       } else if (xsl[p] == -2 && xs == 0) {
@@ -620,9 +637,10 @@
 
 static int devox_launch(const float *coords, const float *feat, int B, int C, int N, int r,
                         int training, float *out, int32_t *inds, float *wgts, const float *scale,
-                        const float *shift, hipStream_t st) {
+                        const float *shift, hipStream_t st, const DevoxFold *hf = nullptr) {
   const int r2 = r * r;
-  if (r == DVR_R && N <= 2048 && (((uintptr_t)feat) & 15) == 0) {
+  const DevoxFold fold = hf ? *hf : DevoxFold{};
+  if (!hf && r == DVR_R && N <= 2048 && (((uintptr_t)feat) & 15) == 0) {
     int CT = 8;
     while (CT > 1 && (long)B * lion_cdiv(C, CT) < 256) CT >>= 1;
     dim3 grid(lion_cdiv(C, CT), B);
@@ -650,17 +668,22 @@
     int CT = 4 * CI;
     while (CT > CI && (long)B * lion_cdiv(C, CT) < 512) CT >>= 1;
     dim3 grid(lion_cdiv(C, CT), B);
+    if (hf && (CT > 64 || (size_t)slab_floats * 4 < sizeof(lion_fold::SeLds))) return LION_EUNSUPPORTED;
 #define DEVOX_SLAB(LD_)                                                                                    \
   {                                                                                                        \
-    static LionLdsLimit cfg0 = {}, cfg1 = {};                                                              \
-    if (scale) {                                                                                           \
+    static LionLdsLimit cfg0 = {}, cfg1 = {}, cfg2 = {};                                                   \
+    if (hf) {                                                                                              \
+      if (int e = lion_dynamic_lds(&devox_slab_kernel<LD_, true, true>, lds, cfg2)) return e;              \
+      devox_slab_kernel<LD_, true, true><<<grid, 256, lds, st>>>(coords, feat, C, N, r, PX, XS, CT, CI, slab_floats, \
+                                                                 training, out, inds, wgts, scale, shift, fold); \
+    } else if (scale) {                                                                                    \
       if (int e = lion_dynamic_lds(&devox_slab_kernel<LD_, true>, lds, cfg1)) return e;                    \
       devox_slab_kernel<LD_, true><<<grid, 256, lds, st>>>(coords, feat, C, N, r, PX, XS, CT, CI, slab_floats, \
-                                                           training, out, inds, wgts, scale, shift);       \
+                                                           training, out, inds, wgts, scale, shift, fold); \
     } else {                                                                                               \
       if (int e = lion_dynamic_lds(&devox_slab_kernel<LD_, false>, lds, cfg0)) return e;                   \
       devox_slab_kernel<LD_, false><<<grid, 256, lds, st>>>(coords, feat, C, N, r, PX, XS, CT, CI, slab_floats, \
-                                                            training, out, inds, wgts, scale, shift);      \
+                                                            training, out, inds, wgts, scale, shift, fold); \
     }                                                                                                      \
   }
     if (ld <= 1) DEVOX_SLAB(1)
@@ -671,6 +694,7 @@
     LION_LAUNCH_CHECK();
     return 0;
   }
+  if (hf) return LION_EUNSUPPORTED;
   const int pt = lion_cdiv(N, 256);
   int ct = 16;
   while (ct > 2 && (long)B * pt * lion_cdiv(C, ct) < 2048) ct >>= 1;
@@ -704,6 +728,18 @@
   if (!coords || !feat || !out || !scale || !shift || B <= 0 || C <= 0 || N <= 0 || r <= 0) return LION_EINVAL;
   return devox_launch(coords, feat, B, C, N, r, 0, out, nullptr, nullptr, scale, shift,
                       static_cast<hipStream_t>(stream));
+}
+
+int lion_trilinear_devoxelize_fold_se_forward(const float *coords, const float *feat, const float *stats, int T, int G,
+                                              int voxels, const float *gamma, const float *beta, const float *fac,
+                                              const float *gbias, int ld_fg, float eps, const float *w1, const float *w2,
+                                              int H, int B, int C, int N, int r, float *out, lionStream_t stream) {
+  if (!coords || !feat || !out || !stats || !gamma || !beta || !fac || !gbias || !w1 || !w2) return LION_EINVAL;
+  if (B <= 0 || C <= 0 || N <= 0 || r <= 0 || T <= 0 || G <= 0 || C % G != 0 || ld_fg < C || H <= 0) return LION_EINVAL;
+  if (C > 256 || C < 4 || H > 128 || r >= DVR_R) return LION_EUNSUPPORTED;
+  const DevoxFold hf = {{stats, C, T, G, (float)voxels, gamma, beta, fac, gbias, ld_fg, eps}, w1, w2, H};
+  return devox_launch(coords, feat, B, C, N, r, 0, out, nullptr, nullptr, nullptr, nullptr,
+                      static_cast<hipStream_t>(stream), &hf);
 }
 
 size_t lion_devoxelize_plan_bytes(int B, int N, int r) {
diff --git a/lion_amd/csrc/gn_fold.h b/lion_amd/csrc/gn_fold.h
--- /dev/null
+++ b/lion_amd/csrc/gn_fold.h
@@ -0,0 +1,162 @@
+#pragma once
+#include "common.h"
+
+namespace lion_fold {
+
+struct Args {
+  const float *stats;
+  int C, T, G;
+  float count;
+  const float *gamma, *beta, *fac, *gbias;
+  int ld_fg;
+  float eps;
+};
+
+constexpr int MAX_C = 256, MAX_G = 32, UNROLL = 8;
+
+struct Lds {
+  double cs[MAX_C][2];
+  double gs[MAX_G][2];
+  double ws[UNROLL][4][2];
+};
+
+template <int U>
+__device__ __forceinline__ bool fold_groups(const Args &f, int b, int g_first, int ng, int tid, Lds &s,
+                                            float *__restrict__ chmean, float &a_out, float &b_out) {
+  static_assert(U >= 1 && U <= UNROLL, "ws holds UNROLL groups");
+  const int cpg = f.C / f.G;
+  int cp2 = 1;
+  while (cp2 < cpg) cp2 <<= 1;
+  const int LPC = 256 / cp2, ch = tid / LPC, sub = tid % LPC;
+  const bool on = tid < 256;
+  for (int g0 = 0; g0 < ng; g0 += U) {
+    double s1[U], s2[U];
+#pragma unroll
+    for (int u = 0; u < U; ++u) { s1[u] = 0.0; s2[u] = 0.0; }
+    if (on && ch < cpg) {
+      const float2 *p = reinterpret_cast<const float2 *>(f.stats + (((size_t)b * f.C + (size_t)(g_first + g0) * cpg + ch) * f.T) * 2);
+      const size_t gstride = (size_t)cpg * f.T;
+      for (int t = sub; t < f.T; t += LPC) {
+        float2 v[U];
+#pragma unroll
+        for (int u = 0; u < U; ++u) v[u] = g0 + u < ng ? p[u * gstride + t] : make_float2(0.f, 0.f);
+#pragma unroll
+        for (int u = 0; u < U; ++u) { s1[u] += (double)v[u].x; s2[u] += (double)v[u].y; }
+      }
+    }
+    if (on) {
+      for (int m = 1; m < LPC && m < 64; m <<= 1) {
+#pragma unroll
+        for (int u = 0; u < U; ++u) { s1[u] += __shfl_xor(s1[u], m, 64); s2[u] += __shfl_xor(s2[u], m, 64); }
+      }
+    }
+    if (LPC > 64) {
+      if (on && (tid & 63) == 0) {
+#pragma unroll
+        for (int u = 0; u < U; ++u) { s.ws[u][tid >> 6][0] = s1[u]; s.ws[u][tid >> 6][1] = s2[u]; }
+      }
+      __syncthreads();
+      if (on && sub == 0) {
+#pragma unroll
+        for (int u = 0; u < U; ++u) {
+          s1[u] = 0.0; s2[u] = 0.0;
+          for (int w = 0; w < LPC / 64; ++w) { s1[u] += s.ws[u][(tid >> 6) + w][0]; s2[u] += s.ws[u][(tid >> 6) + w][1]; }
+        }
+      }
+    }
+    if (on && ch < cpg && sub == 0) {
+#pragma unroll
+      for (int u = 0; u < U; ++u)
+        if (g0 + u < ng) {
+          s.cs[(g0 + u) * cpg + ch][0] = s1[u];
+          s.cs[(g0 + u) * cpg + ch][1] = s2[u];
+          if (chmean) chmean[(size_t)b * f.C + (size_t)(g_first + g0 + u) * cpg + ch] = (float)(s1[u] / f.count);
+        }
+    }
+    if (LPC > 64 && g0 + U < ng) __syncthreads();
+  }
+  __syncthreads();
+  if (on && tid < ng) {
+    double g1 = 0.0, g2 = 0.0;
+    for (int c = 0; c < cpg; ++c) { g1 += s.cs[tid * cpg + c][0]; g2 += s.cs[tid * cpg + c][1]; }
+    s.gs[tid][0] = g1;
+    s.gs[tid][1] = g2;
+  }
+  __syncthreads();
+  const bool mine = on && tid < ng * cpg;
+  if (mine) {
+    const int gl = tid / cpg;
+    const double n = (double)f.count * cpg;
+    const double mean = s.gs[gl][0] / n;
+    double var = s.gs[gl][1] / n - mean * mean;
+    var = var > 0.0 ? var : 0.0;
+    const float rstd = (float)(1.0 / sqrt(var + (double)f.eps));
+    const int c = g_first * cpg + tid;
+    const float fc = f.fac[(size_t)b * f.ld_fg + c], gb = f.gbias[(size_t)b * f.ld_fg + c];
+    const float a0 = rstd * f.gamma[c];
+    a_out = a0 * fc;
+    b_out = (f.beta[c] - (float)mean * a0) * fc + gb;
+  }
+  return mine;
+}
+
+struct SeLds {
+  double cs[256][2];
+  float sA[256], sB[256], sm[256], sh[128];
+};
+
+__device__ __forceinline__ bool fold_se(const Args &f, int b, const float *__restrict__ w1, const float *__restrict__ w2,
+                                        int H, int tid, SeLds &s, float &a_out, float &b_out) {
+  const int C = f.C, T = f.T, lane = tid & 63, wave = tid >> 6, cpg = C / f.G;
+  const bool on = tid < 256;
+  int cp2 = 1;
+  while (cp2 < C) cp2 <<= 1;
+  const int LPC = 256 / cp2, ch = tid / LPC, sub = tid % LPC;
+  double s1 = 0.0, s2 = 0.0;
+  if (on && ch < C) {
+    const float2 *p = reinterpret_cast<const float2 *>(f.stats + (((size_t)b * C + ch) * T) * 2);
+    for (int t = sub; t < T; t += LPC) { const float2 v = p[t]; s1 += (double)v.x; s2 += (double)v.y; }
+  }
+  if (on) {
+    for (int m = 1; m < LPC; m <<= 1) { s1 += __shfl_xor(s1, m, 64); s2 += __shfl_xor(s2, m, 64); }
+    if (ch < C && sub == 0) { s.cs[ch][0] = s1; s.cs[ch][1] = s2; }
+  }
+  __syncthreads();
+  if (on && tid < C) {
+    const int g0 = (tid / cpg) * cpg;
+    double g1 = 0.0, g2 = 0.0;
+    for (int k = 0; k < cpg; ++k) { g1 += s.cs[g0 + k][0]; g2 += s.cs[g0 + k][1]; }
+    const double n = (double)f.count * cpg, mean = g1 / n;
+    double var = g2 / n - mean * mean;
+    var = var > 0.0 ? var : 0.0;
+    const float rstd = (float)(1.0 / sqrt(var + (double)f.eps));
+    const float fc = f.fac[(size_t)b * f.ld_fg + tid], gb = f.gbias[(size_t)b * f.ld_fg + tid];
+    const float a0 = rstd * f.gamma[tid];
+    const float a = a0 * fc, bb = (f.beta[tid] - (float)mean * a0) * fc + gb;
+    s.sA[tid] = a;
+    s.sB[tid] = bb;
+    s.sm[tid] = a * (float)(s.cs[tid][0] / f.count) + bb;
+  }
+  __syncthreads();
+  if (on) {
+    for (int j = wave; j < H; j += 4) {
+      float acc = 0.f;
+      for (int c = lane; c < C; c += 64) acc += w1[(size_t)j * C + c] * s.sm[c];
+#pragma unroll
+      for (int m = 32; m >= 1; m >>= 1) acc += __shfl_xor(acc, m, 64);
+      if (lane == 0) s.sh[j] = acc > 0.f ? acc : 0.f;
+    }
+  }
+  __syncthreads();
+  const bool mine = on && tid < C;
+  if (mine) {
+    float acc = 0.f;
+    for (int j = 0; j < H; ++j) acc += w2[(size_t)tid * H + j] * s.sh[j];
+    const float g = 1.0f / (1.0f + expf(-acc));
+    a_out = s.sA[tid] * g;
+    b_out = s.sB[tid] * g;
+  }
+  return mine;
+}
+
+}
diff --git a/lion_amd/csrc/pointwise.hip b/lion_amd/csrc/pointwise.hip
--- a/lion_amd/csrc/pointwise.hip
+++ b/lion_amd/csrc/pointwise.hip
@@ -1,4 +1,5 @@
 #include "common.h"
+#include "gn_fold.h"
 
 namespace {
 
@@ -63,6 +64,45 @@
                                                      swishf(v.z * a + b) + w.z, swishf(v.w * a + b) + w.w);
   } else {
     for (int j = i; j < L && j < i + 4; ++j) q[j] = swishf(p[j] * a + b) + ad[j];
+  }
+}
+
+constexpr int FOLD_ASA_IT = 4, FOLD_ASA_ELEMS = FOLD_ASA_IT * 1024;
+template <bool VEC>
+__global__ __launch_bounds__(256) void fold_affine_swish_add_kernel(lion_fold::Args f, const float *__restrict__ x,
+                                                                    const float *__restrict__ addend, int L,
+                                                                    float *__restrict__ y) {
+  __shared__ lion_fold::Lds lds;
+  __shared__ float sa[64], sb[64];
+  const int g = blockIdx.y, b = blockIdx.z, tid = threadIdx.x, cpg = f.C / f.G;
+  const size_t base = ((size_t)b * f.C + (size_t)g * cpg) * L;
+  const int n = cpg * L;
+  const int e0 = blockIdx.x * FOLD_ASA_ELEMS;
+  const float *p = x + base, *ad = addend + base;
+  float *q = y + base;
+  float4 v[FOLD_ASA_IT], w[FOLD_ASA_IT];
+  if (VEC) {
+#pragma unroll
+    for (int i = 0; i < FOLD_ASA_IT; ++i) {
+      const int e = e0 + (i * 256 + tid) * 4;
+      if (e < n) { v[i] = *reinterpret_cast<const float4 *>(p + e); w[i] = *reinterpret_cast<const float4 *>(ad + e); }
+    }
+  }
+  float a, bs;
+  if (lion_fold::fold_groups<1>(f, b, g, 1, tid, lds, nullptr, a, bs)) { sa[tid] = a; sb[tid] = bs; }
+  __syncthreads();
+  if (VEC) {
+#pragma unroll
+    for (int i = 0; i < FOLD_ASA_IT; ++i) {
+      const int e = e0 + (i * 256 + tid) * 4;
+      if (e < n) {
+        const float ca = sa[e / L], cb = sb[e / L];
+        *reinterpret_cast<float4 *>(q + e) = make_float4(swishf(v[i].x * ca + cb) + w[i].x, swishf(v[i].y * ca + cb) + w[i].y,
+                                                         swishf(v[i].z * ca + cb) + w[i].z, swishf(v[i].w * ca + cb) + w[i].w);
+      }
+    }
+  } else {
+    for (int e = e0 + tid; e < n && e < e0 + FOLD_ASA_ELEMS; e += 256) q[e] = swishf(p[e] * sa[e / L] + sb[e / L]) + ad[e];
   }
 }
 
@@ -224,6 +264,22 @@
   return 0;
 }
 
+int lion_fold_affine_swish_add(const float *stats, int B, int C, int T, int G, int count, const float *gamma,
+                               const float *beta, const float *fac, const float *gbias, int ld_fg, float eps,
+                               const float *x, const float *addend, int L, float *y, lionStream_t stream) {
+  if (!stats || !gamma || !beta || !fac || !gbias || !x || !addend || !y) return LION_EINVAL;
+  if (B <= 0 || C <= 0 || T <= 0 || G <= 0 || L <= 0 || C % G != 0 || C / G > 64 || ld_fg < C) return LION_EINVAL;
+  if (B > 65535 || G > 65535 || (long)(C / G) * L >= (1L << 31) - FOLD_ASA_ELEMS) return LION_EUNSUPPORTED;
+  const lion_fold::Args f = {stats, C, T, G, (float)count, gamma, beta, fac, gbias, ld_fg, eps};
+  const dim3 grid(lion_cdiv((C / G) * L, FOLD_ASA_ELEMS), G, B);
+  hipStream_t st = static_cast<hipStream_t>(stream);
+  const bool vec = (L & 3) == 0 && ((((uintptr_t)x) | ((uintptr_t)addend) | ((uintptr_t)y)) & 15) == 0;
+  if (vec) fold_affine_swish_add_kernel<true><<<grid, 256, 0, st>>>(f, x, addend, L, y);
+  else fold_affine_swish_add_kernel<false><<<grid, 256, 0, st>>>(f, x, addend, L, y);
+  LION_LAUNCH_CHECK();
+  return 0;
+}
+
 int lion_affine_swish_max(const float *x, const float *A, const float *Bs, int rows, int M, int U,
                           float *y, lionStream_t stream) {
   if (!x || !A || !Bs || !y || rows <= 0 || M <= 0 || U <= 0) return LION_EINVAL;
diff --git a/lion_amd/fused_ops.py b/lion_amd/fused_ops.py
--- a/lion_amd/fused_ops.py
+++ b/lion_amd/fused_ops.py
@@ -27,6 +27,9 @@
     buf = torch.empty((2, n), device=counts.device, dtype=torch.int32)
     _lib.call("lion_conv3d_tile_occupancy_aware", counts.contiguous(), b, r, cout, buf[0], buf[1], int(consumer_aware))
     return buf[0], buf[1]
+
+
+FOLD_MAX_TILES = int(os.environ.get("LION_FOLD_MAX_TILES", "128"))
 
 
 class FoldSpec:
@@ -45,7 +48,29 @@
         return a, b_
 
 
-def conv3d_fused(x, conv, pro=None, want_stats=True, occ=None, prev_conv=None, split=None, fold=None):
+class PendingFold:
+
+    def __init__(self, stats, spec: FoldSpec):
+        self.stats, self.spec = stats, spec
+
+    def resolve(self):
+        return self.spec.apply(self.stats)
+
+    def args(self):
+        gn, c = self.spec.gn, self.stats.shape[1]
+        fac, gbias = _fg_rows(self.spec.fac, self.spec.gbias, c)
+        return dict(stats=self.stats, b=self.stats.shape[0], c=c, t=self.stats.shape[2], g=gn.num_groups,
+                    count=self.spec.count, gamma=gn.weight, beta=gn.bias, fac=fac, gbias=gbias, ld=int(fac.stride(0)),
+                    eps=float(gn.eps))
+
+
+def _fg_rows(fac, gbias, c):
+    if not (fac.stride(1) == 1 and gbias.stride(1) == 1 and fac.stride(0) == gbias.stride(0) and fac.stride(0) >= c):
+        fac, gbias = fac.contiguous(), gbias.contiguous()
+    return fac, gbias
+
+
+def conv3d_fused(x, conv, pro=None, want_stats=True, occ=None, prev_conv=None, split=None, fold=None, defer=False):
     lib = _lib.load()
     b, cin, r = x.shape[0], x.shape[1], x.shape[2]
     cout = conv.out_channels
@@ -58,14 +83,25 @@
     wp = conv_ops.split_packed_weight(conv.weight) if use_split else packed_weight(conv.weight)
     y = torch.empty((b, cout, r, r, r), device=x.device, dtype=torch.float32)
     pa = pb = pbias = tconst = None
-    if pro is not None:
-        pa, pb = pro[0].contiguous(), pro[1].contiguous()
     bias = conv.bias.detach().contiguous() if conv.bias is not None else None
     sparse = occ is not None and r >= 16
-    if sparse and pro is not None:
-        if prev_conv is None or cin > 256:
-            sparse = False
+    if sparse and pro is not None and (prev_conv is None or cin > 256):
+        sparse = False
+    if isinstance(pro, PendingFold):
+        p = pro.args()
+        if sparse and pro.spec.se is None and p["g"] <= 32 and p["c"] == cin and cin // p["g"] <= 64:
+            ws = border_weight_sums(conv.weight)
+            pbias = prev_conv.bias.detach().contiguous() if prev_conv.bias is not None else None
+            tconst = torch.empty((b, 27, cout), device=x.device, dtype=torch.float32)
+            pa = torch.empty((b, cin), device=x.device, dtype=torch.float32)
+            pb = torch.empty_like(pa)
+            _lib.call("lion_conv3d_fold_const_response", p["stats"], b, cin, p["t"], p["g"], p["count"], p["gamma"], p["beta"],
+                      p["fac"], p["gbias"], p["ld"], p["eps"], ws, bias, pbias, cout, pa, pb, tconst)
         else:
+            pro = pro.resolve()
+    if pro is not None and pa is None:
+        pa, pb = pro[0].contiguous(), pro[1].contiguous()
+        if sparse:
             ws = border_weight_sums(conv.weight)
             pbias = prev_conv.bias.detach().contiguous() if prev_conv.bias is not None else None
             tconst = torch.empty((b, 27, cout), device=x.device, dtype=torch.float32)
@@ -81,6 +117,8 @@
         entry = "lion_conv3d_k3_half_forward" if conv_ops.use_half(cin, cout, r, x) else "lion_conv3d_k3_split_forward"
     _lib.call(entry, x, wp, bias, b, cin, cout, r, pa, pb, pbias, tconst, y, stats, occ)
     if fold is not None:
+        if defer and stats.shape[2] <= FOLD_MAX_TILES:
+            return y, PendingFold(stats, fold)
         return y, fold.apply(stats)
     return y, stats
 
@@ -90,8 +128,7 @@
     A = torch.empty((b, c), device=stats.device, dtype=torch.float32)
     Bs = torch.empty_like(A)
     cm = torch.empty_like(A)
-    if not (fac.stride(1) == 1 and gbias.stride(1) == 1 and fac.stride(0) == gbias.stride(0) and fac.stride(0) >= c):
-        fac, gbias = fac.contiguous(), gbias.contiguous()
+    fac, gbias = _fg_rows(fac, gbias, c)
     _lib.call("lion_groupnorm_fold", stats, b, c, t, gn.num_groups, int(voxels), gn.weight, gn.bias, fac, gbias,
               int(fac.stride(0)), float(gn.eps), A, Bs, cm)
     return A, Bs, cm
@@ -105,8 +142,7 @@
         return None
     A = torch.empty((b, c), device=stats.device, dtype=torch.float32)
     Bs = torch.empty_like(A)
-    if not (fac.stride(1) == 1 and gbias.stride(1) == 1 and fac.stride(0) == gbias.stride(0) and fac.stride(0) >= c):
-        fac, gbias = fac.contiguous(), gbias.contiguous()
+    fac, gbias = _fg_rows(fac, gbias, c)
     _lib.call("lion_groupnorm_fold_se", stats, b, c, t, gn.num_groups, int(voxels), gn.weight, gn.bias, fac, gbias,
               int(fac.stride(0)), float(gn.eps), w1, w2, h, A, Bs)
     return A, Bs
@@ -133,10 +169,21 @@
     return {"buf": buf, "coords": coords, "shape": (b, n, int(r))}
 
 
-def devoxelize_affine(grid, coords, r, scale, shift, plan=None):
+def devoxelize_affine(grid, coords, r, scale, shift=None, plan=None):
     b, c = grid.shape[:2]
     n = coords.shape[2]
     out = torch.empty((b, c, n), device=grid.device, dtype=torch.float32)
+    if isinstance(scale, PendingFold):
+        pend, se = scale, scale.spec.se
+        if se is not None and int(r) <= 16 and n <= 2048:
+            w1, w2 = se.fc[0].weight.detach(), se.fc[2].weight.detach()
+            p = pend.args()
+            if (4 <= c <= 256 and p["c"] == c and w1.shape[0] <= 128 and w1.is_contiguous() and w2.is_contiguous()
+                    and _lib.call("lion_trilinear_devoxelize_fold_se_forward", coords.contiguous(), grid.contiguous(),
+                                  p["stats"], p["t"], p["g"], p["count"], p["gamma"], p["beta"], p["fac"], p["gbias"],
+                                  p["ld"], p["eps"], w1, w2, w1.shape[0], b, c, n, int(r), out, unsupported_ok=True)):
+                return out
+        scale, shift = pend.resolve()
     co_c, gr_c, sc_c, sh_c = coords.contiguous(), grid.contiguous(), scale.contiguous(), shift.contiguous()
     if plan is not None and plan["shape"] == (b, n, int(r)) and plan["coords"].data_ptr() == co_c.data_ptr():
         buf = plan["buf"]
@@ -334,7 +381,17 @@
     return y
 
 
-def shared_mlp(x, convs, adagns, style, reduce_max=False, add=None):
+def fold_affine_swish_add(x, stats, gn: torch.nn.GroupNorm, fac, gbias, add):
+    p = PendingFold(stats, FoldSpec(gn, fac, gbias, x[0, 0].numel())).args()
+    add = add.contiguous()
+    assert add.shape == x.shape and add.dtype == torch.float32
+    y = torch.empty_like(x)
+    ok = _lib.call("lion_fold_affine_swish_add", p["stats"], p["b"], p["c"], p["t"], p["g"], p["count"], p["gamma"], p["beta"],
+                   p["fac"], p["gbias"], p["ld"], p["eps"], x, add, x[0, 0].numel(), y, unsupported_ok=True)
+    return y if ok else None
+
+
+def shared_mlp(x, convs, adagns, style, reduce_max=False, add=None, fold_at_consumer=False):
     pro = None
     for li, (conv, gn) in enumerate(zip(convs, adagns)):
         if (MAX_RECOMPUTE and reduce_max and add is None and li == len(convs) - 1 and x.dim() == 4 and x.shape[3] == 32
@@ -351,6 +408,11 @@
             x = conv(x).contiguous()
             st = row_stats(x).view(x.shape[0], x.shape[1], 1, 2)
         f, g = gn.affine(style)
+        if (fold_at_consumer and add is not None and not reduce_max and li == len(convs) - 1
+                and st.shape[2] <= FOLD_MAX_TILES and x.shape[1] // gn.norm.num_groups <= 64):
+            out = fold_affine_swish_add(x, st, gn.norm, f, g, add)
+            if out is not None:
+                return out
         A, Bs, _ = groupnorm_fold(st, gn.norm, f, g, x[0, 0].numel())
         pro = (A, Bs)
     out = affine_swish(x, pro[0], pro[1], reduce_max, add=None if reduce_max else add)
diff --git a/lion_amd/models/pvcnn2_ada.py b/lion_amd/models/pvcnn2_ada.py
--- a/lion_amd/models/pvcnn2_ada.py
+++ b/lion_amd/models/pvcnn2_ada.py
@@ -23,6 +23,7 @@
 SKIP_UNREAD_LEVEL2 = os.environ.get("LION_CONV_SKIP_UNREAD_LEVEL2", "1") != "0"
 OCC_CLONE = os.environ.get("LION_OCC_CLONE", "0") != "0"
 DEVOX_PLAN = os.environ.get("LION_DEVOX_PLAN", "1") != "0"
+FOLD_AT_CONSUMER = os.environ.get("LION_FOLD_AT_CONSUMER", "1") != "0"
 
 
 @contextlib.contextmanager
@@ -257,7 +258,7 @@
         if self._fusable(x):
             n = len(self.layers) // 3
             convs, gns = [self.layers[3 * i] for i in range(n)], [self.layers[3 * i + 1] for i in range(n)]
-            return fused_ops.shared_mlp(x, convs, gns, style, reduce_max, add=add)
+            return fused_ops.shared_mlp(x, convs, gns, style, reduce_max, add=add, fold_at_consumer=FOLD_AT_CONSUMER)
         x = run_layers(list(self.layers), x, style, conv1x1, reduce_max=reduce_max)
         return x if add is None else x + add
 
@@ -361,12 +362,14 @@
         if SPARSE_CONV1 and counts is not None and r >= 16:
             occ1, occ2 = _occupancy(counts, r, conv1.out_channels, grid.shape[0], self._aware_level())
         f1, g1 = gn1.affine(style)
-        y1, (a1, b1) = fused_ops.conv3d_fused(grid, conv1, None, True, occ1,
-                                              fold=fused_ops.FoldSpec(gn1.norm, f1, g1, r ** 3))
+        defer = FOLD_AT_CONSUMER
+        y1, pro1 = fused_ops.conv3d_fused(grid, conv1, None, True, occ1,
+                                          fold=fused_ops.FoldSpec(gn1.norm, f1, g1, r ** 3), defer=defer)
         f2, g2 = gn2.affine(style)
-        y2, (a2, b2) = fused_ops.conv3d_fused(y1, conv2, (a1, b1), True, occ2, prev_conv=conv1,
-                                              fold=fused_ops.FoldSpec(gn2.norm, f2, g2, r ** 3, se))
-        return fused_ops.devoxelize_affine(y2, voxel_coords, r, a2, b2, plan=_devox_plan(voxel_coords, r))
+        y2, pro2 = fused_ops.conv3d_fused(y1, conv2, pro1, True, occ2, prev_conv=conv1,
+                                          fold=fused_ops.FoldSpec(gn2.norm, f2, g2, r ** 3, se), defer=defer and se is not None)
+        scale, shift = (pro2, None) if isinstance(pro2, fused_ops.PendingFold) else pro2
+        return fused_ops.devoxelize_affine(y2, voxel_coords, r, scale, shift, plan=_devox_plan(voxel_coords, r))
 
     def forward(self, inputs):
         features, coords_input, time_emb, style = inputs
```

Result: no change. 5.413, median of 6 (+0.4%).
